# zju3dv/EnvGS

Hardware: AMD Instinct MI355X
Metric: train iters/s (fwd+bwd of the render hot path + Adam step, one 800x800 view per GPU per iter) + render Mpix/s (higher is better)
Workload: dtype f32

## Files before the change

### envgs_amd/_lib.py

```python
import ctypes
import os

import torch

HERE = os.path.dirname(os.path.abspath(__file__))
LIB_PATH = os.path.join(HERE, "libenvgs_hip.so")
_lib = None

c_void_p, c_int, c_uint32, c_size_t = ctypes.c_void_p, ctypes.c_int, ctypes.c_uint32, ctypes.c_size_t


class RasterCfg(ctypes.Structure):
    _fields_ = [("P", ctypes.c_int32), ("sh_degree", ctypes.c_int32), ("sh_coeffs", ctypes.c_int32),
                ("channels", ctypes.c_int32), ("width", ctypes.c_int32), ("height", ctypes.c_int32),
                ("bg_len", ctypes.c_int32), ("debug", ctypes.c_int32), ("scale_modifier", ctypes.c_float),
                ("tanfovx", ctypes.c_float), ("tanfovy", ctypes.c_float), ("feature_f16", ctypes.c_int32)]


class AdamTensor(ctypes.Structure):
    _fields_ = [("param", ctypes.c_void_p), ("grad", ctypes.c_void_p), ("exp_avg", ctypes.c_void_p), ("exp_avg_sq", ctypes.c_void_p),
                ("numel", ctypes.c_int64), ("lr", ctypes.c_float), ("step", ctypes.c_float)]


class RowsTensor(ctypes.Structure):
    _fields_ = [("src", ctypes.c_void_p), ("dst", ctypes.c_void_p), ("row_bytes", ctypes.c_int64)]


class GrowTensor(ctypes.Structure):
    _fields_ = [("src", ctypes.c_void_p), ("dst", ctypes.c_void_p), ("row_bytes", ctypes.c_int64), ("kind", ctypes.c_int32), ("reserved0", ctypes.c_int32)]


class DensifyPlanArgs(ctypes.Structure):
    _fields_ = ([("P", ctypes.c_int64), ("N", ctypes.c_int32), ("flags", ctypes.c_uint32)]
                + [(n, ctypes.c_float) for n in ("grad_threshold", "size_limit", "split_screen_threshold", "min_opacity", "min_gradient", "r")]
                + [(n, ctypes.c_void_p) for n in ("ga", "dn", "mr", "wa", "scal", "opac", "cls", "scan", "counters", "temp")]
                + [("temp_bytes", ctypes.c_size_t)])


class DensifyRewriteArgs(ctypes.Structure):
    _fields_ = ([("P", ctypes.c_int64), ("out_rows", ctypes.c_int64), ("n_samples", ctypes.c_int64), ("N", ctypes.c_int32), ("count", ctypes.c_int32),
                 ("ratio_n", ctypes.c_double), ("r", ctypes.c_float), ("reserved0", ctypes.c_uint32)]
                + [(n, ctypes.c_void_p) for n in ("cls", "scan", "counters", "scal", "rotation", "samples")]
                + [("tensors", ctypes.POINTER(GrowTensor))])


class TraceLists(ctypes.Structure):
    _fields_ = [("hit_lists", ctypes.c_void_p), ("hit_cnt", ctypes.c_void_p), ("n_used", ctypes.c_void_p), ("cap", ctypes.c_int32),
                ("surf_acc", ctypes.c_void_p), ("surf_cnt", ctypes.c_void_p), ("surf_off", ctypes.c_void_p),
                ("scan_temp", ctypes.c_void_p), ("scan_temp_bytes", ctypes.c_size_t), ("ray_keys", ctypes.c_void_p),
                ("ray_order", ctypes.c_void_p), ("ray_sort_temp", ctypes.c_void_p), ("ray_sort_temp_bytes", ctypes.c_size_t),
                ("records", ctypes.c_void_p),
                ("num_records", ctypes.c_uint64), ("hit_state", ctypes.c_void_p), ("entries", ctypes.c_void_p), ("pairs", ctypes.c_void_p),
                ("n_entries", ctypes.c_void_p), ("compact_rows", ctypes.c_uint64), ("row_off", ctypes.c_void_p), ("batch_rows", ctypes.c_void_p),
                ("row_blk", ctypes.c_void_p), ("sh_perm", ctypes.c_void_p), ("state_planes", ctypes.c_int32),
                ("sparse_hits", ctypes.c_void_p), ("sparse_cap", ctypes.c_uint64),
                ("defer_reduce", ctypes.c_uint32), ("reserved0", ctypes.c_uint32), ("bwd_order", ctypes.c_void_p)]


class TraceCfg(ctypes.Structure):
    _fields_ = [("P", ctypes.c_int32), ("num_rays", ctypes.c_int32), ("sh_degree", ctypes.c_int32),
                ("sh_coeffs", ctypes.c_int32), ("max_trace_depth", ctypes.c_int32), ("start_from_first", ctypes.c_int32),
                ("has_others", ctypes.c_int32), ("bg_len", ctypes.c_int32), ("debug", ctypes.c_int32),
                ("ray_h", ctypes.c_int32), ("ray_w", ctypes.c_int32),
                ("scale_modifier", ctypes.c_float), ("specular_threshold", ctypes.c_float), ("feature_f16", ctypes.c_int32)]


TRACE_COUNTER_WORDS, TRACE_COUNTER_MIRROR, TRACE_MAX_SEG = 96, 72, 4
CTR_RAY_FETCH, CTR_MAX_LIST, CTR_TOTALS = 0, 1, 2
(TOT_HITS, TOT_NODE_VISITS, TOT_ROUNDS, TOT_FOUND, TOT_PACKET_NODES, TOT_PACKET_LEAVES, TOT_COOP_EXPAND, TOT_COOP_WALK, TOT_COOP_WAIT,
 TOT_COUNT) = range(10)
CTR_STACK_OVERFLOWS, CTR_RAYS_WITHOUT_ROWS, CTR_ROW_CLAIM, CTR_LONG_QUEUE, CTR_SEG_FIRST_ROW = 20, 21, 22, 24, 28
CTR_BATCH_FETCH, CTR_BATCH_FETCH_STRIDE = 32, 8
CTR_SPARSE_FILED, CTR_BATCH_ENTRIES, CTR_SPARSE_SKIPPED = 64, 65, 66
DBG_TRACE, DBG_TRACE_NO_SORT, DBG_TRACE_SMALL_STACK, DBG_TRACE_PREPARE_INLINE = 0, 64, 1024, 16384
DBG_TRACE_RETIRED = 8 | 16 | 512 | 2048 | 4096 | 8192


class SupervisorArgs(ctypes.Structure):
    _fields_ = ([("N", ctypes.c_int64), ("P", ctypes.c_int64), ("flags", ctypes.c_uint32), ("reserved0", ctypes.c_uint32),
                 ("weight", ctypes.c_float * 5), ("reserved1", ctypes.c_float)]
                + [(n, ctypes.c_void_p) for n in ("norm_map", "surf_norm_map", "acc_map", "dpt_map", "dist_map", "env_opacity", "prior", "msk", "R", "near_far")]
                + [(n, ctypes.c_int64) for n in ("norm_map_row", "norm_map_ch", "surf_norm_map_row", "surf_norm_map_ch", "acc_map_row", "dpt_map_row",
                                                 "dist_map_row", "env_opacity_row", "prior_row", "prior_ch", "msk_row")]
                + [(n, ctypes.c_void_p) for n in ("g_norm_map", "g_surf_norm_map", "g_acc_map", "g_dist_map", "g_env_opacity", "partial")])


class SurfelInputsArgs(ctypes.Structure):
    _fields_ = ([(n, ctypes.c_int32) for n in ("P", "sh_degree", "sh_coeffs", "spec_channels")]
                + [(n, ctypes.c_void_p) for n in ("xyz", "features_dc", "features_rest", "scaling", "rotation", "opacity", "specular", "roughness", "campos",
                                                  "scales", "rotations", "opacities", "specular_act", "roughness_act", "shs", "colors", "others", "vertices",
                                                  "clamped",
                                                  "g_scales", "g_rotations", "g_opacities", "g_specular_act", "g_roughness_act", "g_shs", "g_colors", "g_others",
                                                  "d_xyz", "d_features_dc", "d_features_rest", "d_scaling", "d_rotation", "d_opacity", "d_specular", "d_roughness")])


class TsdfVolume(ctypes.Structure):
    _fields_ = ([(n, ctypes.c_int32) for n in ("nx", "ny", "nz")] + [(n, ctypes.c_float) for n in ("ox", "oy", "oz", "voxel")]
                + [(n, ctypes.c_void_p) for n in ("tsdf", "weight", "rgb")])


class TsdfView(ctypes.Structure):
    _fields_ = [("depth", ctypes.c_void_p), ("rgb", ctypes.c_void_p), ("H", ctypes.c_int32), ("W", ctypes.c_int32),
                ("fx", ctypes.c_float), ("fy", ctypes.c_float), ("cx", ctypes.c_float), ("cy", ctypes.c_float),
                ("R", ctypes.c_float * 9), ("T", ctypes.c_float * 3), ("depth_max", ctypes.c_float), ("trunc", ctypes.c_float)]


class TsdfViews(ctypes.Structure):
    _fields_ = [("count", ctypes.c_int32), ("reserved0", ctypes.c_int32), ("v", TsdfView * 8)]


_P = c_void_p
SYMBOLS = {
    "envgs_raster_scan_temp_bytes": (c_size_t, [ctypes.c_int32]),
    "envgs_raster_sort_temp_bytes": (c_size_t, [c_uint32, ctypes.c_int32, ctypes.c_int32]),
    "envgs_raster_project": (c_int, [ctypes.POINTER(RasterCfg)] + [_P] * 15 + [_P, c_size_t, ctypes.POINTER(c_uint32), _P]),
    "envgs_raster_bin_and_render": (c_int, [ctypes.POINTER(RasterCfg), c_uint32] + [_P] * 7 + [_P, c_size_t] + [_P] * 7 + [_P]),
    "envgs_raster_render_audit": (c_int, [ctypes.POINTER(RasterCfg)] + [_P] * 11 + [ctypes.c_int32, _P, _P]),
    "envgs_raster_backward": (c_int, [ctypes.POINTER(RasterCfg), c_uint32] + [_P] * 29 + [_P]),
    "envgs_bvh_temp_bytes": (c_size_t, [ctypes.c_int32]),
    "envgs_bvh_node_floats": (c_size_t, [ctypes.c_int32]),
    "envgs_bvh_build": (c_int, [ctypes.c_int32, _P, _P, _P, _P, c_size_t, ctypes.c_int32, _P]),
    "envgs_bvh_refit": (c_int, [ctypes.c_int32, _P, _P, _P, _P, _P, c_size_t, ctypes.c_int32, _P]),
    "envgs_bvh_quality": (c_int, [ctypes.c_int32, _P, _P, _P]),
    "envgs_trace_ray_sort_temp_bytes": (c_size_t, [ctypes.c_int32]),
    "envgs_trace_ray_order": (c_int, [ctypes.c_int32, _P, _P, _P, ctypes.c_int32, _P, _P, _P, c_size_t, _P]),
    "envgs_trace_forward": (c_int, [ctypes.POINTER(TraceCfg)] + [_P] * 22 + [ctypes.POINTER(TraceLists), _P]),
    "envgs_trace_backward": (c_int, [ctypes.POINTER(TraceCfg)] + [_P] * 35 + [ctypes.POINTER(TraceLists), _P]),
    "envgs_trace_backward_join": (c_int, [_P]),
    "envgs_sh_colors_forward": (c_int, [ctypes.c_int32] * 4 + [_P] * 7 + [_P]),
    "envgs_sh_colors_backward": (c_int, [ctypes.c_int32] * 4 + [_P] * 9 + [_P]),
    "envgs_surfel_quads": (c_int, [ctypes.c_int32] + [_P] * 5 + [_P]),
    "envgs_blend_forward": (c_int, [ctypes.c_int32] * 3 + [_P] * 3 + [_P]),
    "envgs_blend_backward": (c_int, [ctypes.c_int32] * 3 + [_P] * 5 + [_P]),
    "envgs_bounce_rays_forward": (c_int, [ctypes.c_int32] + [_P] * 8 + [_P]),
    "envgs_bounce_rays_backward": (c_int, [ctypes.c_int32] + [_P] * 13 + [_P]),
    "envgs_bounce_blend_forward": (c_int, [ctypes.c_int32] + [_P] * 5 + [_P]),
    "envgs_bounce_blend_backward": (c_int, [ctypes.c_int32] + [_P] * 8 + [_P]),
    "envgs_bounce_pack_mid": (c_int, [ctypes.c_int32, _P, ctypes.c_int32, ctypes.c_int32] + [_P] * 8 + [_P]),
    "envgs_reflect_forward": (c_int, [ctypes.c_int32, ctypes.c_int32, ctypes.c_float] + [_P] * 8 + [_P]),
    "envgs_reflect_backward": (c_int, [ctypes.c_int32, ctypes.c_int32, ctypes.c_float] + [_P] * 11 + [_P]),
    "envgs_select_acc": (c_int, [ctypes.c_int32, ctypes.c_int32, ctypes.c_float, _P, _P, _P]),
    "envgs_reflect_filtered_forward": (c_int, [ctypes.c_int32, ctypes.c_int32, ctypes.c_float, ctypes.c_int32] + [_P] * 10 + [_P]),
    "envgs_reflect_filtered_backward": (c_int, [ctypes.c_int32, ctypes.c_int32, ctypes.c_float, ctypes.c_int32] + [_P] * 13 + [_P]),
    "envgs_blend_filtered_forward": (c_int, [ctypes.c_int32] * 4 + [_P] * 6 + [_P]),
    "envgs_blend_filtered_backward": (c_int, [ctypes.c_int32] * 4 + [_P] * 7 + [_P]),
    "envgs_surface_normal_forward": (c_int, [ctypes.c_int32, ctypes.c_int32, ctypes.c_float, ctypes.c_float, ctypes.c_float] + [_P] * 4 + [_P]),
    "envgs_surface_normal_backward": (c_int, [ctypes.c_int32, ctypes.c_int32, ctypes.c_float, ctypes.c_float, ctypes.c_float] + [_P] * 5 + [_P]),
    "envgs_surfel_inputs_forward": (c_int, [ctypes.POINTER(SurfelInputsArgs), _P]),
    "envgs_surfel_inputs_backward": (c_int, [ctypes.POINTER(SurfelInputsArgs), _P]),
    "envgs_fused_adam": (c_int, [ctypes.c_int32, ctypes.POINTER(AdamTensor), ctypes.c_float, ctypes.c_float, ctypes.c_float, _P]),
    "envgs_compact_temp_bytes": (ctypes.c_size_t, [ctypes.c_int64]),
    "envgs_compact_scan": (c_int, [ctypes.c_int64, _P, _P, _P, _P, ctypes.c_size_t, _P]),
    "envgs_compact_gather": (c_int, [ctypes.c_int32, ctypes.POINTER(RowsTensor), ctypes.c_int64, _P, _P, _P]),
    "envgs_compact_gather_rows": (c_int, [ctypes.c_int32, ctypes.POINTER(RowsTensor), ctypes.c_int64, ctypes.c_int64, _P, _P, _P]),
    "envgs_knn3_mean_dist2": (c_int, [ctypes.c_int32, _P, _P, _P]),
    "envgs_densify_stats": (c_int, [ctypes.c_int64, ctypes.c_int32] + [_P] * 8 + [_P]),
    "envgs_densify_plan_temp_bytes": (ctypes.c_size_t, [ctypes.c_int64]),
    "envgs_densify_plan": (c_int, [ctypes.POINTER(DensifyPlanArgs), _P]),
    "envgs_densify_split_stds": (c_int, [ctypes.c_int64, ctypes.c_int32] + [_P] * 5 + [ctypes.c_int64, _P]),
    "envgs_densify_rewrite": (c_int, [ctypes.POINTER(DensifyRewriteArgs), _P]),
    "envgs_weight_select_temp_bytes": (ctypes.c_size_t, []),
    "envgs_weight_select": (c_int, [ctypes.c_int64, _P, _P, ctypes.c_int32, ctypes.c_int64, ctypes.c_int64, _P, _P, _P, ctypes.c_size_t, _P]),
    "envgs_visibility_mask_temp_bytes": (ctypes.c_size_t, [ctypes.c_int64]),
    "envgs_visibility_mask": (c_int, [ctypes.c_int64, _P, _P, ctypes.c_int64, _P, _P, _P, _P, ctypes.c_size_t, _P]),
    "envgs_oversize_plan": (c_int, [ctypes.c_int64, c_uint32, ctypes.c_float, ctypes.c_float] + [_P] * 8 + [_P]),
    "envgs_tsdf_integrate": (c_int, [ctypes.POINTER(TsdfVolume), ctypes.POINTER(TsdfViews), ctypes.c_float, _P]),
    "envgs_mesh_temp_bytes": (c_size_t, [ctypes.c_int32] * 3),
    "envgs_mesh_count": (c_int, [ctypes.POINTER(TsdfVolume), ctypes.c_float, ctypes.c_float, _P, c_size_t, _P, _P]),
    "envgs_mesh_extract": (c_int, [ctypes.POINTER(TsdfVolume), ctypes.c_float, _P, c_size_t, c_uint32, c_uint32, _P, _P, _P, _P]),
    "envgs_mesh_components_temp_bytes": (c_size_t, [c_uint32, c_uint32]),
    "envgs_mesh_components": (c_int, [c_uint32, c_uint32, _P, _P, c_size_t] + [_P] * 5 + [_P]),
    "envgs_mesh_select_temp_bytes": (c_size_t, [c_uint32, c_uint32]),
    "envgs_mesh_select_count": (c_int, [c_uint32, c_uint32, _P, _P, _P, c_size_t, _P, _P]),
    "envgs_mesh_select_emit": (c_int, [c_uint32, c_uint32] + [_P] * 4 + [_P, c_size_t, c_uint32, c_uint32] + [_P] * 4 + [_P]),
    "envgs_mesh_simplify_temp_bytes": (c_size_t, [c_uint32, c_uint32] + [ctypes.c_int32] * 3),
    "envgs_mesh_simplify_cluster": (c_int, [c_uint32, c_uint32, _P, _P, _P] + [ctypes.c_float] * 4 + [ctypes.c_int32] * 3 + [_P, c_size_t] + [_P] * 6 + [_P]),
    "envgs_mesh_sample_temp_bytes": (c_size_t, [c_uint32, c_uint32]),
    "envgs_mesh_sample_count": (c_int, [c_uint32, c_uint32, _P, _P, ctypes.c_float, c_uint32, _P, c_size_t, _P, _P]),
    "envgs_mesh_sample_emit": (c_int, [c_uint32, c_uint32, _P, _P, _P, c_uint32, _P, c_size_t, c_uint32, _P, _P, _P, _P]),
    "envgs_points_grid_temp_bytes": (c_size_t, [c_uint32] + [ctypes.c_int32] * 3),
    "envgs_points_grid_build": (c_int, [c_uint32, _P] + [ctypes.c_float] * 4 + [ctypes.c_int32] * 3 + [_P, c_size_t, _P, _P, _P]),
    "envgs_points_nearest": (c_int, [c_uint32, _P] + [ctypes.c_float] * 5 + [ctypes.c_int32] * 3 + [_P] * 4 + [_P]),
    "envgs_l1_ssim_partial_count": (ctypes.c_int64, [ctypes.c_int32, ctypes.c_int32, ctypes.c_int32]),
    "envgs_l1_ssim_forward": (c_int, [ctypes.c_int32, ctypes.c_int32, ctypes.c_int32, _P, _P, _P, _P, _P]),
    "envgs_l1_ssim_backward": (c_int, [ctypes.c_int32, ctypes.c_int32, ctypes.c_int32, _P, _P, _P, _P, ctypes.c_float, ctypes.c_float, _P, _P]),
    "envgs_depth_percentiles_temp_bytes": (c_size_t, []),
    "envgs_depth_percentiles": (c_int, [ctypes.c_int64, _P, ctypes.c_int64, _P, _P, c_size_t, _P]),
    "envgs_supervisor_partial_count": (ctypes.c_int64, [ctypes.c_int64, ctypes.c_int64]),
    "envgs_supervisor_forward": (c_int, [ctypes.POINTER(SupervisorArgs), _P]),
    "envgs_supervisor_finish": (c_int, [ctypes.POINTER(SupervisorArgs), _P, _P]),
    "envgs_supervisor_backward": (c_int, [ctypes.c_int64, _P, _P, _P, _P]),
    "envgs_debug_set": (None, [ctypes.c_int32, ctypes.c_int32]),
    "envgs_debug_get": (ctypes.c_int32, [ctypes.c_int32]),
    "envgs_prof_enable": (None, [c_int]),
    "envgs_prof_select": (None, [ctypes.c_uint64]),
    "envgs_prof_read": (c_int, [c_int, ctypes.POINTER(ctypes.c_double), ctypes.POINTER(c_int)]),
    "envgs_prof_kernel_name": (ctypes.c_char_p, [c_int]),
}


LIB_DIAG_PATH = os.path.join(HERE, "libenvgs_hip_diag.so")
_libs = {}
_selected = {"kind": "product"}


def _open(path):
    if not os.path.exists(path):
        raise RuntimeError(
            "envgs_amd: %s is missing. Build it with `python -m envgs_amd.build` (hipcc, gfx950). "
            "There is no CPU fallback for the render-and-trace path." % path)
    lib = ctypes.CDLL(path)
    for name, (res, args) in SYMBOLS.items():
        fn = getattr(lib, name)
        fn.restype = res
        fn.argtypes = args
    return lib


def load():
    global _lib
    kind = _selected["kind"]
    lib = _libs.get(kind)
    if lib is None:
        lib = _libs[kind] = _open(LIB_PATH if kind == "product" else LIB_DIAG_PATH)
    _lib = lib
    return lib


def select(kind):
    if kind not in ("product", "diag"):
        raise ValueError(kind)
    old = _selected["kind"]
    _selected["kind"] = kind
    load()
    return old


def ptr(t):
    return None if t is None else ctypes.c_void_p(t.data_ptr())


def check(rc, what):
    if rc != 0:
        raise RuntimeError("envgs_amd: %s failed with code %d (%s)" % (
            what, rc, {-1: "bad argument", -2: "temp buffer too small"}.get(rc, "hipError_t")))
```

### envgs_amd/csrc/common.h

```cpp
#pragma once
#include <hip/hip_runtime.h>
#include <hip/hip_fp16.h>
#include <stdint.h>

#include "../../include/envgs_raster.h"
#include "prof.h"

namespace envgs {

constexpr int TILE = ENVGS_TILE;
constexpr int GEOM = ENVGS_GEOM_STRIDE;
constexpr int GREC = ENVGS_GRAD_STRIDE;
constexpr float NEAR_N = 0.2f;
constexpr float FAR_N = 100.0f;
constexpr float FILTER_SIZE = 0.707106f;
constexpr float FILTER_INV_SQ = 2.0f;
constexpr float ALPHA_CAP = 0.99f;
constexpr float ALPHA_MIN = 1.0f / 255.0f;
constexpr float T_EPS = 0.0001f;

struct Feat {
    const void *p;
    bool h;
    __device__ __forceinline__ float operator[](size_t i) const {
        return h ? __half2float(reinterpret_cast<const __half *>(p)[i]) : reinterpret_cast<const float *>(p)[i];
    }
    __device__ __forceinline__ Feat at(size_t i) const { return Feat{reinterpret_cast<const char *>(p) + i * (h ? 2 : 4), h}; }
};

#define ENVGS_CHECK_LAUNCH(cfg, stream)                                             \
    do {                                                                            \
        hipError_t e__ = hipGetLastError();                                         \
        if (e__ != hipSuccess) return (int)e__;                                     \
        if ((cfg)->debug) {                                                         \
            e__ = hipStreamSynchronize((hipStream_t)(stream));                      \
            if (e__ != hipSuccess) return (int)e__;                                 \
        }                                                                           \
    } while (0)

template <int CTRL, int ROW_MASK = 0xf, int BANK_MASK = 0xf, bool BOUND = true>
__device__ __forceinline__ float dpp_mov(float v) {
    return __builtin_bit_cast(float, __builtin_amdgcn_update_dpp(0, __builtin_bit_cast(int, v), CTRL, ROW_MASK, BANK_MASK, BOUND));
}
template <int CTRL> __device__ __forceinline__ int dpp_mov_i32(int v) { return __builtin_amdgcn_update_dpp(0, v, CTRL, 0xf, 0xf, true); }
__device__ __forceinline__ float quad_sum(float v) { v += dpp_mov<0xB1>(v); v += dpp_mov<0x4E>(v); return v; }

__device__ __forceinline__ float wave_sum(float v) {
    v += dpp_mov<0xB1>(v);
    v += dpp_mov<0x4E>(v);
    v += dpp_mov<0x141>(v);
    v += dpp_mov<0x140>(v);
    v += dpp_mov<0x142, 0xa, 0xf, false>(v);
    v += dpp_mov<0x143, 0xc, 0xf, false>(v);
    return __builtin_bit_cast(float, __builtin_amdgcn_readlane(__builtin_bit_cast(int, v), 63));
}


typedef unsigned envgs_u2 __attribute__((ext_vector_type(2)));

__device__ __forceinline__ float wave_reduce64(const float (&g)[64], const int lane)
{
    float z[32];
#pragma unroll
    for (int i = 0; i < 32; i++) {
        const envgs_u2 r = __builtin_amdgcn_permlane32_swap(__float_as_uint(g[i]), __float_as_uint(g[i + 32]), false, false);
        z[i] = __uint_as_float(r.x) + __uint_as_float(r.y);
    }
    float w[16];
#pragma unroll
    for (int k = 0; k < 16; k++) {
        const envgs_u2 q = __builtin_amdgcn_permlane16_swap(__float_as_uint(z[k]), __float_as_uint(z[k + 16]), false, false);
        w[k] = __uint_as_float(q.x) + __uint_as_float(q.y);
    }
    const bool b3 = lane & 8, b2 = lane & 4, b1 = lane & 2, b0 = lane & 1;
    float a[8];
#pragma unroll
    for (int k = 0; k < 8; k++) a[k] = (b3 ? w[k + 8] : w[k]) + dpp_mov<0x140>(b3 ? w[k] : w[k + 8]);
    float b[4];
#pragma unroll
    for (int k = 0; k < 4; k++) b[k] = (b2 ? a[k + 4] : a[k]) + dpp_mov<0x141>(b2 ? a[k] : a[k + 4]);
    float c[2];
#pragma unroll
    for (int k = 0; k < 2; k++) c[k] = (b1 ? b[k + 2] : b[k]) + dpp_mov<0x1B>(b1 ? b[k] : b[k + 2]);
    return (b0 ? c[1] : c[0]) + dpp_mov<0xB1>(b0 ? c[0] : c[1]);
}

template <int CTRL, int ROW_MASK = 0xf>
__device__ __forceinline__ float dpp_fill(float v, float ident) {
    return __builtin_bit_cast(float, __builtin_amdgcn_update_dpp(__builtin_bit_cast(int, ident), __builtin_bit_cast(int, v), CTRL, ROW_MASK, 0xf, false));
}
__device__ __forceinline__ float wave_scan_add(float v) {
    v += dpp_fill<0x111>(v, 0.f); v += dpp_fill<0x112>(v, 0.f); v += dpp_fill<0x114>(v, 0.f); v += dpp_fill<0x118>(v, 0.f);
    v += dpp_fill<0x142, 0xa>(v, 0.f);
    v += dpp_fill<0x143, 0xc>(v, 0.f);
    return v;
}
__device__ __forceinline__ float wave_scan_mul(float v) {
    v *= dpp_fill<0x111>(v, 1.f); v *= dpp_fill<0x112>(v, 1.f); v *= dpp_fill<0x114>(v, 1.f); v *= dpp_fill<0x118>(v, 1.f);
    v *= dpp_fill<0x142, 0xa>(v, 1.f);
    v *= dpp_fill<0x143, 0xc>(v, 1.f);
    return v;
}
__device__ __forceinline__ float wave_bcast(float v, int l) { return __builtin_bit_cast(float, __builtin_amdgcn_readlane(__builtin_bit_cast(int, v), l)); }

template <int CTRL, int ROW_MASK = 0xf>
__device__ __forceinline__ uint32_t dpp_fill_u32(uint32_t v) {
    return (uint32_t)__builtin_amdgcn_update_dpp(0, (int)v, CTRL, ROW_MASK, 0xf, false);
}
__device__ __forceinline__ uint32_t wave_scan_add_u32(uint32_t v) {
    v += dpp_fill_u32<0x111>(v); v += dpp_fill_u32<0x112>(v); v += dpp_fill_u32<0x114>(v); v += dpp_fill_u32<0x118>(v);
    v += dpp_fill_u32<0x142, 0xa>(v);
    v += dpp_fill_u32<0x143, 0xc>(v);
    return v;
}

template <int N4>
__device__ __forceinline__ float wave_transpose_reduce(const float (&g)[4 * N4], const int lane)
{
    float z[2 * N4];
#pragma unroll
    for (int i = 0; i < 2 * N4; i++) {
        const envgs_u2 r = __builtin_amdgcn_permlane32_swap(__float_as_uint(g[i]), __float_as_uint(g[i + 2 * N4]), false, false);
        z[i] = __uint_as_float(r.x) + __uint_as_float(r.y);
    }
    float w[N4];
#pragma unroll
    for (int k = 0; k < N4; k++) {
        const envgs_u2 q = __builtin_amdgcn_permlane16_swap(__float_as_uint(z[k]), __float_as_uint(z[k + N4]), false, false);
        float v = __uint_as_float(q.x) + __uint_as_float(q.y);
        v += dpp_mov<0x128>(v);
        v += dpp_mov<0x124>(v);
        v += dpp_mov<0x122>(v);
        v += dpp_mov<0x121>(v);
        w[k] = v;
    }
    float out = w[0];
#pragma unroll
    for (int k = 1; k < N4; k++) out = ((lane & 15) == k) ? w[k] : out;
    return out;
}

__device__ __forceinline__ int lane_id() { return __builtin_amdgcn_mbcnt_hi(~0u, __builtin_amdgcn_mbcnt_lo(~0u, 0u)); }

template <int NW>
__device__ __forceinline__ uint32_t block_exclusive_u32(uint32_t v, uint32_t *s_w, uint32_t &total)
{
    const int lane = lane_id(), wave = threadIdx.x >> 6;
    const uint32_t inc = wave_scan_add_u32(v);
    if (lane == 63) s_w[wave] = inc;
    __syncthreads();
    uint32_t before = 0, all = 0;
#pragma unroll
    for (int k = 0; k < NW; k++) { const uint32_t t = s_w[k]; all += t; before += (k < wave) ? t : 0u; }
    total = all;
    __syncthreads();
    return before + inc - v;
}

__device__ __forceinline__ void atomic_add_f32(float *p, float v) { unsafeAtomicAdd(p, v); }

int launch_project(const envgs_raster_cfg *cfg, const float *means3D, const float *scales, const float *rotations,
                   const float *opacities, const float *shs, const float *transmat_precomp, const float *viewmatrix,
                   const float *projmatrix, const float *campos, float *geom, float *rgb, uint8_t *clamped,
                   int32_t *radii, uint32_t *tiles_touched, hipStream_t stream);
int launch_scan(const uint32_t *in, uint32_t *out, int n, void *temp, size_t temp_bytes, hipStream_t stream);
size_t scan_temp_bytes(int n);
size_t sort_temp_bytes(uint32_t n, int width, int height);
int launch_bin(const envgs_raster_cfg *cfg, uint32_t N, const float *geom, const int32_t *radii, uint64_t *tile_pairs,
               uint64_t *keys_sorted, uint32_t *point_list, void *bin_temp, size_t bin_temp_bytes, uint32_t *ranges, hipStream_t stream);
size_t key_sort_temp_bytes(int n);
int launch_key_sort(int n, const uint64_t *keys_in, uint64_t *keys_out, int top_bit, void *temp, size_t temp_bytes, hipStream_t stream);
size_t ray_sort_temp_bytes(int R);
int launch_ray_sort(int R, const float *ray_o, const float *ray_d, const float4 *nodes, int P, uint64_t *pairs, uint32_t *order, void *temp,
                    size_t temp_bytes, hipStream_t stream);
int launch_render_fwd(const envgs_raster_cfg *cfg, const uint32_t *ranges, const uint32_t *point_list, const float *geom,
                      const float *colors, const float *bg, float *out_color, float *allmap, float *final_T,
                      int32_t *n_contrib, float *weight, hipStream_t stream, uint8_t *audit_contrib = nullptr, int audit_lmax = 0, int colors_f16 = 0,
                      uint8_t *contrib_mask = nullptr, const uint8_t *audit_skip = nullptr);
int launch_render_bwd(const envgs_raster_cfg *cfg, const uint32_t *ranges, const uint32_t *point_list, const float *geom,
                      const float *colors, const float *bg, const float *final_T, const int32_t *n_contrib,
                      const float *dL_dcolor, const float *dL_dallmap, float *grad_rec, hipStream_t stream, int colors_f16 = 0,
                      const uint8_t *contrib_mask = nullptr);
int launch_project_bwd(const envgs_raster_cfg *cfg, const float *geom, const float *means3D, const float *scales,
                       const float *rotations, const float *shs, const uint8_t *clamped, const float *transmat_precomp,
                       const int32_t *radii, const float *viewmatrix, const float *projmatrix, const float *campos,
                       const float *grad_rec, float *dmeans3D, float *dmeans2D, float *dscales, float *drots, float *dshs,
                       float *dcolors, float *dopacities, float *dtransmat_precomp, hipStream_t stream);

int launch_sh_record_bwd(int P, int D, const float *means3D, const float *shs, const float *campos, const uint8_t *clamped, const int32_t *radii,
                         const float *grad_rec, float *dmeans3D, float *dshs, hipStream_t stream);

__host__ __device__ inline int tile_bits(int width, int height) {
    int tiles = ((width + TILE - 1) / TILE) * ((height + TILE - 1) / TILE);
    int b = 0;
    while ((1 << b) < tiles) b++;
    return b < 1 ? 1 : b;
}

}
```

### envgs_amd/csrc/raster_api.hip

```cpp
#include "common.h"

using namespace envgs;

extern "C" {

size_t envgs_raster_scan_temp_bytes(int32_t P) { return scan_temp_bytes(P); }

size_t envgs_raster_sort_temp_bytes(uint32_t N, int32_t width, int32_t height)
{
    return sort_temp_bytes(N, width, height);
}

static int check_cfg(const envgs_raster_cfg *cfg)
{
    if (!cfg) return ENVGS_ERR_BAD_ARG;
    if (cfg->channels != 3 && cfg->channels != 5 && cfg->channels != 7) return ENVGS_ERR_BAD_ARG;
    if (cfg->sh_degree < 0 || cfg->sh_degree > 3) return ENVGS_ERR_BAD_ARG;
    if (cfg->width <= 0 || cfg->height <= 0 || cfg->P < 0) return ENVGS_ERR_BAD_ARG;
    return 0;
}

int envgs_raster_project(const envgs_raster_cfg *cfg, const float *means3D, const float *scales, const float *rotations,
                         const float *opacities, const float *shs, const float *transmat_precomp,
                         const float *viewmatrix, const float *projmatrix, const float *campos, float *geom, float *rgb,
                         uint8_t *clamped, int32_t *radii, uint32_t *tiles_touched, uint32_t *offsets, void *scan_temp,
                         size_t scan_temp_bytes_, uint32_t *num_rendered_host, void *stream_)
{
    int rc = check_cfg(cfg);
    if (rc) return rc;
    if (num_rendered_host) *num_rendered_host = 0;
    if (cfg->P == 0) return 0;
    if (!means3D || !opacities || !viewmatrix || !projmatrix || !geom || !radii || !tiles_touched || !offsets) return ENVGS_ERR_BAD_ARG;
    if (!transmat_precomp && (!scales || !rotations)) return ENVGS_ERR_BAD_ARG;
    if (shs && (cfg->channels != 3 || !rgb || !clamped || !campos || cfg->sh_coeffs < (cfg->sh_degree + 1) * (cfg->sh_degree + 1))) return ENVGS_ERR_BAD_ARG;
    hipStream_t stream = (hipStream_t)stream_;
    rc = launch_project(cfg, means3D, scales, rotations, opacities, shs, transmat_precomp, viewmatrix, projmatrix, campos,
                        geom, rgb, clamped, radii, tiles_touched, stream);
    if (rc) return rc;
    if (scan_temp_bytes_ < scan_temp_bytes(cfg->P)) return ENVGS_ERR_TEMP_TOO_SMALL;
    rc = launch_scan(tiles_touched, offsets, cfg->P, scan_temp, scan_temp_bytes_, stream);
    if (rc) return rc;
    if (!num_rendered_host) return 0;
    hipError_t e = hipMemcpyAsync(num_rendered_host, offsets + (cfg->P - 1), sizeof(uint32_t), hipMemcpyDeviceToHost, stream);
    if (e != hipSuccess) return (int)e;
    e = hipStreamSynchronize(stream);
    return (int)e;
}

int envgs_raster_bin_and_render(const envgs_raster_cfg *cfg, uint32_t N, const float *geom, const int32_t *radii,
                                const float *colors, const float *bg, uint64_t *tile_pairs, uint64_t *keys_sorted, uint32_t *point_list,
                                void *bin_temp, size_t bin_temp_bytes_, uint32_t *ranges, float *out_color, float *allmap,
                                float *final_T, int32_t *n_contrib, float *weight, uint8_t *contrib_mask, void *stream_)
{
    int rc = check_cfg(cfg);
    if (rc) return rc;
    if (!ranges || !out_color || !allmap || !final_T || !n_contrib || !bg) return ENVGS_ERR_BAD_ARG;
    if (cfg->P > 0 && (!geom || !radii || !colors || !weight)) return ENVGS_ERR_BAD_ARG;
    if (N > 0 && (!tile_pairs || !point_list || !bin_temp)) return ENVGS_ERR_BAD_ARG;
    hipStream_t stream = (hipStream_t)stream_;
    rc = launch_bin(cfg, N, geom, radii, tile_pairs, keys_sorted, point_list, bin_temp, bin_temp_bytes_, ranges, stream);
    if (rc) return rc;
    return launch_render_fwd(cfg, ranges, point_list, geom, colors, bg, out_color, allmap, final_T, n_contrib, weight, stream, nullptr, 0,
                             (cfg->feature_f16 && cfg->sh_coeffs == 0) ? 1 : 0, contrib_mask);
}

int envgs_raster_render_audit(const envgs_raster_cfg *cfg, const float *geom, const float *colors, const float *bg,
                              const uint32_t *point_list, const uint32_t *ranges, float *out_color, float *allmap, float *final_T,
                              int32_t *n_contrib, float *weight, uint8_t *contrib, int32_t lmax, const uint8_t *skip_px, void *stream_)
{
    int rc = check_cfg(cfg);
    if (rc) return rc;
    if (!ranges || !out_color || !allmap || !final_T || !n_contrib || !bg || !contrib || lmax <= 0) return ENVGS_ERR_BAD_ARG;
    if (cfg->P > 0 && (!geom || !colors || !weight || !point_list)) return ENVGS_ERR_BAD_ARG;
    hipStream_t stream = (hipStream_t)stream_;
    hipError_t e = hipMemsetAsync(contrib, 0, (size_t)cfg->width * cfg->height * (size_t)lmax, stream);
    if (e != hipSuccess) return (int)e;
    return launch_render_fwd(cfg, ranges, point_list, geom, colors, bg, out_color, allmap, final_T, n_contrib, weight, stream, contrib, lmax,
                             (cfg->feature_f16 && cfg->sh_coeffs == 0) ? 1 : 0, nullptr, skip_px);
}

int envgs_raster_backward(const envgs_raster_cfg *cfg, uint32_t N, const float *geom, const float *colors, const float *bg,
                          const uint32_t *point_list, const uint32_t *ranges, const float *final_T,
                          const int32_t *n_contrib, const uint8_t *contrib_mask, const float *dL_dcolor, const float *dL_dallmap, const float *means3D,
                          const float *scales, const float *rotations, const float *shs, const uint8_t *clamped,
                          const float *transmat_precomp, const int32_t *radii, const float *viewmatrix,
                          const float *projmatrix, const float *campos, float *grad_rec, float *dmeans3D, float *dmeans2D,
                          float *dscales, float *drots, float *dshs, float *dcolors, float *dopacities,
                          float *dtransmat_precomp, void *stream_)
{
    int rc = check_cfg(cfg);
    if (rc) return rc;
    if (cfg->P == 0) return 0;
    if (!geom || !colors || !bg || !ranges || !final_T || !n_contrib || !grad_rec || !radii ||
        !dmeans2D || !dopacities || !viewmatrix || !projmatrix)
        return ENVGS_ERR_BAD_ARG;
    if (N > 0 && !point_list) return ENVGS_ERR_BAD_ARG;
    if (shs ? (!dshs || !clamped || !campos || !means3D) : !dcolors) return ENVGS_ERR_BAD_ARG;
    if (transmat_precomp ? !dtransmat_precomp : (!scales || !rotations || !means3D || !dmeans3D || !dscales || !drots)) return ENVGS_ERR_BAD_ARG;
    hipStream_t stream = (hipStream_t)stream_;
    rc = launch_render_bwd(cfg, ranges, point_list, geom, colors, bg, final_T, n_contrib, dL_dcolor, dL_dallmap, grad_rec, stream,
                           (cfg->feature_f16 && !shs) ? 1 : 0, contrib_mask);
    if (rc) return rc;
    return launch_project_bwd(cfg, geom, means3D, scales, rotations, shs, clamped, transmat_precomp, radii, viewmatrix,
                              projmatrix, campos, grad_rec, dmeans3D, dmeans2D, dscales, drots, dshs, dcolors, dopacities,
                              dtransmat_precomp, stream);
}

}
```

### envgs_amd/csrc/raster_bin.hip

```cpp
#include "common.h"
#include "ray_key.h"
#include "tile_sort.h"

namespace envgs {

constexpr int SCAN_ITEMS = 1024;

size_t scan_temp_bytes(int n) { return sizeof(uint32_t) * (size_t)(((n > 0 ? n : 1) + SCAN_ITEMS - 1) / SCAN_ITEMS) + 64; }

__global__ void __launch_bounds__(256)
scan_block_sums(const uint32_t *__restrict__ in, uint32_t *__restrict__ sums, int n)
{
    __shared__ uint32_t s_w[5];
    const int base = blockIdx.x * SCAN_ITEMS + threadIdx.x * 4;
    uint32_t s = 0;
#pragma unroll
    for (int k = 0; k < 4; k++) s += (base + k < n) ? in[base + k] : 0u;
    uint32_t total;
    (void)block_exclusive_u32<4>(s, s_w, total);
    if (threadIdx.x == 0) sums[blockIdx.x] = total;
}

__global__ void __launch_bounds__(256)
scan_apply(const uint32_t *in, uint32_t *out, const uint32_t *__restrict__ sums, int n)
{
    __shared__ uint32_t s_w[5];
    uint32_t pre = 0;
    for (int k = threadIdx.x; k < (int)blockIdx.x; k += 256) pre += sums[k];
    uint32_t before;
    (void)block_exclusive_u32<4>(pre, s_w, before);
    const int base = blockIdx.x * SCAN_ITEMS + threadIdx.x * 4;
    uint32_t a[4];
#pragma unroll
    for (int k = 0; k < 4; k++) a[k] = (base + k < n) ? in[base + k] : 0u;
    a[1] += a[0]; a[2] += a[1]; a[3] += a[2];
    uint32_t total;
    const uint32_t ex = block_exclusive_u32<4>(a[3], s_w, total) + before;
#pragma unroll
    for (int k = 0; k < 4; k++) if (base + k < n) out[base + k] = ex + a[k];
}

int launch_scan(const uint32_t *in, uint32_t *out, int n, void *temp, size_t temp_bytes, hipStream_t stream)
{
    if (n <= 0) return 0;
    if (temp_bytes < scan_temp_bytes(n)) return ENVGS_ERR_TEMP_TOO_SMALL;
    ProfScope prof_(K_SCAN, stream);
    const int nb = (n + SCAN_ITEMS - 1) / SCAN_ITEMS;
    hipLaunchKernelGGL(scan_block_sums, dim3(nb), dim3(256), 0, stream, in, (uint32_t *)temp, n);
    hipLaunchKernelGGL(scan_apply, dim3(nb), dim3(256), 0, stream, in, out, (const uint32_t *)temp, n);
    return (int)hipGetLastError();
}

constexpr int BIN_ROWS_MAX = 512;
constexpr int BIN_SLICE_MIN = 1024;
constexpr int BIN_BAND = 16384;
constexpr int BIG_RECT = 32;
constexpr int SORT_LONG_N = 16384;
constexpr int SORT_LONG_WGS = 256;

struct BinPlan { int rows, slice, ntiles; };
static BinPlan bin_plan(int P, int W, int H)
{
    BinPlan p;
    p.ntiles = ((W + TILE - 1) / TILE) * ((H + TILE - 1) / TILE);
    int rows = (P + BIN_SLICE_MIN - 1) / BIN_SLICE_MIN;
    rows = rows < 1 ? 1 : (rows > BIN_ROWS_MAX ? BIN_ROWS_MAX : rows);
    p.slice = (((P + rows - 1) / rows + 255) / 256) * 256;
    p.rows = p.slice > 0 ? (P + p.slice - 1) / p.slice : 1;
    if (p.rows < 1) p.rows = 1;
    return p;
}

size_t sort_temp_bytes(uint32_t, int width, int height)
{
    const size_t ntiles = (size_t)((width + TILE - 1) / TILE) * ((height + TILE - 1) / TILE);
    return sizeof(uint32_t) * ((size_t)BIN_ROWS_MAX * ntiles + 3 * ntiles + 1 + 4) + 256;
}

__device__ __forceinline__ bool tile_rect(int i, int W, int H, const float *__restrict__ geom, const int32_t *__restrict__ radii,
                                          int &x0, int &y0, int &x1, int &y1, uint32_t &dbits)
{
    const int rad = radii[i];
    if (rad <= 0) return false;
    const float cx = geom[(size_t)i * GEOM + 9], cy = geom[(size_t)i * GEOM + 10];
    dbits = __float_as_uint(geom[(size_t)i * GEOM + 15]);
    const float radius = (float)rad;
    const int gx = (W + TILE - 1) / TILE, gy = (H + TILE - 1) / TILE;
    x0 = (int)((cx - radius) / (float)TILE); x0 = x0 < 0 ? 0 : (x0 > gx ? gx : x0);
    y0 = (int)((cy - radius) / (float)TILE); y0 = y0 < 0 ? 0 : (y0 > gy ? gy : y0);
    x1 = (int)((cx + radius + (float)(TILE - 1)) / (float)TILE); x1 = x1 < 0 ? 0 : (x1 > gx ? gx : x1);
    y1 = (int)((cy + radius + (float)(TILE - 1)) / (float)TILE); y1 = y1 < 0 ? 0 : (y1 > gy ? gy : y1);
    return x1 > x0 && y1 > y0;
}

struct SurfelRect { int x0, y0, x1, y1; uint32_t dbits; bool vis; };
__device__ __forceinline__ SurfelRect load_rect(int i, int g1, int W, int H, const float *__restrict__ geom, const int32_t *__restrict__ radii)
{
    SurfelRect r;
    r.x0 = r.y0 = r.x1 = r.y1 = 0; r.dbits = 0;
    r.vis = i < g1 && tile_rect(i, W, H, geom, radii, r.x0, r.y0, r.x1, r.y1, r.dbits);
    return r;
}

template <bool SCATTER>
__global__ void __launch_bounds__(256)
bin_pass(int P, int W, int H, int slice, int ntiles, const float *__restrict__ geom, const int32_t *__restrict__ radii,
         uint32_t *hist, const uint32_t *__restrict__ tile_start, uint64_t *__restrict__ pairs, uint32_t cap)
{
    extern __shared__ uint32_t s_bin[];
    const int gx = (W + TILE - 1) / TILE;
    const int g0 = blockIdx.x * slice, g1 = min(P, g0 + slice);
    uint32_t *row = hist + (size_t)blockIdx.x * ntiles;
    const int lane = lane_id();
    for (int band0 = 0; band0 < ntiles; band0 += BIN_BAND) {
        const int bn = min(BIN_BAND, ntiles - band0);
        SurfelRect cur = load_rect(g0 + (int)threadIdx.x, g1, W, H, geom, radii);
        for (int t = threadIdx.x; t < bn; t += 256) s_bin[t] = SCATTER ? tile_start[band0 + t] + row[band0 + t] : 0u;
        __syncthreads();
        auto visit = [&](int t, uint64_t pair) {
            t -= band0;
            if ((unsigned)t >= (unsigned)bn) return;
            const uint32_t slot = atomicAdd(&s_bin[t], 1u);
            if (SCATTER && slot < cap) pairs[slot] = pair;
        };
        for (int ib = g0; ib < g1; ib += 256) {
            const int i = ib + (int)threadIdx.x;
            const SurfelRect c = cur;
            cur = load_rect(i + 256, g1, W, H, geom, radii);
            const int x0 = c.x0, y0 = c.y0, x1 = c.x1, y1 = c.y1;
            const uint32_t dbits = c.dbits;
            const bool vis = c.vis;
            const uint64_t pair = ((uint64_t)dbits << 32) | (uint32_t)i;
            const bool big = vis && (x1 - x0) * (y1 - y0) > BIG_RECT;
            if (vis && !big)
                for (int y = y0; y < y1; y++)
                    for (int x = x0; x < x1; x++) visit(y * gx + x, pair);
            uint64_t m = __builtin_amdgcn_ballot_w64(big);
            while (m) {
                const int l = __builtin_ctzll(m);
                m &= m - 1;
                const int bx0 = __builtin_amdgcn_readlane(x0, l), by0 = __builtin_amdgcn_readlane(y0, l);
                const int bw = __builtin_amdgcn_readlane(x1, l) - bx0, bh = __builtin_amdgcn_readlane(y1, l) - by0;
                const uint64_t bp = ((uint64_t)(uint32_t)__builtin_amdgcn_readlane((int)dbits, l) << 32) | (uint32_t)__builtin_amdgcn_readlane(i, l);
                for (int k = lane; k < bw * bh; k += 64) visit((by0 + k / bw) * gx + bx0 + k % bw, bp);
            }
        }
        __syncthreads();
        if (!SCATTER)
            for (int t = threadIdx.x; t < bn; t += 256) row[band0 + t] = s_bin[t];
        __syncthreads();
    }
}

constexpr int CS_SEG = 16, CS_ROWS = BIN_ROWS_MAX / CS_SEG;
__global__ void __launch_bounds__(256)
bin_column_scan(int rows, int ntiles, uint32_t *hist, uint32_t *__restrict__ tile_count)
{
    __shared__ uint32_t s_seg[CS_SEG][16];
    const int tl = threadIdx.x & 15, seg = threadIdx.x >> 4;
    const int t = blockIdx.x * 16 + tl;
    const int per = (rows + CS_SEG - 1) / CS_SEG, r0 = seg * per;
    uint32_t v[CS_ROWS];
    uint32_t s = 0;
#pragma unroll
    for (int k = 0; k < CS_ROWS; k++) {
        const int r = r0 + k;
        v[k] = (t < ntiles && k < per && r < rows) ? hist[(size_t)r * ntiles + t] : 0u;
        s += v[k];
    }
    s_seg[seg][tl] = s;
    __syncthreads();
    uint32_t acc = 0;
#pragma unroll
    for (int k = 0; k < CS_SEG; k++) acc += (k < seg) ? s_seg[k][tl] : 0u;
    if (t >= ntiles) return;
#pragma unroll
    for (int k = 0; k < CS_ROWS; k++) {
        const int r = r0 + k;
        if (k < per && r < rows) hist[(size_t)r * ntiles + t] = acc;
        acc += v[k];
    }
    if (seg == CS_SEG - 1) tile_count[t] = acc;
}

__global__ void __launch_bounds__(1024)
bin_tile_scan(int ntiles, const uint32_t *__restrict__ tile_count, uint32_t *__restrict__ tile_start, uint32_t *__restrict__ ranges,
              uint32_t cap, uint32_t *__restrict__ hdr)
{
    __shared__ uint32_t s_w[17];
    const int per = (ntiles + 1023) / 1024, b = min(ntiles, (int)threadIdx.x * per), e = min(ntiles, b + per);
    uint32_t s = 0;
    for (int k = b; k < e; k++) s += tile_count[k];
    uint32_t total;
    uint32_t run = block_exclusive_u32<16>(s, s_w, total);
    const bool ok = total <= cap;
    for (int k = b; k < e; k++) {
        const uint32_t c = tile_count[k];
        tile_start[k] = run;
        ranges[2 * k] = (c && ok) ? run : 0u;
        ranges[2 * k + 1] = (c && ok) ? run + c : 0u;
        run += c;
    }
    if (threadIdx.x == 0) { tile_start[ntiles] = total; hdr[0] = total; hdr[1] = 0u; hdr[2] = 0u; hdr[3] = 0u; }
}

template <int NT>
__device__ __forceinline__ void sort_padded_lds(uint64_t *s, int lp, int tid)
{
    const int npad = 1 << lp;
    for (int g = tid; g < (npad >> TS_S); g += NT) bitonic_first(s, g, lp);
    __syncthreads();
    for (int lk = TS_S + 1; lk <= lp; lk++)
        for (int a = lk - 1; a >= 0;) {
            const int S = ts_chunk(a);
            if (S == 4) { for (int g = tid; g < (npad >> 4); g += NT) bitonic_group<4>(s, g, lk, a, lp); }
            else if (S == 3) { for (int g = tid; g < (npad >> 3); g += NT) bitonic_group<3>(s, g, lk, a, lp); }
            else if (S == 2) { for (int g = tid; g < (npad >> 2); g += NT) bitonic_group<2>(s, g, lk, a, lp); }
            else { for (int g = tid; g < (npad >> 1); g += NT) bitonic_group<1>(s, g, lk, a, lp); }
            __syncthreads();
            a -= S;
        }
}

template <int NT>
__device__ __forceinline__ void merge_padded_lds(uint64_t *s, int lc, int tid)
{
    const int npad = 1 << lc;
    for (int a = lc - 1; a >= 0;) {
        const int S = ts_chunk(a);
        if (S == 4) { for (int g = tid; g < (npad >> 4); g += NT) bitonic_group<4>(s, g, lc, a, lc); }
        else if (S == 3) { for (int g = tid; g < (npad >> 3); g += NT) bitonic_group<3>(s, g, lc, a, lc); }
        else if (S == 2) { for (int g = tid; g < (npad >> 2); g += NT) bitonic_group<2>(s, g, lc, a, lc); }
        else { for (int g = tid; g < (npad >> 1); g += NT) bitonic_group<1>(s, g, lc, a, lc); }
        __syncthreads();
        a -= S;
    }
}

constexpr int lds_slots(int lp_cap) { return (1 << lp_cap) + (1 << (lp_cap - 5)); }

__device__ __forceinline__ void store_sorted(uint64_t v, uint32_t tile, size_t at, uint64_t *keys_sorted, uint32_t *point_list, int full64)
{
    if (full64) { keys_sorted[at] = v; return; }
    point_list[at] = (uint32_t)v;
    if (keys_sorted) keys_sorted[at] = ((uint64_t)tile << 32) | (v >> 32);
}

template <int NT>
__device__ __forceinline__ void load_sort_write(uint64_t *s, const uint64_t *pairs, int n, uint32_t tile, uint32_t b,
                                                uint64_t *keys_sorted, uint32_t *point_list, int tid, int full64)
{
    const int lp = ts_log2_padded(n);
    for (int i = tid; i < (1 << lp); i += NT) s[ts_slot(i)] = i < n ? pairs[b + i] : ~0ull;
    __syncthreads();
    sort_padded_lds<NT>(s, lp, tid);
    for (int i = tid; i < n; i += NT) store_sorted(s[ts_slot(i)], tile, (size_t)b + i, keys_sorted, point_list, full64);
}

template <int LP_CAP, int NT>
__global__ void __launch_bounds__(NT)
sort_tile_lists(const uint32_t *__restrict__ ranges, const uint64_t *pairs, uint64_t *keys_sorted, uint32_t *__restrict__ point_list,
                uint32_t *__restrict__ hdr, uint32_t *__restrict__ long_list, int full64)
{
    __shared__ uint64_t s_k[lds_slots(LP_CAP)];
    const uint32_t t = blockIdx.x, b = ranges[2 * t];
    const int n = (int)(ranges[2 * t + 1] - b);
    if (n == 0) return;
    if (n > (1 << LP_CAP)) {
        if (threadIdx.x == 0) long_list[atomicAdd(&hdr[1], 1u)] = t;
        return;
    }
    load_sort_write<NT>(s_k, pairs, n, t, b, keys_sorted, point_list, (int)threadIdx.x, full64);
}

constexpr int LONG_ITEM = 4096;
constexpr int LONG_BATCH = 256;

__device__ __forceinline__ uint32_t long_claim(uint32_t *hdr, uint32_t *s_item)
{
    __syncthreads();
    if (threadIdx.x == 0) *s_item = atomicAdd(&hdr[2], 1u);
    __syncthreads();
    return *s_item;
}
__device__ __forceinline__ void long_wait(uint32_t *hdr, const uint32_t base)
{
    if (threadIdx.x == 0)
        while (__hip_atomic_load(&hdr[3], __ATOMIC_ACQUIRE, __HIP_MEMORY_SCOPE_AGENT) < base) __builtin_amdgcn_s_sleep(4);
    __syncthreads();
    __threadfence();
}
__device__ __forceinline__ void long_done(uint32_t *hdr)
{
    __threadfence();
    __syncthreads();
    if (threadIdx.x == 0) __hip_atomic_fetch_add(&hdr[3], 1u, __ATOMIC_RELEASE, __HIP_MEMORY_SCOPE_AGENT);
}

__global__ void __launch_bounds__(1024)
sort_long_lists(const uint32_t *__restrict__ ranges, uint64_t *pairs, uint64_t *keys_sorted, uint32_t *__restrict__ point_list,
                uint32_t *hdr, const uint32_t *__restrict__ long_list, int full64)
{
    __shared__ uint64_t s_long[lds_slots(14)];
    __shared__ uint32_t s_item;
    __shared__ uint32_t s_bt[LONG_BATCH], s_bb[LONG_BATCH], s_bn[LONG_BATCH], s_pref[LONG_BATCH + 1];
    const uint32_t count = hdr[1];
    const int tid = (int)threadIdx.x, G = (int)gridDim.x;
    constexpr int LC = 14, C = 1 << LC;
    const bool copy_out = !(full64 && keys_sorted == pairs);
    uint32_t small_seen = 0u, big = 0u;
    for (uint32_t w = 0; w < count; w++) {
        const uint32_t t = long_list[w], b = ranges[2 * t];
        const int n = (int)(ranges[2 * t + 1] - b);
        if (n > SORT_LONG_N) { big++; continue; }
        if ((small_seen++ % (uint32_t)G) != blockIdx.x) continue;
        load_sort_write<1024>(s_long, pairs, n, t, b, keys_sorted, point_list, tid, full64);
        __syncthreads();
    }
    if (big == 0u) return;
    auto lp_of = [&](const int n) { int lp = LC; while ((1 << lp) < n) lp++; return lp; };
    auto items_of = [&](const int kind, const int lk, const int n) -> uint32_t {
        const int lp = lp_of(n);
        if (kind == 1) return lk <= lp ? (uint32_t)(((1ll << (lp - 1)) + LONG_ITEM - 1) / LONG_ITEM) : 0u;
        return (kind == 2 || lk <= lp) ? (uint32_t)((n + C - 1) / C) : 0u;
    };
    auto do_item = [&](const int kind, const int lk, const int q, const int l, const uint32_t it) {
        const uint32_t t = s_bt[l], b = s_bb[l];
        const int n = (int)s_bn[l];
        uint64_t *seg = pairs + b;
        if (kind == 0) {
            const int c = (int)it;
            for (int i = tid; i < C; i += 1024) s_long[ts_slot(i)] = ((long long)c * C + i) < n ? seg[(size_t)c * C + i] : ~0ull;
            __syncthreads();
            if (lk == LC) sort_padded_lds<1024>(s_long, LC, tid);
            else merge_padded_lds<1024>(s_long, LC, tid);
            for (int i = tid; i < C; i += 1024)
                if ((long long)c * C + i < n) seg[(size_t)c * C + i] = s_long[ts_slot(i)];
        } else if (kind == 1) {
            const int lp = lp_of(n);
            const long long i0 = (long long)it * LONG_ITEM, i1 = min(i0 + LONG_ITEM, 1ll << (lp - 1));
            for (long long idx = i0 + tid; idx < i1; idx += 1024) ascending_step(seg, n, lk, q, (int)idx);
        } else {
            const long long i0 = (long long)it * C, i1 = min(i0 + C, (long long)n);
            for (long long i = i0 + tid; i < i1; i += 1024) store_sorted(seg[i], t, (size_t)b + (size_t)i, keys_sorted, point_list, full64);
        }
    };
    uint32_t base = 0u, my = long_claim(hdr, &s_item);
    uint32_t w = 0;
    while (w < count) {
        __syncthreads();
        int nl = 0, lp_max = LC;
        for (; w < count && nl < LONG_BATCH; w++) {
            const uint32_t t = long_list[w], b = ranges[2 * t];
            const int n = (int)(ranges[2 * t + 1] - b);
            if (n <= SORT_LONG_N) continue;
            if (tid == 0) { s_bt[nl] = t; s_bb[nl] = b; s_bn[nl] = (uint32_t)n; }
            lp_max = max(lp_max, lp_of(n));
            nl++;
        }
        if (nl == 0) break;
        auto run_phase = [&](const int kind, const int lk, const int q) {
            __syncthreads();
            if (tid < nl) {
                uint32_t acc = 0u;
                for (int l = 0; l < tid; l++) acc += items_of(kind, lk, (int)s_bn[l]);
                s_pref[tid] = acc;
                if (tid == nl - 1) s_pref[nl] = acc + items_of(kind, lk, (int)s_bn[tid]);
            }
            __syncthreads();
            const uint32_t items = s_pref[nl];
            while (my - base < items) {
                const uint32_t j = my - base;
                int lo = 0, hi = nl - 1;
                while (lo < hi) { const int mid = (lo + hi + 1) >> 1; if (s_pref[mid] <= j) lo = mid; else hi = mid - 1; }
                long_wait(hdr, base);
                do_item(kind, lk, q, lo, j - s_pref[lo]);
                long_done(hdr);
                my = long_claim(hdr, &s_item);
            }
            base += items;
        };
        run_phase(0, LC, 0);
        for (int lk = LC + 1; lk <= lp_max; lk++) {
            for (int q = 0; q <= lk - LC - 1; q++) run_phase(1, lk, q);
            run_phase(0, lk, 0);
        }
        if (copy_out) run_phase(2, 0, 0);
    }
}

static int long_sort_grid()
{
    static int cached[16] = {};
    int dev = 0;
    if (hipGetDevice(&dev) != hipSuccess || dev < 0 || dev >= 16) return 64;
    if (cached[dev] == 0) {
        int cus = 0;
        if (hipDeviceGetAttribute(&cus, hipDeviceAttributeMultiprocessorCount, dev) != hipSuccess || cus <= 0) cus = 64;
        cached[dev] = cus < SORT_LONG_WGS ? cus : SORT_LONG_WGS;
    }
    return cached[dev];
}

int launch_bin(const envgs_raster_cfg *cfg, uint32_t N, const float *geom, const int32_t *radii, uint64_t *tile_pairs,
               uint64_t *keys_sorted, uint32_t *point_list, void *bin_temp, size_t bin_temp_bytes, uint32_t *ranges, hipStream_t stream)
{
    const BinPlan pl = bin_plan(cfg->P, cfg->width, cfg->height);
    if (N == 0 || cfg->P <= 0) return (int)hipMemsetAsync(ranges, 0, sizeof(uint32_t) * 2 * (size_t)pl.ntiles, stream);
    if (bin_temp_bytes < sort_temp_bytes(N, cfg->width, cfg->height)) return ENVGS_ERR_TEMP_TOO_SMALL;
    uint32_t *hist = (uint32_t *)bin_temp;
    uint32_t *tile_count = hist + (size_t)BIN_ROWS_MAX * pl.ntiles;
    uint32_t *tile_start = tile_count + pl.ntiles;
    uint32_t *long_list = tile_start + pl.ntiles + 1;
    uint32_t *hdr = long_list + pl.ntiles;
    const size_t lds = sizeof(uint32_t) * (size_t)(pl.ntiles < BIN_BAND ? pl.ntiles : BIN_BAND);
    prof_begin(K_EMIT_KEYS, stream);
    hipLaunchKernelGGL(bin_pass<false>, dim3(pl.rows), dim3(256), lds, stream, cfg->P, cfg->width, cfg->height, pl.slice, pl.ntiles,
                       geom, radii, hist, (const uint32_t *)nullptr, (uint64_t *)nullptr, 0u);
    ENVGS_CHECK_LAUNCH(cfg, stream);
    hipLaunchKernelGGL(bin_column_scan, dim3((pl.ntiles + 15) / 16), dim3(256), 0, stream, pl.rows, pl.ntiles, hist, tile_count);
    ENVGS_CHECK_LAUNCH(cfg, stream);
    hipLaunchKernelGGL(bin_tile_scan, dim3(1), dim3(1024), 0, stream, pl.ntiles, tile_count, tile_start, ranges, N, hdr);
    ENVGS_CHECK_LAUNCH(cfg, stream);
    hipLaunchKernelGGL(bin_pass<true>, dim3(pl.rows), dim3(256), lds, stream, cfg->P, cfg->width, cfg->height, pl.slice, pl.ntiles,
                       geom, radii, hist, tile_start, tile_pairs, N);
    ENVGS_CHECK_LAUNCH(cfg, stream);
    prof_end(K_EMIT_KEYS, stream);
    ProfScope prof_(K_SORT, stream);
    const uint64_t want = (uint64_t)N * 8 / ((uint64_t)pl.ntiles * 5);
    if (want <= 2048)
        hipLaunchKernelGGL((sort_tile_lists<11, 128>), dim3(pl.ntiles), dim3(128), 0, stream, ranges, tile_pairs, keys_sorted, point_list, hdr, long_list, 0);
    else if (want <= 4096)
        hipLaunchKernelGGL((sort_tile_lists<12, 256>), dim3(pl.ntiles), dim3(256), 0, stream, ranges, tile_pairs, keys_sorted, point_list, hdr, long_list, 0);
    else
        hipLaunchKernelGGL((sort_tile_lists<13, 512>), dim3(pl.ntiles), dim3(512), 0, stream, ranges, tile_pairs, keys_sorted, point_list, hdr, long_list, 0);
    ENVGS_CHECK_LAUNCH(cfg, stream);
    hipLaunchKernelGGL(sort_long_lists, dim3(long_sort_grid()), dim3(1024), 0, stream, ranges, tile_pairs,
                       keys_sorted, point_list, hdr, long_list, 0);
    ENVGS_CHECK_LAUNCH(cfg, stream);
    return 0;
}

static void launch_bucket_sorts(uint64_t n, int nb, const uint32_t *ranges, uint64_t *pairs, uint64_t *keys_sorted, uint32_t *point_list,
                                uint32_t *hdr, uint32_t *long_list, int full64, hipStream_t stream)
{
    const uint64_t want = n * 8 / ((uint64_t)nb * 5);
    if (want <= 2048)
        hipLaunchKernelGGL((sort_tile_lists<11, 128>), dim3(nb), dim3(128), 0, stream, ranges, pairs, keys_sorted, point_list, hdr, long_list, full64);
    else if (want <= 4096)
        hipLaunchKernelGGL((sort_tile_lists<12, 256>), dim3(nb), dim3(256), 0, stream, ranges, pairs, keys_sorted, point_list, hdr, long_list, full64);
    else
        hipLaunchKernelGGL((sort_tile_lists<13, 512>), dim3(nb), dim3(512), 0, stream, ranges, pairs, keys_sorted, point_list, hdr, long_list, full64);
    hipLaunchKernelGGL(sort_long_lists, dim3(long_sort_grid()), dim3(1024), 0, stream, ranges, pairs, keys_sorted, point_list, hdr, long_list, full64);
}

static int ray_bucket_bits(int R)
{
    int b = 4;
    while (b < 13 && ((long long)160 << b) < R) b++;
    return b;
}

size_t ray_sort_temp_bytes(int R)
{
    const size_t nb = (size_t)1 << ray_bucket_bits(R);
    return sizeof(uint32_t) * ((size_t)BIN_ROWS_MAX * nb + 5 * nb + 1 + 4 + (size_t)(R > 0 ? R : 1) + 6 * (size_t)BIN_ROWS_MAX) + 256;
}

__global__ void __launch_bounds__(256)
ray_origin_bounds(int R, int slice, const float *__restrict__ ray_o, float *__restrict__ partial)
{
    __shared__ float s_red[4][6];
    const int g0 = blockIdx.x * slice, g1 = min(R, g0 + slice);
    float lo[3] = {3.0e38f, 3.0e38f, 3.0e38f}, hi[3] = {-3.0e38f, -3.0e38f, -3.0e38f};
    for (int i = g0 + (int)threadIdx.x; i < g1; i += 256) {
#pragma unroll
        for (int c = 0; c < 3; c++) { const float x = ray_o[3 * i + c]; if (x == x && fabsf(x) < 1.0e30f) { lo[c] = fminf(lo[c], x); hi[c] = fmaxf(hi[c], x); } }
    }
#pragma unroll
    for (int c = 0; c < 3; c++)
        for (int o = 32; o > 0; o >>= 1) { lo[c] = fminf(lo[c], __shfl_xor(lo[c], o)); hi[c] = fmaxf(hi[c], __shfl_xor(hi[c], o)); }
    const int wave = threadIdx.x >> 6, lane = threadIdx.x & 63;
    if (lane == 0) { for (int c = 0; c < 3; c++) { s_red[wave][c] = lo[c]; s_red[wave][3 + c] = hi[c]; } }
    __syncthreads();
    if (threadIdx.x < 6) {
        const int c = threadIdx.x;
        float v = s_red[0][c];
        for (int w = 1; w < 4; w++) v = c < 3 ? fminf(v, s_red[w][c]) : fmaxf(v, s_red[w][c]);
        partial[blockIdx.x * 6 + c] = v;
    }
}

template <bool SCATTER>
__global__ void __launch_bounds__(256)
ray_bucket_pass(int R, int slice, int nb, int shift, const float *__restrict__ ray_o, const float *__restrict__ ray_d,
                const float *__restrict__ bounds_partial, int nrows, int lead, uint32_t *__restrict__ keys, uint32_t *hist, const uint32_t *__restrict__ bucket_start,
                uint64_t *__restrict__ pairs)
{
    extern __shared__ uint32_t s_bin[];
    __shared__ float s_box[6];
    const int g0 = blockIdx.x * slice, g1 = min(R, g0 + slice);
    uint32_t *row = hist + (size_t)blockIdx.x * nb;
    for (int t = threadIdx.x; t < nb; t += 256) s_bin[t] = SCATTER ? bucket_start[t] + row[t] : 0u;
    if (!SCATTER && threadIdx.x < 64) {
        const int c = threadIdx.x % 6, j0 = threadIdx.x / 6;
        float v = c < 3 ? 3.0e38f : -3.0e38f;
        if (j0 < 10)
            for (int j = j0; j < nrows; j += 10) { const float x = bounds_partial[j * 6 + c]; v = c < 3 ? fminf(v, x) : fmaxf(v, x); }
        float acc = v;
        for (int k = 1; k < 10; k++) { const float x = __shfl(v, (int)(threadIdx.x % 6) + 6 * k); if (threadIdx.x < 6) acc = c < 3 ? fminf(acc, x) : fmaxf(acc, x); }
        if (threadIdx.x < 6) s_box[c] = acc;
    }
    __syncthreads();
    float lo0 = 0.f, lo1 = 0.f, lo2 = 0.f, s0 = 0.f, s1 = 0.f, s2 = 0.f;
    if (!SCATTER) {
        lo0 = s_box[0]; lo1 = s_box[1]; lo2 = s_box[2];
        const float e0 = s_box[3] - lo0, e1 = s_box[4] - lo1, e2 = s_box[5] - lo2;
        s0 = e0 > 0.f ? 32.0f / e0 : 0.f; s1 = e1 > 0.f ? 32.0f / e1 : 0.f; s2 = e2 > 0.f ? 32.0f / e2 : 0.f;
    }
    for (int i = g0 + (int)threadIdx.x; i < g1; i += 256) {
        uint32_t key;
        if (SCATTER) key = keys[i];
        else keys[i] = key = ray_coherence_key(i, ray_o, ray_d, lo0, lo1, lo2, s0, s1, s2, lead);
        const uint32_t slot = atomicAdd(&s_bin[key >> shift], 1u);
        if (SCATTER) pairs[slot] = ((uint64_t)key << 32) | (uint32_t)i;
    }
    __syncthreads();
    if (!SCATTER)
        for (int t = threadIdx.x; t < nb; t += 256) row[t] = s_bin[t];
}

int launch_ray_sort(int R, const float *ray_o, const float *ray_d, const float4 *nodes, int P, uint64_t *pairs, uint32_t *order,
                    void *temp, size_t temp_bytes, hipStream_t stream)
{
    (void)nodes; (void)P;
    if (R <= 0) return 0;
    if (temp_bytes < ray_sort_temp_bytes(R)) return ENVGS_ERR_TEMP_TOO_SMALL;
    const int bits = ray_bucket_bits(R), nb = 1 << bits, shift = 31 - bits;
    int rows = (R + BIN_SLICE_MIN - 1) / BIN_SLICE_MIN;
    rows = rows < 1 ? 1 : (rows > BIN_ROWS_MAX ? BIN_ROWS_MAX : rows);
    const int slice = (((R + rows - 1) / rows + 255) / 256) * 256;
    rows = (R + slice - 1) / slice;
    uint32_t *hist = (uint32_t *)temp;
    uint32_t *count = hist + (size_t)BIN_ROWS_MAX * nb;
    uint32_t *start = count + nb;
    uint32_t *long_list = start + nb + 1;
    uint32_t *hdr = long_list + nb;
    uint32_t *ranges = hdr + 4;
    uint32_t *keys = ranges + 2 * (size_t)nb;
    float *partial = (float *)(keys + (size_t)R);
    const size_t lds = sizeof(uint32_t) * (size_t)nb;
    int lead = debug_switch(ENVGS_DBG_RAYKEY) > 0 ? debug_switch(ENVGS_DBG_RAYKEY) - 1 : RAY_KEY_LEAD;
    lead = lead > 8 ? 8 : lead;
    hipLaunchKernelGGL(ray_origin_bounds, dim3(rows), dim3(256), 0, stream, R, slice, ray_o, partial);
    hipLaunchKernelGGL(ray_bucket_pass<false>, dim3(rows), dim3(256), lds, stream, R, slice, nb, shift, ray_o, ray_d, (const float *)partial, rows, lead, keys, hist,
                       (const uint32_t *)nullptr, (uint64_t *)nullptr);
    hipLaunchKernelGGL(bin_column_scan, dim3((nb + 15) / 16), dim3(256), 0, stream, rows, nb, hist, count);
    hipLaunchKernelGGL(bin_tile_scan, dim3(1), dim3(1024), 0, stream, nb, count, start, ranges, (uint32_t)R, hdr);
    hipLaunchKernelGGL(ray_bucket_pass<true>, dim3(rows), dim3(256), lds, stream, R, slice, nb, shift, ray_o, ray_d, (const float *)partial, rows, lead, keys, hist, start, pairs);
    launch_bucket_sorts(R, nb, ranges, pairs, (uint64_t *)nullptr, order, hdr, long_list, 0, stream);
    return (int)hipGetLastError();
}

size_t key_sort_temp_bytes(int n)
{
    const size_t nb = (size_t)1 << ray_bucket_bits(n);
    return sizeof(uint32_t) * ((size_t)BIN_ROWS_MAX * nb + 5 * nb + 1 + 4) + 256;
}

template <bool SCATTER>
__global__ void __launch_bounds__(256)
key_bucket_pass(int n, int slice, int nb, int shift, const uint64_t *__restrict__ keys, uint32_t *hist, const uint32_t *__restrict__ bucket_start,
                uint64_t *__restrict__ out)
{
    extern __shared__ uint32_t s_bin[];
    const int g0 = blockIdx.x * slice, g1 = min(n, g0 + slice);
    uint32_t *row = hist + (size_t)blockIdx.x * nb;
    for (int t = threadIdx.x; t < nb; t += 256) s_bin[t] = SCATTER ? bucket_start[t] + row[t] : 0u;
    __syncthreads();
    for (int i = g0 + (int)threadIdx.x; i < g1; i += 256) {
        const uint64_t k = keys[i];
        const uint32_t slot = atomicAdd(&s_bin[(uint32_t)(k >> shift) & (uint32_t)(nb - 1)], 1u);
        if (SCATTER) out[slot] = k;
    }
    __syncthreads();
    if (!SCATTER)
        for (int t = threadIdx.x; t < nb; t += 256) row[t] = s_bin[t];
}

int launch_key_sort(int n, const uint64_t *keys_in, uint64_t *keys_out, int top_bit, void *temp, size_t temp_bytes, hipStream_t stream)
{
    if (n <= 0) return 0;
    if (temp_bytes < key_sort_temp_bytes(n)) return ENVGS_ERR_TEMP_TOO_SMALL;
    const int bits = ray_bucket_bits(n), nb = 1 << bits, shift = top_bit - bits;
    int rows = (n + BIN_SLICE_MIN - 1) / BIN_SLICE_MIN;
    rows = rows < 1 ? 1 : (rows > BIN_ROWS_MAX ? BIN_ROWS_MAX : rows);
    const int slice = (((n + rows - 1) / rows + 255) / 256) * 256;
    rows = (n + slice - 1) / slice;
    uint32_t *hist = (uint32_t *)temp;
    uint32_t *count = hist + (size_t)BIN_ROWS_MAX * nb;
    uint32_t *start = count + nb;
    uint32_t *long_list = start + nb + 1;
    uint32_t *hdr = long_list + nb;
    uint32_t *ranges = hdr + 4;
    const size_t lds = sizeof(uint32_t) * (size_t)nb;
    hipLaunchKernelGGL(key_bucket_pass<false>, dim3(rows), dim3(256), lds, stream, n, slice, nb, shift, keys_in, hist, (const uint32_t *)nullptr, (uint64_t *)nullptr);
    hipLaunchKernelGGL(bin_column_scan, dim3((nb + 15) / 16), dim3(256), 0, stream, rows, nb, hist, count);
    hipLaunchKernelGGL(bin_tile_scan, dim3(1), dim3(1024), 0, stream, nb, count, start, ranges, (uint32_t)n, hdr);
    hipLaunchKernelGGL(key_bucket_pass<true>, dim3(rows), dim3(256), lds, stream, n, slice, nb, shift, keys_in, hist, start, keys_out);
    launch_bucket_sorts((uint64_t)n, nb, ranges, keys_out, keys_out, (uint32_t *)nullptr, hdr, long_list, 1, stream);
    return (int)hipGetLastError();
}

}
```

### envgs_amd/csrc/raster_render.hip

```cpp
#include "common.h"

namespace envgs {

struct Hit {
    float sx, sy, inv, kx, ky, kz, lx, ly, lz, rho3d, rho2d, dx, dy, depth, G, alpha;
    bool ok;
};

template <bool EXACT>
__device__ __forceinline__ float recip(float x)
{
    if (EXACT) return 1.0f / x;
    const float r = __builtin_amdgcn_rcpf(x);
    return __builtin_fmaf(__builtin_fmaf(-x, r, 1.0f), r, r);
}
template <bool EXACT>
__device__ __forceinline__ float recip1(float x) { return EXACT ? 1.0f / x : __builtin_amdgcn_rcpf(x); }
template <bool EXACT>
__device__ __forceinline__ float expneg(float x) { return EXACT ? expf(x) : __expf(x); }

template <bool EXACT = false>
__device__ __forceinline__ Hit eval_splat(const float4 r0, const float4 r1, const float4 r2, const float4 r3, float px, float py)
{
    Hit h;
    const float Tux = r0.x, Tuy = r0.y, Tuz = r0.z, Tvx = r0.w, Tvy = r1.x, Tvz = r1.y, Twx = r1.z, Twy = r1.w, Twz = r2.x;
    const float cx = r2.y, cy = r2.z, opa = r3.z;
    h.kx = __builtin_fmaf(px, Twx, -Tux); h.ky = __builtin_fmaf(px, Twy, -Tuy); h.kz = __builtin_fmaf(px, Twz, -Tuz);
    h.lx = __builtin_fmaf(py, Twx, -Tvx); h.ly = __builtin_fmaf(py, Twy, -Tvy); h.lz = __builtin_fmaf(py, Twz, -Tvz);
    const float ppx = __builtin_fmaf(h.ky, h.lz, -(h.kz * h.ly));
    const float ppy = __builtin_fmaf(h.kz, h.lx, -(h.kx * h.lz));
    const float ppz = __builtin_fmaf(h.kx, h.ly, -(h.ky * h.lx));
    h.inv = recip<EXACT>(ppz);
    h.sx = ppx * h.inv; h.sy = ppy * h.inv;
    h.rho3d = __builtin_fmaf(h.sx, h.sx, h.sy * h.sy);
    h.dx = cx - px; h.dy = cy - py;
    h.rho2d = FILTER_INV_SQ * __builtin_fmaf(h.dx, h.dx, h.dy * h.dy);
    const bool use3d = h.rho3d <= h.rho2d;
    const float rho = use3d ? h.rho3d : h.rho2d;
    h.depth = use3d ? __builtin_fmaf(h.sx, Twx, __builtin_fmaf(h.sy, Twy, Twz)) : Twz;
    const float power = -0.5f * rho;
    h.G = expneg<EXACT>(power);
    const float a = opa * h.G;
    h.alpha = a < ALPHA_CAP ? a : ALPHA_CAP;
    h.ok = (ppz != 0.0f) && (h.depth >= NEAR_N) && (power <= 0.0f) && (h.alpha >= ALPHA_MIN);
    return h;
}

template <int C, int B = 256>
struct TileLds {
    float4 rec[4][B];
    float col[C][B];
    uint32_t id[B];
    unsigned long long qbits[4][(B + 63) / 64];
};

constexpr int BWD_BATCH = 192;

__device__ __forceinline__ int xcd_tile(int b, int ntiles)
{
    const int per = (ntiles + 7) >> 3;
    return (b & 7) * per + (b >> 3);
}

__device__ __forceinline__ uint32_t quadrant_mask(const float4 r0, const float4 r1, const float4 r2, const float4 r3, int tile_px, int tile_py)
{
    const float Tux = r0.x, Tuy = r0.y, Tuz = r0.z, Tvx = r0.w, Tvy = r1.x, Tvz = r1.y, Twx = r1.z, Twy = r1.w, Twz = r2.x;
    const float cx = r2.y, cy = r2.z, opa = r3.z;
    const float tau = 2.0f * __logf(255.0f * opa);
    if (!(tau >= 0.0f)) return 0u;
    const float r2d = sqrtf(0.5f * tau);
    float bx0 = cx - r2d, bx1 = cx + r2d, by0 = cy - r2d, by1 = cy + r2d;
    const float d = tau * (Twx * Twx + Twy * Twy) - Twz * Twz;
    if (!(d < 0.0f)) return 0xFu;
    const float id = 1.0f / d;
    const float f0 = tau * id, f2 = -id;
    const float pxc = f0 * (Tux * Twx + Tuy * Twy) + f2 * (Tuz * Twz);
    const float pyc = f0 * (Tvx * Twx + Tvy * Twy) + f2 * (Tvz * Twz);
    const float hx = pxc * pxc - (f0 * (Tux * Tux + Tuy * Tuy) + f2 * (Tuz * Tuz));
    const float hy = pyc * pyc - (f0 * (Tvx * Tvx + Tvy * Tvy) + f2 * (Tvz * Tvz));
    const float ex = sqrtf(fmaxf(hx, 0.0f)), ey = sqrtf(fmaxf(hy, 0.0f));
    bx0 = fminf(bx0, pxc - ex); bx1 = fmaxf(bx1, pxc + ex); by0 = fminf(by0, pyc - ey); by1 = fmaxf(by1, pyc + ey);
    const float mx = 0.05f + 1e-3f * (bx1 - bx0), my = 0.05f + 1e-3f * (by1 - by0);
    bx0 -= mx; bx1 += mx; by0 -= my; by1 += my;
    if (!(bx0 <= bx1 && by0 <= by1)) return 0xFu;
    const float ax = Tvy * Twz - Tvz * Twy, ay = Tvz * Twx - Tvx * Twz, az = Tvx * Twy - Tvy * Twx;
    const float bxx = Twy * Tuz - Twz * Tuy, bxy = Twz * Tux - Twx * Tuz, bxz = Twx * Tuy - Twy * Tux;
    const float A00 = ax * ax + ay * ay - tau * az * az, A11 = bxx * bxx + bxy * bxy - tau * bxz * bxz, A01 = ax * bxx + ay * bxy - tau * az * bxz;
    const float det = A00 * A11 - A01 * A01;
    const bool conic = A00 > 0.0f && A11 > 0.0f && det > 1e-6f * A00 * A11 && hx > 0.0f && hy > 0.0f &&
                       fabsf(hx * A00 - hy * A11) <= 0.02f * (hx * A00 + hy * A11);
    const float bound = conic ? 1.05f * hx * det / A11 : 0.0f;
    const float iA00 = conic ? 1.0f / A00 : 0.0f, iA11 = conic ? 1.0f / A11 : 0.0f;
    uint32_t m = 0;
#pragma unroll
    for (int q = 0; q < 4; q++) {
        const float qx = (float)(tile_px + (q & 1) * 8), qy = (float)(tile_py + (q >> 1) * 8);
        if (!(bx0 <= qx + 7.0f && bx1 >= qx && by0 <= qy + 7.0f && by1 >= qy)) continue;
        bool hit = true;
        if (conic) {
            const float ddx = fmaxf(fmaxf(qx - cx, cx - (qx + 7.0f)), 0.0f), ddy = fmaxf(fmaxf(qy - cy, cy - (qy + 7.0f)), 0.0f);
            const bool disc = ddx * ddx + ddy * ddy <= (r2d + 0.05f) * (r2d + 0.05f);
            const float x0 = qx - 0.05f - pxc, x1 = qx + 7.05f - pxc, y0 = qy - 0.05f - pyc, y1 = qy + 7.05f - pyc;
            bool ell = x0 <= 0.0f && x1 >= 0.0f && y0 <= 0.0f && y1 >= 0.0f;
            if (!ell) {
                float fmin = 3.0e38f;
#pragma unroll
                for (int e = 0; e < 2; e++) {
                    const float yy = e ? y1 : y0;
                    const float xs = fminf(fmaxf(-A01 * yy * iA00, x0), x1);
                    fmin = fminf(fmin, (A00 * xs + 2.0f * A01 * yy) * xs + A11 * yy * yy);
                    const float xx = e ? x1 : x0;
                    const float ys = fminf(fmaxf(-A01 * xx * iA11, y0), y1);
                    fmin = fminf(fmin, (A11 * ys + 2.0f * A01 * xx) * ys + A00 * xx * xx);
                }
                ell = fmin <= bound;
            }
            hit = disc || ell || !(bound == bound);
        }
        if (hit) m |= 1u << q;
    }
    return m;
}

template <int C, bool AUDIT, bool EXACT = false>
__global__ void __launch_bounds__(256, 5)
composite_fwd(int W, int H, int bg_len, const uint32_t *__restrict__ ranges, const uint32_t *__restrict__ point_list,
              const float *__restrict__ geom, const Feat colors, const float *__restrict__ bg,
              float *__restrict__ out_color, float *__restrict__ allmap, float *__restrict__ final_T,
              int32_t *__restrict__ n_contrib, float *__restrict__ weight, uint8_t *__restrict__ audit_contrib, int audit_lmax,
              uint8_t *__restrict__ contrib_mask, const uint8_t *__restrict__ audit_skip)
{
    __shared__ TileLds<C> lds;
    __shared__ float wacc[256];
    __shared__ unsigned char cmk[256][4];
    const int gx = (W + TILE - 1) / TILE, gy = (H + TILE - 1) / TILE;
    const int tile = xcd_tile(blockIdx.x, gx * gy);
    if (tile >= gx * gy) return;
    const int tx = tile % gx, ty = tile / gx;
    const int tid = threadIdx.x, wave = tid >> 6, lane = tid & 63;
    const int pxi = tx * TILE + (wave & 1) * 8 + (lane & 7);
    const int pyi = ty * TILE + (wave >> 1) * 8 + (lane >> 3);
    const bool inside = pxi < W && pyi < H;
    const float px = (float)pxi, py = (float)pyi;
    const uint32_t r0 = ranges[2 * tile], r1 = ranges[2 * tile + 1];

    const bool wskip = AUDIT && audit_skip && inside && audit_skip[(size_t)pyi * W + pxi] != 0;
    bool done = !inside;
    float T = 1.0f, Cacc[C], N0 = 0.f, N1 = 0.f, N2 = 0.f, D = 0.f, M1 = 0.f, M2 = 0.f, dist = 0.f, med = 0.f;
    int32_t last = 0, medc = -1;
#pragma unroll
    for (int c = 0; c < C; c++) Cacc[c] = 0.f;
    wacc[tid] = 0.f; reinterpret_cast<unsigned *>(&cmk[0][0])[tid] = 0u;

    for (uint32_t base = r0; base < r1; base += 256) {
        if (__syncthreads_and(done)) break;
        uint32_t qm = 0u;
        if (base + tid < r1) {
            const uint32_t g = point_list[base + tid];
            const float4 *gp = reinterpret_cast<const float4 *>(geom + (size_t)g * GEOM);
            const float4 a0 = gp[0], a1 = gp[1], a2 = gp[2], a3 = gp[3];
            lds.id[tid] = g;
            lds.rec[0][tid] = a0; lds.rec[1][tid] = a1; lds.rec[2][tid] = a2; lds.rec[3][tid] = a3;
            qm = quadrant_mask(a0, a1, a2, a3, tx * TILE, ty * TILE);
#pragma unroll
            for (int c = 0; c < C; c++) lds.col[c][tid] = colors[(size_t)g * C + c];
        }
#pragma unroll
        for (int q = 0; q < 4; q++) {
            const unsigned long long m = __builtin_amdgcn_ballot_w64((qm >> q) & 1u);
            if (lane == 0) lds.qbits[q][wave] = m;
        }
        __syncthreads();
        const int count = (int)min(256u, r1 - base);
        for (int ck = 0; ck * 64 < count && __builtin_amdgcn_ballot_w64(!done) != 0; ck++) {
          unsigned long long todo = lds.qbits[wave][ck];
          todo = ((unsigned long long)(unsigned)__builtin_amdgcn_readfirstlane((int)(todo >> 32)) << 32) | (unsigned)__builtin_amdgcn_readfirstlane((int)todo);
          while (todo != 0ull) {
            const int j = ck * 64 + (int)__builtin_ctzll(todo);
            todo &= todo - 1ull;
            if (__builtin_amdgcn_ballot_w64(!done) == 0) break;
            const Hit h = eval_splat<EXACT>(lds.rec[0][j], lds.rec[1][j], lds.rec[2][j], lds.rec[3][j], px, py);
            bool contrib = !done && h.ok;
            const float test_T = T * (1.0f - h.alpha);
            const bool stop = contrib && test_T < T_EPS;
            done = done || stop;
            contrib = contrib && !stop;
            float w = 0.f;
            if (contrib) {
                const float4 r2 = lds.rec[2][j], r3 = lds.rec[3][j];
                w = h.alpha * T;
                const float A = 1.0f - T;
                const float m = FAR_N / (FAR_N - NEAR_N) * (1.0f - NEAR_N / h.depth);
                dist += (m * m * A + M2 - 2.0f * m * M1) * w;
                D += h.depth * w;
                M1 += m * w;
                M2 += m * m * w;
                const int32_t contributor = (int32_t)(base - r0) + j + 1;
                if (AUDIT) { if (contributor <= audit_lmax) audit_contrib[((size_t)pyi * W + pxi) * (size_t)audit_lmax + (contributor - 1)] = 1; }
                if (T > 0.5f) { med = h.depth; medc = contributor; }
                N0 += r2.w * w; N1 += r3.x * w; N2 += r3.y * w;
#pragma unroll
                for (int c = 0; c < C; c++) Cacc[c] += lds.col[c][j] * w;
                T = test_T;
                last = contributor;
            }
            if (__builtin_amdgcn_ballot_w64(contrib) != 0) {
                const float ws = wave_sum((AUDIT && wskip) ? 0.f : w);
                if (lane == 0) { atomic_add_f32(&wacc[j], ws); cmk[j][wave] = 1; }
            }
          }
        }
        __syncthreads();
        if (tid < count) {
            const float ws = wacc[tid];
            if (ws != 0.0f) { atomic_add_f32(weight + lds.id[tid], ws); wacc[tid] = 0.f; }
            if (contrib_mask) {
                unsigned *cw = reinterpret_cast<unsigned *>(&cmk[0][0]) + tid;
                const unsigned v = *cw;
                contrib_mask[base + tid] = (uint8_t)((v & 1u) | ((v >> 7) & 2u) | ((v >> 14) & 4u) | ((v >> 21) & 8u));
                if (v) *cw = 0u;
            }
        }
    }

    if (inside) {
        const size_t HW = (size_t)H * W, pid = (size_t)pyi * W + pxi;
        final_T[pid] = T; final_T[HW + pid] = M1; final_T[2 * HW + pid] = M2;
        n_contrib[pid] = last; n_contrib[HW + pid] = medc;
#pragma unroll
        for (int c = 0; c < C; c++) out_color[c * HW + pid] = Cacc[c] + T * (c < bg_len ? bg[c] : 0.0f);
        allmap[0 * HW + pid] = D;
        allmap[1 * HW + pid] = 1.0f - T;
        allmap[2 * HW + pid] = N0; allmap[3 * HW + pid] = N1; allmap[4 * HW + pid] = N2;
        allmap[5 * HW + pid] = med;
        allmap[6 * HW + pid] = dist;
    }
}

template <int C, bool DIST, bool EXACT>
__device__ __forceinline__ void composite_bwd_tile(TileLds<C, BWD_BATCH> &lds, float (*gacc)[15 + C], const int W, const int H, const int bg_len,
                                                   const uint32_t *__restrict__ point_list, const float *__restrict__ geom,
                                                   const Feat colors, const float *__restrict__ bg,
                                                   const float *__restrict__ final_T, const int32_t *__restrict__ n_contrib,
                                                   const float *__restrict__ dL_dcolor, const float *__restrict__ dL_dallmap,
                                                   float *__restrict__ grad_rec, const uint32_t r0, const int tx, const int ty, const int max_last,
                                                   const uint8_t *__restrict__ contrib_mask)
{
    constexpr int V = 15 + C;
    constexpr int N4 = (V + 3) / 4;
    const int tid = threadIdx.x, wave = tid >> 6, lane = tid & 63;
    const int pxi = tx * TILE + (wave & 1) * 8 + (lane & 7);
    const int pyi = ty * TILE + (wave >> 1) * 8 + (lane >> 3);
    const bool inside = pxi < W && pyi < H;
    const float px = (float)pxi, py = (float)pyi;
    const size_t HW = (size_t)H * W, pid = (size_t)(inside ? pyi : 0) * W + (inside ? pxi : 0);

    const float T_final = inside ? final_T[pid] : 0.f;
    float T = T_final;
    const int32_t last = inside ? n_contrib[pid] : 0;
    const int32_t medc = inside ? n_contrib[HW + pid] : 0;
    float dpix[C];
    float bg_dot = 0.f;
#pragma unroll
    for (int c = 0; c < C; c++) {
        dpix[c] = (inside && dL_dcolor) ? dL_dcolor[c * HW + pid] : 0.f;
        bg_dot += (c < bg_len ? bg[c] : 0.0f) * dpix[c];
    }
    const float dL_ddepth = (inside && dL_dallmap) ? dL_dallmap[0 * HW + pid] : 0.f;
    const float dL_daccum = (inside && dL_dallmap) ? dL_dallmap[1 * HW + pid] : 0.f;
    const float dL_dn0 = (inside && dL_dallmap) ? dL_dallmap[2 * HW + pid] : 0.f;
    const float dL_dn1 = (inside && dL_dallmap) ? dL_dallmap[3 * HW + pid] : 0.f;
    const float dL_dn2 = (inside && dL_dallmap) ? dL_dallmap[4 * HW + pid] : 0.f;
    const float dL_dmed = (inside && dL_dallmap) ? dL_dallmap[5 * HW + pid] : 0.f;
    const float dL_dreg = (DIST && inside && dL_dallmap) ? dL_dallmap[6 * HW + pid] : 0.f;
    const float final_D = (DIST && inside) ? final_T[HW + pid] : 0.f;
    const float final_D2 = (DIST && inside) ? final_T[2 * HW + pid] : 0.f;
    const float final_A = 1.0f - T_final;
    const float bgT = -T_final * bg_dot;
    float last_alpha = 0.f, lastX = 0.f, accX = 0.f;
    int wmax_last = last;
    wmax_last = max(wmax_last, __shfl_xor(wmax_last, 1)); wmax_last = max(wmax_last, __shfl_xor(wmax_last, 2)); wmax_last = max(wmax_last, __shfl_xor(wmax_last, 4));
    wmax_last = max(wmax_last, __shfl_xor(wmax_last, 8)); wmax_last = max(wmax_last, __shfl_xor(wmax_last, 16)); wmax_last = max(wmax_last, __shfl_xor(wmax_last, 32));
    wmax_last = __builtin_amdgcn_readfirstlane(wmax_last);
    constexpr float MD_A = FAR_N / (FAR_N - NEAR_N), MD_B = (FAR_N * NEAR_N) / (FAR_N - NEAR_N);

    for (int top = max_last; top > 0; top -= BWD_BATCH) {
        __syncthreads();
        uint32_t qm = 0u;
        if (tid < BWD_BATCH && top - 1 - tid >= 0) {
            const uint32_t g = point_list[r0 + (uint32_t)(top - 1 - tid)];
            const float4 *gp = reinterpret_cast<const float4 *>(geom + (size_t)g * GEOM);
            const float4 a0 = gp[0], a1 = gp[1], a2 = gp[2], a3 = gp[3];
            lds.id[tid] = g;
            lds.rec[0][tid] = a0; lds.rec[1][tid] = a1; lds.rec[2][tid] = a2; lds.rec[3][tid] = a3;
            qm = contrib_mask ? (uint32_t)contrib_mask[r0 + (uint32_t)(top - 1 - tid)] : quadrant_mask(a0, a1, a2, a3, tx * TILE, ty * TILE);
#pragma unroll
            for (int c = 0; c < C; c++) lds.col[c][tid] = colors[(size_t)g * C + c];
        }
        if (wave * 64 < BWD_BATCH) {
#pragma unroll
            for (int q = 0; q < 4; q++) {
                const unsigned long long m = __builtin_amdgcn_ballot_w64((qm >> q) & 1u);
                if (lane == 0) lds.qbits[q][wave] = m;
            }
        }
        __syncthreads();
        const int count = min(BWD_BATCH, top);
        const int jmin = max(0, top - wmax_last);
        for (int ck = jmin >> 6; ck * 64 < count; ck++) {
          unsigned long long todo = lds.qbits[wave][ck];
          todo = ((unsigned long long)(unsigned)__builtin_amdgcn_readfirstlane((int)(todo >> 32)) << 32) | (unsigned)__builtin_amdgcn_readfirstlane((int)todo);
          if (ck == (jmin >> 6)) todo &= ~0ull << (jmin & 63);
          while (todo != 0ull) {
            const int j = ck * 64 + (int)__builtin_ctzll(todo);
            todo &= todo - 1ull;
            const int ci = top - 1 - j;
            const bool cand = ci < last;
            if (__builtin_amdgcn_ballot_w64(cand) == 0) continue;
            const float4 q0 = lds.rec[0][j], q1 = lds.rec[1][j], q2 = lds.rec[2][j], q3 = lds.rec[3][j];
            const Hit h = eval_splat<EXACT>(q0, q1, q2, q3, px, py);
            const bool act = cand && h.ok;
            if (__builtin_amdgcn_ballot_w64(act) == 0) continue;

            float gv[4 * N4];
#pragma unroll
            for (int v = 0; v < 4 * N4; v++) gv[v] = 0.f;
            if (act) {
                const float Twx = q1.z, Twy = q1.w, opa = q3.z;
                const float nrm0 = q2.w, nrm1 = q3.x, nrm2 = q3.y;
                const float alpha = h.alpha, G = h.G;
                const float r1 = recip1<EXACT>(1.0f - alpha);
                T = T * r1;
                const float w = alpha * T;
                float X = h.depth * dL_ddepth + dL_daccum;
                X += nrm0 * dL_dn0; X += nrm1 * dL_dn1; X += nrm2 * dL_dn2;
#pragma unroll
                for (int c = 0; c < C; c++) {
                    X += lds.col[c][j] * dpix[c];
                    gv[15 + c] = w * dpix[c];
                }
                float dL_dz = w * dL_ddepth;
                if (ci == medc - 1) dL_dz += dL_dmed;
                if (DIST) {
                    const float idep = recip1<EXACT>(h.depth);
                    const float m_d = MD_A * (1.0f - NEAR_N * idep);
                    X += (final_D2 + m_d * m_d * final_A - 2.0f * m_d * final_D) * dL_dreg;
                    dL_dz += 2.0f * w * (m_d * final_A - final_D) * dL_dreg * (MD_B * idep * idep);
                }
                accX = last_alpha * lastX + (1.f - last_alpha) * accX;
                lastX = X;
                last_alpha = alpha;
                const float dL_dalpha = (X - accX) * T + bgT * r1;
                gv[9] = w * dL_dn0; gv[10] = w * dL_dn1; gv[11] = w * dL_dn2;
                gv[12] = G * dL_dalpha;
                const float nGd = -(opa * dL_dalpha) * G;
                if (h.rho3d <= h.rho2d) {
                    const float dsx = __builtin_fmaf(nGd, h.sx, dL_dz * Twx);
                    const float dsy = __builtin_fmaf(nGd, h.sy, dL_dz * Twy);
                    const float dpx = dsx * h.inv, dpy = dsy * h.inv;
                    const float dpz = -__builtin_fmaf(dpx, h.sx, dpy * h.sy);
                    const float dkx = __builtin_fmaf(h.ly, dpz, -(h.lz * dpy)), dky = __builtin_fmaf(h.lz, dpx, -(h.lx * dpz)), dkz = __builtin_fmaf(h.lx, dpy, -(h.ly * dpx));
                    const float dlx = __builtin_fmaf(dpy, h.kz, -(dpz * h.ky)), dly = __builtin_fmaf(dpz, h.kx, -(dpx * h.kz)), dlz = __builtin_fmaf(dpx, h.ky, -(dpy * h.kx));
                    gv[0] = -dkx; gv[1] = -dky; gv[2] = -dkz;
                    gv[3] = -dlx; gv[4] = -dly; gv[5] = -dlz;
                    gv[6] = __builtin_fmaf(px, dkx, __builtin_fmaf(py, dlx, dL_dz * h.sx));
                    gv[7] = __builtin_fmaf(px, dky, __builtin_fmaf(py, dly, dL_dz * h.sy));
                    gv[8] = __builtin_fmaf(px, dkz, __builtin_fmaf(py, dlz, dL_dz));
                } else {
                    gv[13] = nGd * (FILTER_INV_SQ * h.dx);
                    gv[14] = nGd * (FILTER_INV_SQ * h.dy);
                    gv[8] = dL_dz;
                }
            }
            const float mine = wave_transpose_reduce<N4>(gv, lane);
            const int vi = (lane & 15) + (lane >> 4) * N4;
            if ((lane & 15) < N4 && vi < V) atomic_add_f32(&gacc[j][vi], mine);
          }
        }
        __syncthreads();
        for (int i = tid; i < count * V; i += 256) {
            const int j = i / V, v = i - j * V;
            const float val = gacc[j][v];
            if (val != 0.0f) { atomic_add_f32(grad_rec + (size_t)lds.id[j] * GREC + v, val); gacc[j][v] = 0.f; }
        }
    }
}

template <int C, bool EXACT = false>
__global__ void __launch_bounds__(256, 4)
composite_bwd(int W, int H, int bg_len, const uint32_t *__restrict__ ranges, const uint32_t *__restrict__ point_list,
              const float *__restrict__ geom, const Feat colors, const float *__restrict__ bg,
              const float *__restrict__ final_T, const int32_t *__restrict__ n_contrib,
              const float *__restrict__ dL_dcolor, const float *__restrict__ dL_dallmap, float *__restrict__ grad_rec,
              const uint8_t *__restrict__ contrib_mask)
{
    constexpr int V = 15 + C;
    __shared__ TileLds<C, BWD_BATCH> lds;
    __shared__ float gacc[BWD_BATCH][V];
    __shared__ int s_max_last, s_dist;
    const int gx = (W + TILE - 1) / TILE, gy = (H + TILE - 1) / TILE;
    const int tile = xcd_tile(blockIdx.x, gx * gy);
    if (tile >= gx * gy) return;
    const int tx = tile % gx, ty = tile / gx;
    const int tid = threadIdx.x, wave = tid >> 6, lane = tid & 63;
    const int pxi = tx * TILE + (wave & 1) * 8 + (lane & 7);
    const int pyi = ty * TILE + (wave >> 1) * 8 + (lane >> 3);
    const bool inside = pxi < W && pyi < H;
    const size_t HW = (size_t)H * W, pid = (size_t)(inside ? pyi : 0) * W + (inside ? pxi : 0);
    const int32_t last = inside ? n_contrib[pid] : 0;
    const bool reg = inside && dL_dallmap && dL_dallmap[6 * HW + pid] != 0.0f;

    if (tid == 0) { s_max_last = 0; s_dist = 0; }
    for (int i = tid; i < BWD_BATCH * V; i += 256) (&gacc[0][0])[i] = 0.f;
    __syncthreads();
    {
        int m = last;
        m = max(m, __shfl_xor(m, 1)); m = max(m, __shfl_xor(m, 2)); m = max(m, __shfl_xor(m, 4));
        m = max(m, __shfl_xor(m, 8)); m = max(m, __shfl_xor(m, 16)); m = max(m, __shfl_xor(m, 32));
        if (lane == 0) atomicMax(&s_max_last, m);
        const bool any_reg = __builtin_amdgcn_ballot_w64(reg) != 0;
        if (lane == 0 && any_reg) s_dist = 1;
    }
    __syncthreads();
    const int max_last = s_max_last;
    const uint32_t r0 = ranges[2 * tile];
    if (s_dist)
        composite_bwd_tile<C, true, EXACT>(lds, gacc, W, H, bg_len, point_list, geom, colors, bg, final_T, n_contrib, dL_dcolor, dL_dallmap, grad_rec, r0, tx, ty, max_last, contrib_mask);
    else
        composite_bwd_tile<C, false, EXACT>(lds, gacc, W, H, bg_len, point_list, geom, colors, bg, final_T, n_contrib, dL_dcolor, dL_dallmap, grad_rec, r0, tx, ty, max_last, contrib_mask);
}

template <int C>
static int run_fwd(const envgs_raster_cfg *cfg, const uint32_t *ranges, const uint32_t *point_list, const float *geom,
                   const float *colors, const float *bg, float *out_color, float *allmap, float *final_T,
                   int32_t *n_contrib, float *weight, uint8_t *audit_contrib, int audit_lmax, hipStream_t stream, int colors_f16, uint8_t *contrib_mask,
                   const uint8_t *audit_skip)
{
    const int gx = (cfg->width + TILE - 1) / TILE, gy = (cfg->height + TILE - 1) / TILE;
    ProfScope prof_(K_COMPOSITE_FWD, stream);
    const dim3 grid(8 * ((gx * gy + 7) / 8)), block(256);
    const Feat colors_{colors, colors_f16 != 0};
#ifdef ENVGS_DIAG
    if (debug_switch(ENVGS_DBG_RASTER_EXACT)) {
        if (audit_contrib)
            hipLaunchKernelGGL((composite_fwd<C, true, true>), grid, block, 0, stream, cfg->width, cfg->height, cfg->bg_len, ranges,
                               point_list, geom, colors_, bg, out_color, allmap, final_T, n_contrib, weight, audit_contrib, audit_lmax, contrib_mask, audit_skip);
        else
            hipLaunchKernelGGL((composite_fwd<C, false, true>), grid, block, 0, stream, cfg->width, cfg->height, cfg->bg_len, ranges,
                               point_list, geom, colors_, bg, out_color, allmap, final_T, n_contrib, weight, (uint8_t *)nullptr, 0, contrib_mask, (const uint8_t *)nullptr);
        ENVGS_CHECK_LAUNCH(cfg, stream);
        return 0;
    }
#endif
    if (audit_contrib)
        hipLaunchKernelGGL((composite_fwd<C, true>), grid, block, 0, stream, cfg->width, cfg->height, cfg->bg_len, ranges,
                           point_list, geom, colors_, bg, out_color, allmap, final_T, n_contrib, weight, audit_contrib, audit_lmax, contrib_mask, audit_skip);
    else
        hipLaunchKernelGGL((composite_fwd<C, false>), grid, block, 0, stream, cfg->width, cfg->height, cfg->bg_len, ranges,
                           point_list, geom, colors_, bg, out_color, allmap, final_T, n_contrib, weight, (uint8_t *)nullptr, 0, contrib_mask, (const uint8_t *)nullptr);
    ENVGS_CHECK_LAUNCH(cfg, stream);
    return 0;
}

int launch_render_fwd(const envgs_raster_cfg *cfg, const uint32_t *ranges, const uint32_t *point_list, const float *geom,
                      const float *colors, const float *bg, float *out_color, float *allmap, float *final_T,
                      int32_t *n_contrib, float *weight, hipStream_t stream, uint8_t *audit_contrib, int audit_lmax, int colors_f16, uint8_t *contrib_mask,
                      const uint8_t *audit_skip)
{
    if (cfg->P > 0) {
        hipError_t e = hipMemsetAsync(weight, 0, sizeof(float) * (size_t)cfg->P, stream);
        if (e != hipSuccess) return (int)e;
    }
    switch (cfg->channels) {
    case 3: return run_fwd<3>(cfg, ranges, point_list, geom, colors, bg, out_color, allmap, final_T, n_contrib, weight, audit_contrib, audit_lmax, stream, colors_f16, contrib_mask, audit_skip);
    case 5: return run_fwd<5>(cfg, ranges, point_list, geom, colors, bg, out_color, allmap, final_T, n_contrib, weight, audit_contrib, audit_lmax, stream, colors_f16, contrib_mask, audit_skip);
    case 7: return run_fwd<7>(cfg, ranges, point_list, geom, colors, bg, out_color, allmap, final_T, n_contrib, weight, audit_contrib, audit_lmax, stream, colors_f16, contrib_mask, audit_skip);
    default: return ENVGS_ERR_BAD_ARG;
    }
}

template <int C>
static int run_bwd(const envgs_raster_cfg *cfg, const uint32_t *ranges, const uint32_t *point_list, const float *geom,
                   const float *colors, const float *bg, const float *final_T, const int32_t *n_contrib,
                   const float *dL_dcolor, const float *dL_dallmap, float *grad_rec, hipStream_t stream, int colors_f16, const uint8_t *contrib_mask)
{
    const int gx = (cfg->width + TILE - 1) / TILE, gy = (cfg->height + TILE - 1) / TILE;
    ProfScope prof_(K_COMPOSITE_BWD, stream);
#ifdef ENVGS_DIAG
    if (debug_switch(ENVGS_DBG_RASTER_EXACT)) {
        hipLaunchKernelGGL((composite_bwd<C, true>), dim3(8 * ((gx * gy + 7) / 8)), dim3(256), 0, stream, cfg->width, cfg->height, cfg->bg_len, ranges,
                           point_list, geom, Feat{colors, colors_f16 != 0}, bg, final_T, n_contrib, dL_dcolor, dL_dallmap, grad_rec, contrib_mask);
        ENVGS_CHECK_LAUNCH(cfg, stream);
        return 0;
    }
#endif
    hipLaunchKernelGGL((composite_bwd<C, false>), dim3(8 * ((gx * gy + 7) / 8)), dim3(256), 0, stream, cfg->width, cfg->height, cfg->bg_len, ranges,
                       point_list, geom, Feat{colors, colors_f16 != 0}, bg, final_T, n_contrib, dL_dcolor, dL_dallmap, grad_rec, contrib_mask);
    ENVGS_CHECK_LAUNCH(cfg, stream);
    return 0;
}

int launch_render_bwd(const envgs_raster_cfg *cfg, const uint32_t *ranges, const uint32_t *point_list, const float *geom,
                      const float *colors, const float *bg, const float *final_T, const int32_t *n_contrib,
                      const float *dL_dcolor, const float *dL_dallmap, float *grad_rec, hipStream_t stream, int colors_f16, const uint8_t *contrib_mask)
{
    if (cfg->P <= 0) return 0;
    hipError_t e = hipMemsetAsync(grad_rec, 0, sizeof(float) * GREC * (size_t)cfg->P, stream);
    if (e != hipSuccess) return (int)e;
    switch (cfg->channels) {
    case 3: return run_bwd<3>(cfg, ranges, point_list, geom, colors, bg, final_T, n_contrib, dL_dcolor, dL_dallmap, grad_rec, stream, colors_f16, contrib_mask);
    case 5: return run_bwd<5>(cfg, ranges, point_list, geom, colors, bg, final_T, n_contrib, dL_dcolor, dL_dallmap, grad_rec, stream, colors_f16, contrib_mask);
    case 7: return run_bwd<7>(cfg, ranges, point_list, geom, colors, bg, final_T, n_contrib, dL_dcolor, dL_dallmap, grad_rec, stream, colors_f16, contrib_mask);
    default: return ENVGS_ERR_BAD_ARG;
    }
}

}
```

### envgs_amd/csrc/trace_common.h

```cpp
#ifndef ENVGS_TRACE_COMMON_H
#define ENVGS_TRACE_COMMON_H

#include "common.h"
#include "prof.h"
#include "sh_basis.h"

#include <cstdlib>
#include <cstring>

#include "../../include/envgs_trace.h"

namespace envgs {

constexpr int KBUF = 16;
constexpr int STACK = 64;
constexpr int NCOPY = 8;
constexpr int MAX_ROUNDS = 256;
constexpr float UV_MAX = 3.0f;
constexpr int MID = ENVGS_MID_CHANNELS;
constexpr int SREC = ENVGS_SREC_STRIDE;
constexpr int NODE = ENVGS_NODE_STRIDE;

struct SurfHit { float t, u, v, G, alpha, denom; bool ok; };

__device__ __forceinline__ SurfHit hit_surfel(const float4 s0, const float4 s1, const float4 s2, const float4 s3,
                                              const float ox, const float oy, const float oz, const float dx,
                                              const float dy, const float dz)
{
    SurfHit h;
    float qx, qy, qz;
    {
#pragma clang fp contract(off)
        h.denom = s3.x * dx + s3.y * dy + s3.z * dz;
        const float num = s3.x * (s0.x - ox) + s3.y * (s0.y - oy) + s3.z * (s0.z - oz);
        h.t = num / h.denom;
        qx = ox + h.t * dx - s0.x; qy = oy + h.t * dy - s0.y; qz = oz + h.t * dz - s0.z;
    }
    h.u = s1.x * qx + s1.y * qy + s1.z * qz;
    h.v = s2.x * qx + s2.y * qy + s2.z * qz;
    h.G = __expf(-0.5f * (h.u * h.u + h.v * h.v));
    const float a = s0.w * h.G;
    h.alpha = a < ALPHA_CAP ? a : ALPHA_CAP;
    h.ok = (h.denom != 0.0f) && (fabsf(h.u) <= UV_MAX) && (fabsf(h.v) <= UV_MAX) && (h.alpha >= ALPHA_MIN);
    return h;
}

__device__ __forceinline__ SurfHit hit_surfel_at(const float4 s0, const float4 s1, const float4 s2, const float4 s3, const float t,
                                                 const float ox, const float oy, const float oz, const float dx, const float dy, const float dz)
{
    SurfHit h;
    float qx, qy, qz;
    {
#pragma clang fp contract(off)
        h.denom = s3.x * dx + s3.y * dy + s3.z * dz;
        h.t = t;
        qx = ox + h.t * dx - s0.x; qy = oy + h.t * dy - s0.y; qz = oz + h.t * dz - s0.z;
    }
    h.u = s1.x * qx + s1.y * qy + s1.z * qz;
    h.v = s2.x * qx + s2.y * qy + s2.z * qz;
    h.G = __expf(-0.5f * (h.u * h.u + h.v * h.v));
    const float a = s0.w * h.G;
    h.alpha = a < ALPHA_CAP ? a : ALPHA_CAP;
    h.ok = true;
    return h;
}

__device__ __forceinline__ float first_tmin(int start_from_first) { return start_from_first == 1 ? NEAR_N : (start_from_first == 2 ? 1.0e-3f : 0.0f); }

struct TraceArgs {
    int P, R, D, M, ND, start_from_first, has_others, bg_len;
    int f16;
    float spec_thr;
    const float4 *nodes;
    const float4 *srec;
    const float *shs, *colors, *others, *bg;
    const float *ray_o, *ray_d;
    unsigned *counter;
    unsigned long long *stats;
    float *rgb, *dpt, *acc, *norm, *dist, *aux, *mid, *wet, *final_T;
    const float *f_rgb, *f_dpt, *f_acc, *f_norm, *f_aux, *f_T;
    const float *g_rgb, *g_dpt, *g_acc, *g_norm, *g_aux;
    float *geo_rec, *dshs, *dcolors, *dothers, *dray_o, *dray_d;
    float mod;
    uint2 *hits;
    int *hit_cnt;
    int *n_used;
    int cap;
    unsigned long long *surf_acc;
    int wfrac;
    unsigned *surf_cnt;
    const unsigned *surf_off;
    float *records;
    unsigned long long num_records;
    const unsigned *order;
    int exp;
    int only_overflow;
    int batch0, batch1;
    uint4 *sparse;
    unsigned sparse_cap;
    int sparse_max;
    int reduce_adds;
    int seg;
    unsigned long long *entries;
    unsigned *pairs;
    int *n_entries;
    unsigned *long_list;
    float4 *state;
    size_t state_plane;
    int colour_state;
    unsigned *batch_cnt;
    const unsigned *row_off;
    const uint2 *batch_rows;
    const void *shp;
    const unsigned *bwd_order;
};

struct KBuf {
    float t[KBUF];
    int id[KBUF];
    int n;
    __device__ __forceinline__ void reset() {
#pragma unroll
        for (int i = 0; i < KBUF; i++) { t[i] = 3.0e38f; id[i] = 0x7fffffff; }
        n = 0;
    }
    __device__ __forceinline__ void insert(float ct, int cid) {
#pragma unroll
        for (int i = 0; i < KBUF; i++) {
            const bool before = (ct < t[i]) || (ct == t[i] && cid < id[i]);
            const float tt = before ? t[i] : ct; const int ii = before ? id[i] : cid;
            t[i] = before ? ct : t[i]; id[i] = before ? cid : id[i];
            ct = tt; cid = ii;
        }
        n = n < KBUF ? n + 1 : KBUF;
    }
};

__device__ __forceinline__ void traverse(const TraceArgs &A, int (*stk)[64], const int lane, const bool active,
                                         const float ox, const float oy, const float oz, const float dx, const float dy,
                                         const float dz, const float tlo, const int idlo, KBuf &kb, unsigned &visits)
{
    kb.reset();
    const float ix = 1.0f / dx, iy = 1.0f / dy, iz = 1.0f / dz;
    int sp = 0;
    int cur = active ? 0 : -1;
    float tmax = 3.0e38f;
    while (true) {
        if (cur < 0) {
            if (sp == 0) break;
            cur = stk[--sp][lane];
        }
        const float4 *nd = A.nodes + (size_t)cur * 4;
        visits++;
        const float4 n0 = nd[0], n1 = nd[1], n2 = nd[2], n3 = nd[3];
        const int lc = __float_as_int(n3.x), rc = __float_as_int(n3.y);
        float a0 = (n0.x - ox) * ix, a1 = (n0.w - ox) * ix, b0 = (n0.y - oy) * iy, b1 = (n1.x - oy) * iy, c0 = (n0.z - oz) * iz, c1 = (n1.y - oz) * iz;
        float tnL = fmaxf(fmaxf(fminf(a0, a1), fminf(b0, b1)), fminf(c0, c1));
        float tfL = fminf(fminf(fmaxf(a0, a1), fmaxf(b0, b1)), fmaxf(c0, c1));
        a0 = (n1.z - ox) * ix; a1 = (n2.y - ox) * ix; b0 = (n1.w - oy) * iy; b1 = (n2.z - oy) * iy; c0 = (n2.x - oz) * iz; c1 = (n2.w - oz) * iz;
        float tnR = fmaxf(fmaxf(fminf(a0, a1), fminf(b0, b1)), fminf(c0, c1));
        float tfR = fminf(fminf(fmaxf(a0, a1), fmaxf(b0, b1)), fmaxf(c0, c1));
        bool hitL = (tnL <= tfL) && (tfL >= tlo) && (tnL <= tmax);
        bool hitR = (tnR <= tfR) && (tfR >= tlo) && (tnR <= tmax);
#pragma unroll
        for (int side = 0; side < 2; side++) {
            const bool hit = side == 0 ? hitL : hitR;
            const int ch = side == 0 ? lc : rc;
            if (hit && ch < 0) {
                const int sid = ~ch;
                const float4 *sr = A.srec + (size_t)sid * 4;
                const SurfHit h = hit_surfel(sr[0], sr[1], sr[2], sr[3], ox, oy, oz, dx, dy, dz);
                const bool after = (h.t > tlo) || (h.t == tlo && sid > idlo);
                const bool fits = (kb.n < KBUF) || (h.t < kb.t[KBUF - 1]) || (h.t == kb.t[KBUF - 1] && sid < kb.id[KBUF - 1]);
                if (h.ok && after && fits) {
                    kb.insert(h.t, sid);
                    if (kb.n == KBUF) tmax = kb.t[KBUF - 1];
                }
            }
        }
        hitL = hitL && lc >= 0;
        hitR = hitR && rc >= 0;
        if (hitL && hitR) {
            const bool leftFirst = tnL <= tnR;
            stk[sp++][lane] = leftFirst ? rc : lc;
            cur = leftFirst ? lc : rc;
        } else if (hitL) cur = lc;
        else if (hitR) cur = rc;
        else cur = -1;
    }
}

struct StageSums { float rgb[3], dpt, acc, nrm[3], dist, aux[2], T, M1, M2; };

__device__ __forceinline__ void unpack_h8(const uint4 x, float *v)
{
    const unsigned w[4] = {x.x, x.y, x.z, x.w};
#pragma unroll
    for (int q = 0; q < 4; q++) {
        v[2 * q] = __half2float(__ushort_as_half((unsigned short)(w[q] & 0xFFFFu)));
        v[2 * q + 1] = __half2float(__ushort_as_half((unsigned short)(w[q] >> 16)));
    }
}

__device__ __forceinline__ void load_sh(const TraceArgs &A, const int sid, const int nb, float *v)
{
    if (A.M == 16 && A.f16) {
        const uint4 *s8 = reinterpret_cast<const uint4 *>(reinterpret_cast<const __half *>(A.shs) + (size_t)sid * 48);
        const int nq = (nb * 3 + 7) >> 3;
#pragma unroll
        for (int q = 0; q < 6; q++) {
            uint4 x = make_uint4(0u, 0u, 0u, 0u);
            if (q < nq) x = s8[q];
            unpack_h8(x, v + 8 * q);
        }
#pragma unroll
        for (int k = 0; k < 48; k++) if (k >= nb * 3) v[k] = 0.f;
    } else if (A.M == 16) {
        const float4 *s4 = reinterpret_cast<const float4 *>(A.shs + (size_t)sid * 48);
        const int nq = (nb * 3 + 3) >> 2;
#pragma unroll
        for (int q = 0; q < 12; q++) {
            float4 x = make_float4(0.f, 0.f, 0.f, 0.f);
            if (q < nq) x = s4[q];
            v[4 * q] = x.x; v[4 * q + 1] = x.y; v[4 * q + 2] = x.z; v[4 * q + 3] = x.w;
        }
    } else {
        const Feat sh = Feat{A.shs, A.f16 != 0}.at((size_t)sid * A.M * 3);
#pragma unroll
        for (int k = 0; k < 16; k++) {
            const bool in = k < nb;
            v[k * 3] = in ? sh[k * 3] : 0.f; v[k * 3 + 1] = in ? sh[k * 3 + 1] : 0.f; v[k * 3 + 2] = in ? sh[k * 3 + 2] : 0.f;
        }
    }
}

__device__ __forceinline__ void sh_colour_clamped(const float *basis, const float *shv, const int nb, float *col, bool *cl)
{
    float r0 = 0.f, r1 = 0.f, r2 = 0.f;
#pragma unroll
    for (int k = 0; k < 16; k++)
        if (k < nb) { const float b = basis[k]; r0 += b * shv[k * 3]; r1 += b * shv[k * 3 + 1]; r2 += b * shv[k * 3 + 2]; }
    r0 += 0.5f; r1 += 0.5f; r2 += 0.5f;
    cl[0] = r0 < 0.f; cl[1] = r1 < 0.f; cl[2] = r2 < 0.f;
    col[0] = cl[0] ? 0.f : r0; col[1] = cl[1] ? 0.f : r1; col[2] = cl[2] ? 0.f : r2;
}

__device__ __forceinline__ void surfel_color(const TraceArgs &A, int sid, const float *basis, float *col, bool *cl)
{
    if (A.M > 0) {
        const int nb = (A.D + 1) * (A.D + 1);
        float v[48];
        load_sh(A, sid, nb, v);
        sh_colour_clamped(basis, v, nb, col, cl);
    } else {
        const Feat c = Feat{A.colors, A.f16 != 0}.at((size_t)sid * 3);
        col[0] = c[0]; col[1] = c[1]; col[2] = c[2];
        cl[0] = cl[1] = cl[2] = false;
    }
}

__device__ __forceinline__ int ray_index(int slot, int R, int rh, int rw)
{
    if (rh > 0 && (rh & 7) == 0 && (rw & 7) == 0) {
        const int blk = slot >> 6, in = slot & 63;
        const int bw = rw >> 3;
        const int by = blk / bw, bx = blk - by * bw;
        return (by * 8 + (in >> 3)) * rw + bx * 8 + (in & 7);
    }
    return slot;
}

static __device__ __constant__ float kShForm[16][11] = {
    {1, 0, 0, 0, kC0, 0, 0, 0, 0, 0, 0},
    {0, 0, 1, 0, -kC1, 0, 0, 0, 0, 0, 0},
    {0, 0, 0, 1, kC1, 0, 0, 0, 0, 0, 0},
    {0, 1, 0, 0, -kC1, 0, 0, 0, 0, 0, 0},
    {1, 0, 0, 0, 0, 0, 0, 0, kC2xy, 0, 0},
    {1, 0, 0, 0, 0, 0, 0, 0, 0, -kC2xy, 0},
    {1, 0, 0, 0, 0, -kC2zz, -kC2zz, 2.f * kC2zz, 0, 0, 0},
    {1, 0, 0, 0, 0, 0, 0, 0, 0, 0, -kC2xy},
    {1, 0, 0, 0, 0, kC2xx, -kC2xx, 0, 0, 0, 0},
    {0, 0, 1, 0, 0, 3.f * -kC3a, kC3a, 0, 0, 0, 0},
    {0, 0, 0, 1, 0, 0, 0, 0, kC3b, 0, 0},
    {0, 0, 1, 0, 0, kC3c, kC3c, 4.f * -kC3c, 0, 0, 0},
    {0, 0, 0, 1, 0, -3.f * kC3d, -3.f * kC3d, 2.f * kC3d, 0, 0, 0},
    {0, 1, 0, 0, 0, kC3c, kC3c, 4.f * -kC3c, 0, 0, 0},
    {0, 0, 0, 1, 0, kC3e, -kC3e, 0, 0, 0, 0},
    {0, 1, 0, 0, 0, -kC3a, 3.f * kC3a, 0, 0, 0, 0},
};

constexpr int NFLD = 22;
constexpr int GEO = ENVGS_GEOREC_STRIDE;

struct BwdRay {
    float ox, oy, oz, dx, dy, dz;
    float gR0, gR1, gR2, gD, gA, gN0, gN1, gN2, gX0, gX1;
    float fT, bgdot, fr0, fr1, fr2, fD, fA, fN0, fN1, fN2, fX0, fX1;
    float dl2, il, ux, uy, uz;
};
struct BwdAcc {
    float T, c0, c1, c2, cD, cA, cN0, cN1, cN2, cX0, cX1;
    float dO0, dO1, dO2, dD0, dD1, dD2;
    float Sk[16];
};

__device__ __forceinline__ void bwd_load_ray(const TraceArgs &A, int r, BwdRay &B)
{
    B.ox = A.ray_o[3 * r]; B.oy = A.ray_o[3 * r + 1]; B.oz = A.ray_o[3 * r + 2];
    B.dx = A.ray_d[3 * r]; B.dy = A.ray_d[3 * r + 1]; B.dz = A.ray_d[3 * r + 2];
    B.gR0 = B.gR1 = B.gR2 = B.gD = B.gA = B.gN0 = B.gN1 = B.gN2 = B.gX0 = B.gX1 = 0.f;
    if (A.g_rgb) { B.gR0 = A.g_rgb[3 * r]; B.gR1 = A.g_rgb[3 * r + 1]; B.gR2 = A.g_rgb[3 * r + 2]; }
    if (A.g_dpt) B.gD = A.g_dpt[r];
    if (A.g_acc) B.gA = A.g_acc[r];
    if (A.g_norm) { B.gN0 = A.g_norm[3 * r]; B.gN1 = A.g_norm[3 * r + 1]; B.gN2 = A.g_norm[3 * r + 2]; }
    if (A.g_aux) { B.gX0 = A.g_aux[2 * r]; B.gX1 = A.g_aux[2 * r + 1]; }
    B.fT = A.f_T[r];
    const float bg0 = 0 < A.bg_len ? A.bg[0] : 0.f, bg1 = 1 < A.bg_len ? A.bg[1] : 0.f, bg2 = 2 < A.bg_len ? A.bg[2] : 0.f;
    B.bgdot = bg0 * B.gR0 + bg1 * B.gR1 + bg2 * B.gR2;
    B.fr0 = A.f_rgb[3 * r] - B.fT * bg0; B.fr1 = A.f_rgb[3 * r + 1] - B.fT * bg1; B.fr2 = A.f_rgb[3 * r + 2] - B.fT * bg2;
    B.fD = A.f_dpt[r]; B.fA = A.f_acc[r];
    B.fN0 = A.f_norm[3 * r]; B.fN1 = A.f_norm[3 * r + 1]; B.fN2 = A.f_norm[3 * r + 2];
    B.fX0 = A.f_aux[2 * r]; B.fX1 = A.f_aux[2 * r + 1];
    B.dl2 = B.dx * B.dx + B.dy * B.dy + B.dz * B.dz; B.il = 1.0f / sqrtf(B.dl2);
    B.ux = B.dx * B.il; B.uy = B.dy * B.il; B.uz = B.dz * B.il;
}

__device__ __forceinline__ void bwd_init_acc(BwdAcc &a)
{
    a.T = 1.0f; a.c0 = a.c1 = a.c2 = a.cD = a.cA = a.cN0 = a.cN1 = a.cN2 = a.cX0 = a.cX1 = 0.f;
    a.dO0 = a.dO1 = a.dO2 = a.dD0 = a.dD1 = a.dD2 = 0.f;
#pragma unroll
    for (int k = 0; k < 16; k++) a.Sk[k] = 0.f;
}

__device__ __forceinline__ float bwd_final_dot(const BwdRay &B)
{
    return B.gR0 * B.fr0 + B.gR1 * B.fr1 + B.gR2 * B.fr2 + B.gD * B.fD + B.gA * B.fA + B.gN0 * B.fN0 + B.gN1 * B.fN1 + B.gN2 * B.fN2 +
           B.gX0 * B.fX0 + B.gX1 * B.fX1 + B.fT * B.bgdot;
}

__device__ __forceinline__ float alpha_grad_from_state(const bool colour_only, const float gR0, const float gR1, const float gR2, const float gD, const float gA,
                                                       const float gN0, const float gN1, const float gN2, const float gX0, const float gX1, const float Fsum,
                                                       const float *col, const float t, const float nf0, const float nf1, const float nf2, const float x0, const float x1,
                                                       const float alpha, const float inv1m, const float4 st0, const float4 st1, const float sx0, const float sx1)
{
    const float Tb = st0.x;
    float gv_ = gR0 * col[0] + gR1 * col[1] + gR2 * col[2], gS = gR0 * st0.y + gR1 * st0.z + gR2 * st0.w;
    if (!colour_only) {
        gv_ += gD * t + gA + gN0 * nf0 + gN1 * nf1 + gN2 * nf2 + gX0 * x0 + gX1 * x1;
        gS += gD * st1.x + gA * (1.0f - Tb * (1.0f - alpha)) + gN0 * st1.y + gN1 * st1.z + gN2 * st1.w + gX0 * sx0 + gX1 * sx1;
    }
    return Tb * gv_ - (Fsum - gS) * inv1m;
}

__device__ __forceinline__ void hit_geometry_grad(const float4 s0, const float4 s1, const float4 s2, const float4 s3, const SurfHit &h, const float ox, const float oy,
                                                  const float oz, const float dx, const float dy, const float dz, const float w, const float sgn, const float dLa,
                                                  const float gD, const float gN0, const float gN1, const float gN2, const float mod, const float isu, const float isv,
                                                  const float iden, float *gw, float &e0, float &e1, float &e2)
{
    const float dLG = s0.w * dLa;
    const float dLu = dLG * (-h.G * h.u), dLv = dLG * (-h.G * h.v);
    const float qx = ox + h.t * dx - s0.x, qy = oy + h.t * dy - s0.y, qz = oz + h.t * dz - s0.z;
    const float dq0 = dLu * s1.x + dLv * s2.x, dq1 = dLu * s1.y + dLv * s2.y, dq2 = dLu * s1.z + dLv * s2.z;
    const float cu = dLu * isu, cv = dLv * isv;
    const float dLt_tot = w * gD + dq0 * dx + dq1 * dy + dq2 * dz;
    const float kt = dLt_tot * iden;
    e0 = dq0 - kt * s3.x; e1 = dq1 - kt * s3.y; e2 = dq2 - kt * s3.z;
    gw[0] = -e0; gw[1] = -e1; gw[2] = -e2;
    gw[3] = cu * qx; gw[4] = cu * qy; gw[5] = cu * qz;
    gw[6] = cv * qx; gw[7] = cv * qy; gw[8] = cv * qz;
    const float ws = w * sgn;
    gw[9] = ws * gN0 - kt * qx; gw[10] = ws * gN1 - kt * qy; gw[11] = ws * gN2 - kt * qz;
    gw[12] = -cu * h.u * mod;
    gw[13] = -cv * h.v * mod;
    gw[14] = h.G * dLa;
}

__device__ __forceinline__ void ray_dir_grad(const BwdRay &B, const float dd0, const float dd1, const float dd2, float *out)
{
    const float inv3 = B.il * B.il * B.il;
    out[0] = ((B.dl2 - B.dx * B.dx) * dd0 - B.dy * B.dx * dd1 - B.dz * B.dx * dd2) * inv3;
    out[1] = (-B.dx * B.dy * dd0 + (B.dl2 - B.dy * B.dy) * dd1 - B.dz * B.dy * dd2) * inv3;
    out[2] = (-B.dx * B.dz * dd0 - B.dy * B.dz * dd1 + (B.dl2 - B.dz * B.dz) * dd2) * inv3;
}

__device__ __forceinline__ bool bwd_hit(const TraceArgs &A, const BwdRay &B, BwdAcc &a, const float *basis, const int nb,
                                        const int sid, float &dc0, float &dc1, float &dc2, float *gv)
{
    const float4 *sr = A.srec + (size_t)sid * 4;
    const float4 s0 = sr[0], s1 = sr[1], s2 = sr[2], s3 = sr[3];
    const SurfHit h = hit_surfel(s0, s1, s2, s3, B.ox, B.oy, B.oz, B.dx, B.dy, B.dz);
    const float alpha = h.alpha;
    const float test_T = a.T * (1.0f - alpha);
    if (test_T < T_EPS) return false;
    const float T = a.T;
    const float w = alpha * T;
    float col[3]; bool cl[3];
    float shv[48];
    if (A.M > 0) {
        load_sh(A, sid, nb, shv);
        sh_colour_clamped(basis, shv, nb, col, cl);
    } else surfel_color(A, sid, basis, col, cl);
    const float sgn = h.denom < 0.0f ? 1.0f : -1.0f;
    const float nf0 = sgn * s3.x, nf1 = sgn * s3.y, nf2 = sgn * s3.z;
    const float x0 = A.has_others ? A.others[2 * sid] : 0.f, x1 = A.has_others ? A.others[2 * sid + 1] : 0.f;
    a.c0 += w * col[0]; a.c1 += w * col[1]; a.c2 += w * col[2];
    a.cD += w * h.t; a.cA += w;
    a.cN0 += w * nf0; a.cN1 += w * nf1; a.cN2 += w * nf2;
    a.cX0 += w * x0; a.cX1 += w * x1;
    const float inv1m = 1.0f / (1.0f - alpha);
    float dLa = B.gR0 * (T * col[0] - (B.fr0 - a.c0) * inv1m) + B.gR1 * (T * col[1] - (B.fr1 - a.c1) * inv1m) + B.gR2 * (T * col[2] - (B.fr2 - a.c2) * inv1m);
    dLa += B.gD * (T * h.t - (B.fD - a.cD) * inv1m);
    dLa += B.gA * (T - (B.fA - a.cA) * inv1m);
    dLa += B.gN0 * (T * nf0 - (B.fN0 - a.cN0) * inv1m) + B.gN1 * (T * nf1 - (B.fN1 - a.cN1) * inv1m) + B.gN2 * (T * nf2 - (B.fN2 - a.cN2) * inv1m);
    dLa += B.gX0 * (T * x0 - (B.fX0 - a.cX0) * inv1m) + B.gX1 * (T * x1 - (B.fX1 - a.cX1) * inv1m);
    dLa += -(B.fT * inv1m) * B.bgdot;
    dc0 = cl[0] ? 0.f : w * B.gR0; dc1 = cl[1] ? 0.f : w * B.gR1; dc2 = cl[2] ? 0.f : w * B.gR2;
    if (A.M > 0) {
#pragma unroll
        for (int k = 0; k < 16; k++)
            if (k < nb) a.Sk[k] += shv[k * 3] * dc0 + shv[k * 3 + 1] * dc1 + shv[k * 3 + 2] * dc2;
    }
    if (A.has_others && A.dothers) { atomic_add_f32(A.dothers + 2 * sid, w * B.gX0); atomic_add_f32(A.dothers + 2 * sid + 1, w * B.gX1); }
    float e0, e1, e2;
    hit_geometry_grad(s0, s1, s2, s3, h, B.ox, B.oy, B.oz, B.dx, B.dy, B.dz, w, sgn, dLa, B.gD, B.gN0, B.gN1, B.gN2, A.mod,
                      1.0f / s1.w, 1.0f / s2.w, 1.0f / h.denom, gv, e0, e1, e2);
    a.dO0 += e0; a.dO1 += e1; a.dO2 += e2;
    a.dD0 += h.t * e0; a.dD1 += h.t * e1; a.dD2 += h.t * e2;
    a.T = test_T;
    return true;
}

struct FlushRole { float form[11]; int fc; bool sh_lane, geo_lane; };

__device__ __forceinline__ FlushRole flush_role(const TraceArgs &A, int lane)
{
    FlushRole R;
    const int fk = lane / 3;
    R.fc = lane - 3 * fk;
#pragma unroll
    for (int i = 0; i < 11; i++) R.form[i] = kShForm[fk < 16 ? fk : 0][i];
    const int nb = (A.D + 1) * (A.D + 1);
    R.sh_lane = A.M > 0 ? (lane < 48 && fk < nb) : (lane < 3);
    R.geo_lane = lane >= 48 && lane < 48 + 15;
    return R;
}

__device__ __forceinline__ void flush_hits(const TraceArgs &A, float (*fld)[65], const int lane, const FlushRole &R,
                                           const bool has, const int sid, const float dc0, const float dc1, const float dc2, const float *gv)
{
    const unsigned long long hm = __builtin_amdgcn_ballot_w64(has);
    if (hm == 0) return;
    fld[0][lane] = __int_as_float(sid); fld[1][lane] = dc0; fld[2][lane] = dc1; fld[3][lane] = dc2;
#pragma unroll
    for (int k = 0; k < 15; k++) fld[4 + k][lane] = gv[k];
    __syncthreads();
    unsigned long long m = hm;
    while (m) {
        const int l = __builtin_ctzll(m);
        m &= m - 1;
        const int hs = __float_as_int(fld[0][l]);
        float val = 0.f; float *dst = nullptr;
        if (A.M > 0) {
            const float x = fld[19][l], y = fld[20][l], z = fld[21][l];
            const float lin = R.form[0] + R.form[1] * x + R.form[2] * y + R.form[3] * z;
            const float quad = R.form[4] + R.form[5] * (x * x) + R.form[6] * (y * y) + R.form[7] * (z * z) + R.form[8] * (x * y) + R.form[9] * (y * z) + R.form[10] * (x * z);
            const float dcc = R.fc == 0 ? fld[1][l] : (R.fc == 1 ? fld[2][l] : fld[3][l]);
            val = lin * quad * dcc;
            dst = A.dshs + (size_t)hs * A.M * 3 + lane;
        } else {
            val = fld[1 + (lane < 3 ? lane : 0)][l];
            dst = A.dcolors + (size_t)hs * 3 + lane;
        }
        if (R.geo_lane) { val = fld[4 + (lane - 48)][l]; dst = A.geo_rec + (size_t)hs * GEO + (lane - 48); }
        if (R.sh_lane || R.geo_lane) atomic_add_f32(dst, val);
    }
    __syncthreads();
}

__device__ __forceinline__ void bwd_store_ray(const TraceArgs &A, int r, const BwdRay &B, const BwdAcc &a)
{
    float dd0 = 0.f, dd1 = 0.f, dd2 = 0.f;
    if (A.M > 0) {
        float bgx[16], bgy[16], bgz[16];
        basis16_grad_contracted(A.D, B.ux, B.uy, B.uz, bgx, bgy, bgz);
#pragma unroll
        for (int k = 0; k < 16; k++) { dd0 += bgx[k] * a.Sk[k]; dd1 += bgy[k] * a.Sk[k]; dd2 += bgz[k] * a.Sk[k]; }
    }
    float e[3];
    ray_dir_grad(B, dd0, dd1, dd2, e);
    A.dray_o[3 * r] = a.dO0; A.dray_o[3 * r + 1] = a.dO1; A.dray_o[3 * r + 2] = a.dO2;
    A.dray_d[3 * r] = a.dD0 + e[0]; A.dray_d[3 * r + 1] = a.dD1 + e[1]; A.dray_d[3 * r + 2] = a.dD2 + e[2];
}

__device__ __forceinline__ int ray_of(const TraceArgs &A, int slot) { return slot < A.R ? (A.order ? (int)A.order[slot] : slot) : A.R; }


__device__ __forceinline__ int xcd_block(int b, int nblocks) { return (b & 7) * (nblocks >> 3) + (b >> 3); }

__device__ __forceinline__ int xcc_id()
{
    unsigned v;
    asm volatile("s_getreg_b32 %0, hwreg(HW_REG_XCC_ID)" : "=s"(v));
    return (int)(v & 7u);
}

__device__ __forceinline__ int fetch_batch(unsigned *ctr , int nbatch, int home, int lane)
{
    const int per = (nbatch + 7) >> 3;
    int b = -1;
    if (lane == 0) {
        for (int k = 0; k < 8 && b < 0; k++) {
            const int x = (home + k) & 7;
            const int lo = x * per, hi = min(lo + per, nbatch);
            if (lo >= hi) continue;
            const int i = (int)atomicAdd(ctr + x, 1u);
            if (lo + i < hi) b = lo + i;
        }
    }
    return __builtin_amdgcn_readfirstlane(b);
}

__device__ __forceinline__ size_t state_row0(const TraceArgs &A, const int slot, const int r)
{
    return A.row_off ? (size_t)A.row_off[slot] : (size_t)r * A.cap;
}
__device__ __forceinline__ char *state_row1(const TraceArgs &A, const size_t i)
{
    return reinterpret_cast<char *>(A.state + A.state_plane) + i * (A.has_others ? (size_t)24 : (size_t)16);
}
__device__ __forceinline__ void batch_region(const TraceArgs &A, const int batch, size_t &start, size_t &size)
{
    if (A.batch_rows) { const uint2 br = A.batch_rows[batch]; start = br.x; size = br.y; }
    else { size = (size_t)64 * A.cap; start = (size_t)batch * size; }
}

constexpr float KILL_OD = 9.2104f * 1.03f + 0.05f;

constexpr int WIDE_EMPTY = ENVGS_WIDE_EMPTY;
constexpr int SORT_MAX = 1024;
constexpr int RH_W = 8;

#ifndef ENVGS_BSB_WAVES
#define ENVGS_BSB_WAVES 2
#endif
struct ForwardPrepare {
    ZeroBatch zero; int zero_blocks;
    int P, rec_blocks; float mod; const float *means, *scales, *rots, *opac; float *srec;
    int perm_blocks, nb, f16; const void *shs; void *shp;
};
__global__ void __launch_bounds__(256) forward_prepare(const ForwardPrepare F);
__global__ void __launch_bounds__(64) trace_fwd(const TraceArgs A, const int ray_h, const int ray_w);
__global__ void __launch_bounds__(64) trace_bwd(const TraceArgs A, const int ray_h, const int ray_w);
__global__ void __launch_bounds__(256, 8)
collect_hits_coop(const TraceArgs A, const float4 *__restrict__ nodes, const float4 *__restrict__ nodes4, const float4 *__restrict__ srec);

template <int EMAX, bool LONG, bool QSH> __global__ void __launch_bounds__(256) sort_composite_fwd(const TraceArgs A);
extern template __global__ void __launch_bounds__(256) sort_composite_fwd<4, false, false>(const TraceArgs A);
extern template __global__ void __launch_bounds__(256) sort_composite_fwd<8, true, false>(const TraceArgs A);
extern template __global__ void __launch_bounds__(256) sort_composite_fwd<16, true, false>(const TraceArgs A);
extern template __global__ void __launch_bounds__(256) sort_composite_fwd<4, false, true>(const TraceArgs A);
extern template __global__ void __launch_bounds__(256) sort_composite_fwd<8, true, true>(const TraceArgs A);
extern template __global__ void __launch_bounds__(256) sort_composite_fwd<16, true, true>(const TraceArgs A);
template <bool CACHED> __global__ void __launch_bounds__(64 * RH_W) register_hits(const TraceArgs A);
__global__ void __launch_bounds__(256) row_scan_blocks(unsigned *__restrict__ blk, int n, unsigned *rows_used, unsigned *seg_base);
__global__ void __launch_bounds__(256) row_offsets(const TraceArgs A, const unsigned *__restrict__ blk, unsigned *__restrict__ row_off, uint2 *__restrict__ batch_rows,
                                                   const unsigned *__restrict__ seg_base, unsigned long long limit);
__global__ void __launch_bounds__(256) unpack_surfel_acc(int P, int wfrac, const unsigned long long *__restrict__ acc, unsigned *__restrict__ cnt,
                                                         float *__restrict__ wet, unsigned *ray_counter, const int *__restrict__ n_entries, int nbatch,
                                                         unsigned *__restrict__ bwd_order, int order_classes);
__global__ void __launch_bounds__(256) sparse_hits_bwd(const TraceArgs A, const int rgbo);
template <bool RGBO, bool OTH> __global__ void __attribute__((amdgpu_waves_per_eu(ENVGS_BSB_WAVES, ENVGS_BSB_WAVES))) __launch_bounds__(64) batch_surfel_bwd(const TraceArgs A);
extern template __global__ void __attribute__((amdgpu_waves_per_eu(ENVGS_BSB_WAVES, ENVGS_BSB_WAVES))) __launch_bounds__(64) batch_surfel_bwd<false, false>(const TraceArgs A);
extern template __global__ void __attribute__((amdgpu_waves_per_eu(ENVGS_BSB_WAVES, ENVGS_BSB_WAVES))) __launch_bounds__(64) batch_surfel_bwd<false, true>(const TraceArgs A);
extern template __global__ void __attribute__((amdgpu_waves_per_eu(ENVGS_BSB_WAVES, ENVGS_BSB_WAVES))) __launch_bounds__(64) batch_surfel_bwd<true, false>(const TraceArgs A);
__global__ void __launch_bounds__(256) reduce_surfel_records(const TraceArgs A);
__global__ void __launch_bounds__(256) finish_surfel_grads(int P, const float *__restrict__ rots, const float *__restrict__ geo_rec,
                                                           float *__restrict__ dmeans, float *__restrict__ dscales, float *__restrict__ dopac,
                                                           float *__restrict__ drots, float *__restrict__ dgrads3D);

}
#endif
```

### envgs_amd/raster.py

```python
from typing import NamedTuple

import torch
from torch import nn

from . import _lib


LAST_STATS = {}


class GaussianRasterizationSettings(NamedTuple):
    image_height: int
    image_width: int
    tanfovx: float
    tanfovy: float
    bg: torch.Tensor
    scale_modifier: float
    viewmatrix: torch.Tensor
    projmatrix: torch.Tensor
    sh_degree: int
    campos: torch.Tensor
    prefiltered: bool
    debug: bool


def _f32c(t):
    if t is None:
        return None
    if t.dtype != torch.float32:
        t = t.float()
    return t.contiguous()


def _featc(t):
    if t is None:
        return None
    if t.dtype != torch.float16:
        return _f32c(t)
    return t.contiguous()


def _stream(dev):
    return _lib.c_void_p(torch.cuda.current_stream(dev).cuda_stream)


import weakref

_DEG_CACHE = {}


def sh_degree_of(deg):
    if not torch.is_tensor(deg):
        return int(deg)
    key = id(deg)
    hit = _DEG_CACHE.get(key)
    if hit is not None and hit[0]() is deg and hit[1] == deg._version:
        return hit[2]
    v = int(deg.reshape(-1)[0].item())
    if len(_DEG_CACHE) > 64:
        for k in [k for k, h in _DEG_CACHE.items() if h[0]() is None]:
            del _DEG_CACHE[k]
    _DEG_CACHE[key] = (weakref.ref(deg), deg._version, v)
    return v


SPECULATIVE_N = {"on": True}
_N_GUESS = {}
_N_MIRROR = {}


def _n_mirror(dev):
    m = _N_MIRROR.get(dev.index)
    if m is None:
        m = _N_MIRROR[dev.index] = dict(host=torch.empty(1, dtype=torch.int32).pin_memory(), event=torch.cuda.Event())
    return m


FEATURE_STORAGE = {"f16": False}


def _store(t):
    if t is not None and FEATURE_STORAGE["f16"] and t.dtype == torch.float32 and t.numel() > 0:
        return t.detach().half()
    return t


CONTRIB_MASK = {"on": True}


def _cfg(settings, P, C, sh_coeffs, bg_len, f16=False):
    deg = sh_degree_of(settings.sh_degree)
    return _lib.RasterCfg(P, deg, sh_coeffs, C, int(settings.image_width), int(settings.image_height), bg_len,
                          1 if settings.debug else 0, float(settings.scale_modifier), float(settings.tanfovx),
                          float(settings.tanfovy), 1 if f16 else 0)


def rasterize_forward(C, means3D, shs, colors_precomp, opacities, scales, rotations, cov3D_precomp, settings,
                      keep_binning=False):
    lib = _lib.load()
    dev = means3D.device
    if dev.type != "cuda":
        raise RuntimeError("envgs_amd rasterizer needs tensors on the GPU (got %s); there is no CPU path" % dev)
    P = means3D.shape[0]
    H, W = int(settings.image_height), int(settings.image_width)
    means3D = _f32c(means3D); opacities = _f32c(opacities)
    shs = _featc(shs); colors_precomp = _featc(colors_precomp)
    f16 = any(t is not None and t.dtype == torch.float16 for t in (shs, colors_precomp))
    scales = _f32c(scales); rotations = _f32c(rotations); cov3D_precomp = _f32c(cov3D_precomp)
    if shs is not None and C != 3:
        raise RuntimeError("in-kernel SH evaluation produces 3 channels; the %d-channel rasterizer needs colors_precomp" % C)
    if colors_precomp is not None and colors_precomp.shape[-1] != C:
        raise RuntimeError("colors_precomp has %d channels, this rasterizer composites %d" % (colors_precomp.shape[-1], C))
    bg = _f32c(settings.bg).reshape(-1).to(dev)
    view = _f32c(settings.viewmatrix).to(dev); proj = _f32c(settings.projmatrix).to(dev)
    campos = _f32c(settings.campos).reshape(-1).to(dev)
    sh_coeffs = 0 if shs is None else int(shs.shape[1])
    cfg = _cfg(settings, P, C, sh_coeffs, min(int(bg.numel()), C), f16)
    stream = _stream(dev)
    f32 = dict(dtype=torch.float32, device=dev)
    i32 = dict(dtype=torch.int32, device=dev)

    geom = torch.empty(P, 16, **f32)
    radii = torch.empty(P, **i32)
    tiles = torch.empty(P, **i32)
    offsets = torch.empty(P, **i32)
    rgb = torch.empty(P, 3, **f32) if shs is not None else None
    clamped = torch.empty(P, 3, dtype=torch.uint8, device=dev) if shs is not None else None
    scan_bytes = lib.envgs_raster_scan_temp_bytes(P)
    scan_temp = torch.empty(max(scan_bytes, 1), dtype=torch.uint8, device=dev)
    p = _lib.ptr
    tiles_n = ((W + 15) // 16) * ((H + 15) // 16)
    colors = rgb if shs is not None else colors_precomp
    out_color = torch.empty(C, H, W, **f32)
    allmap = torch.empty(7, H, W, **f32)
    final_T = torch.empty(3, H, W, **f32)
    n_contrib = torch.empty(2, H, W, **i32)
    weight = torch.empty(P, 1, **f32)
    ranges = torch.empty(tiles_n, 2, **i32)

    def bin_and_render(cap):
        pairs = torch.empty(max(cap, 1), dtype=torch.int64, device=dev)
        keys_s = torch.empty(max(cap, 1), dtype=torch.int64, device=dev) if keep_binning else None
        point_list = torch.empty(max(cap, 1), **i32)
        bin_bytes = lib.envgs_raster_sort_temp_bytes(max(cap, 1), W, H)
        bin_temp = torch.empty(max(bin_bytes, 1), dtype=torch.uint8, device=dev)
        cmask = torch.empty(max(cap, 1), dtype=torch.uint8, device=dev) if CONTRIB_MASK["on"] else None
        _lib.check(lib.envgs_raster_bin_and_render(cfg, cap, p(geom), p(radii), p(colors), p(bg), p(pairs), p(keys_s), p(point_list),
                                                   p(bin_temp), bin_bytes, p(ranges), p(out_color), p(allmap), p(final_T),
                                                   p(n_contrib), p(weight), p(cmask), stream),
                   "envgs_raster_bin_and_render")
        return pairs, keys_s, point_list, cmask

    key = (dev.index, P, H, W)
    guess = _N_GUESS.get(key) if SPECULATIVE_N["on"] else None
    mirror = _n_mirror(dev)
    if guess is None or P == 0:
        n_host = _lib.c_uint32(0)
        _lib.check(lib.envgs_raster_project(cfg, p(means3D), p(scales), p(rotations), p(opacities), p(shs), p(cov3D_precomp),
                                            p(view), p(proj), p(campos), p(geom), p(rgb), p(clamped), p(radii), p(tiles),
                                            p(offsets), p(scan_temp), scan_bytes, n_host, stream), "envgs_raster_project")
        N = int(n_host.value)
        bufs = bin_and_render(N)
    else:
        _lib.check(lib.envgs_raster_project(cfg, p(means3D), p(scales), p(rotations), p(opacities), p(shs), p(cov3D_precomp),
                                            p(view), p(proj), p(campos), p(geom), p(rgb), p(clamped), p(radii), p(tiles),
                                            p(offsets), p(scan_temp), scan_bytes, None, stream), "envgs_raster_project")
        mirror["host"].copy_(offsets[P - 1:P], non_blocking=True)
        mirror["event"].record(torch.cuda.current_stream(dev))
        cap = guess
        bufs = bin_and_render(cap)
        mirror["event"].synchronize()
        N = int(mirror["host"][0]) & 0xFFFFFFFF
        if N > cap:
            LAST_STATS["n_guess_misses"] = LAST_STATS.get("n_guess_misses", 0) + 1
            bufs = bin_and_render(N)
    pairs, keys_s, point_list, cmask = bufs
    _N_GUESS[key] = max(((max(int(N * 1.15), N + 4096) + 65535) // 65536) * 65536, int(0.97 * (guess or 0)))
    LAST_STATS.update(N=N, P=P, H=H, W=W, C=C)
    saved = dict(cfg=cfg, N=N, geom=geom, colors=colors, bg=bg, point_list=point_list, ranges=ranges, final_T=final_T,
                 n_contrib=n_contrib, contrib_mask=cmask, means3D=means3D, scales=scales, rotations=rotations, shs=shs, clamped=clamped,
                 cov3D_precomp=cov3D_precomp, radii=radii, view=view, proj=proj, campos=campos)
    if keep_binning:
        saved.update(tiles_touched=tiles, offsets=offsets, tile_pairs=pairs, keys_sorted=keys_s)
    return (out_color, radii, allmap, weight), saved


def render_audit(saved, lmax, skip_px=None, want_weight=False):
    lib = _lib.load()
    cfg = saved["cfg"]
    dev = saved["geom"].device
    H, W, C, P = cfg.height, cfg.width, cfg.channels, cfg.P
    f32 = dict(dtype=torch.float32, device=dev)
    out_color = torch.empty(C, H, W, **f32); allmap = torch.empty(7, H, W, **f32); final_T = torch.empty(3, H, W, **f32)
    n_contrib = torch.empty(2, H, W, dtype=torch.int32, device=dev); weight = torch.empty(max(P, 1), **f32)
    contrib = torch.empty(H * W, int(lmax), dtype=torch.uint8, device=dev)
    skip = None if skip_px is None else skip_px.to(device=dev, dtype=torch.uint8).reshape(-1).contiguous()
    if skip is not None and skip.numel() != H * W:
        raise RuntimeError("skip_px must have H*W elements")
    p = _lib.ptr
    _lib.check(lib.envgs_raster_render_audit(cfg, p(saved["geom"]), p(saved["colors"]), p(saved["bg"]), p(saved["point_list"]),
                                             p(saved["ranges"]), p(out_color), p(allmap), p(final_T), p(n_contrib), p(weight),
                                             p(contrib), int(lmax), p(skip), _stream(dev)), "envgs_raster_render_audit")
    if want_weight:
        return contrib, n_contrib, out_color, weight[:P]
    return contrib, n_contrib, out_color


def rasterize_backward(saved, dL_dcolor, dL_dallmap):
    lib = _lib.load()
    cfg = saved["cfg"]
    P, C = cfg.P, cfg.channels
    dev = saved["geom"].device
    f32 = dict(dtype=torch.float32, device=dev)
    dL_dcolor = _f32c(dL_dcolor); dL_dallmap = _f32c(dL_dallmap)
    shs, cov = saved["shs"], saved["cov3D_precomp"]
    grad_rec = torch.empty(P, 32, **f32)
    dmeans3D = torch.empty(P, 3, **f32)
    dmeans2D = torch.empty(P, 3, **f32)
    dopac = torch.empty(P, 1, **f32)
    dscales = torch.empty(P, 2, **f32) if cov is None else None
    drots = torch.empty(P, 4, **f32) if cov is None else None
    dcov = torch.empty(P, 9, **f32) if cov is not None else None
    dshs = torch.empty(shs.shape, **f32) if shs is not None else None
    dcolors = torch.empty(P, C, **f32) if shs is None else None
    p = _lib.ptr
    _lib.check(lib.envgs_raster_backward(cfg, saved["N"], p(saved["geom"]), p(saved["colors"]), p(saved["bg"]),
                                         p(saved["point_list"]), p(saved["ranges"]), p(saved["final_T"]), p(saved["n_contrib"]),
                                         p(saved.get("contrib_mask")), p(dL_dcolor), p(dL_dallmap), p(saved["means3D"]), p(saved["scales"]), p(saved["rotations"]),
                                         p(shs), p(saved["clamped"]), p(cov), p(saved["radii"]), p(saved["view"]), p(saved["proj"]),
                                         p(saved["campos"]), p(grad_rec), p(dmeans3D), p(dmeans2D), p(dscales), p(drots), p(dshs),
                                         p(dcolors), p(dopac), p(dcov), _stream(dev)), "envgs_raster_backward")
    return dict(means3D=dmeans3D, means2D=dmeans2D, shs=dshs, colors_precomp=dcolors, opacities=dopac, scales=dscales,
                rotations=drots, cov3D_precomp=dcov, grad_rec=grad_rec)


def make_package(C):

    class _RasterizeGaussians(torch.autograd.Function):
        @staticmethod
        def forward(ctx, means3D, means2D, sh, colors_precomp, opacities, scales, rotations, cov3Ds_precomp, raster_settings):
            ctx.set_materialize_grads(False)
            none = lambda t: None if (t is None or t.numel() == 0) else t
            outs, saved = rasterize_forward(C, means3D, _store(none(sh)), _store(none(colors_precomp)), opacities, none(scales),
                                            none(rotations), none(cov3Ds_precomp), raster_settings)
            ctx.saved = saved
            ctx.in_dtypes = tuple(None if t is None else t.dtype for t in (means3D, means2D, sh, colors_precomp, opacities, scales, rotations, cov3Ds_precomp))
            color, radii, allmap, weight = outs
            ctx.mark_non_differentiable(radii, weight)
            return color, radii, allmap, weight

        @staticmethod
        def backward(ctx, grad_color, grad_radii, grad_allmap, grad_weight):
            saved = ctx.saved
            cfg = saved["cfg"]
            dev = saved["geom"].device
            g = rasterize_backward(saved, grad_color, grad_allmap)
            outs = (g["means3D"] if saved["cov3D_precomp"] is None or saved["shs"] is not None else None, g["means2D"],
                    g["shs"], g["colors_precomp"], g["opacities"], g["scales"], g["rotations"], g["cov3D_precomp"])
            outs = tuple(None if (o is None or dt is None) else o.to(dt) for o, dt in zip(outs, ctx.in_dtypes))
            return outs + (None,)

    class GaussianRasterizer(nn.Module):
        def __init__(self, raster_settings):
            super().__init__()
            self.raster_settings = raster_settings

        def markVisible(self, positions):
            with torch.no_grad():
                V = self.raster_settings.viewmatrix.to(positions.device).float()
                z = positions.float() @ V[:3, 2] + V[3, 2]
                return z > 0.2

        def forward(self, means3D, means2D, opacities, shs=None, colors_precomp=None, scales=None, rotations=None,
                    cov3D_precomp=None):
            rs = self.raster_settings
            if (shs is None and colors_precomp is None) or (shs is not None and colors_precomp is not None):
                raise Exception('Please provide excatly one of either SHs or precomputed colors!')
            if ((scales is None or rotations is None) and cov3D_precomp is None) or \
               ((scales is not None or rotations is not None) and cov3D_precomp is not None):
                raise Exception('Please provide exactly one of either scale/rotation pair or precomputed 3D covariance!')
            e = torch.Tensor([])
            return _RasterizeGaussians.apply(means3D, means2D, e if shs is None else shs,
                                             e if colors_precomp is None else colors_precomp, opacities,
                                             e if scales is None else scales, e if rotations is None else rotations,
                                             e if cov3D_precomp is None else cov3D_precomp, rs)

    GaussianRasterizer.channels = C
    GaussianRasterizer._function = _RasterizeGaussians
    return GaussianRasterizationSettings, GaussianRasterizer
```

### include/envgs_raster.h

```cpp
#ifndef ENVGS_RASTER_H
#define ENVGS_RASTER_H

#include <stddef.h>
#include <stdint.h>

#ifdef __cplusplus
extern "C" {
#endif

#if defined(__GNUC__)
#define ENVGS_API __attribute__((visibility("default")))
#else
#define ENVGS_API
#endif

#define ENVGS_TILE 16
#define ENVGS_GEOM_STRIDE 16
#define ENVGS_GRAD_STRIDE 32

typedef enum envgs_status {
    ENVGS_OK = 0,
    ENVGS_ERR_BAD_ARG = -1,
    ENVGS_ERR_TEMP_TOO_SMALL = -2
} envgs_status;

typedef struct envgs_raster_cfg {
    int32_t P;
    int32_t sh_degree;
    int32_t sh_coeffs;
    int32_t channels;
    int32_t width, height;
    int32_t bg_len;
    int32_t debug;
    float scale_modifier;
    float tanfovx, tanfovy;
    int32_t feature_f16;
} envgs_raster_cfg;

ENVGS_API size_t envgs_raster_scan_temp_bytes(int32_t P);
ENVGS_API size_t envgs_raster_sort_temp_bytes(uint32_t N, int32_t width, int32_t height);

ENVGS_API int envgs_raster_project(const envgs_raster_cfg *cfg,
                         const float *means3D, const float *scales, const float *rotations,
                         const float *opacities, const float *shs, const float *transmat_precomp,
                         const float *viewmatrix, const float *projmatrix, const float *campos,
                         float *geom, float *rgb, uint8_t *clamped, int32_t *radii,
                         uint32_t *tiles_touched, uint32_t *offsets,
                         void *scan_temp, size_t scan_temp_bytes,
                         uint32_t *num_rendered_host, void *stream);

ENVGS_API int envgs_raster_bin_and_render(const envgs_raster_cfg *cfg, uint32_t N,
                                const float *geom, const int32_t *radii,
                                const float *colors, const float *bg,
                                uint64_t *tile_pairs, uint64_t *keys_sorted , uint32_t *point_list,
                                void *bin_temp, size_t bin_temp_bytes, uint32_t *ranges,
                                float *out_color, float *allmap, float *final_T, int32_t *n_contrib,
                                float *weight, uint8_t *contrib_mask, void *stream);

ENVGS_API int envgs_raster_render_audit(const envgs_raster_cfg *cfg, const float *geom, const float *colors, const float *bg,
                              const uint32_t *point_list, const uint32_t *ranges,
                              float *out_color, float *allmap, float *final_T, int32_t *n_contrib, float *weight,
                              uint8_t *contrib, int32_t lmax, const uint8_t *skip_px, void *stream);

ENVGS_API int envgs_raster_backward(const envgs_raster_cfg *cfg, uint32_t N,
                          const float *geom, const float *colors, const float *bg,
                          const uint32_t *point_list, const uint32_t *ranges,
                          const float *final_T, const int32_t *n_contrib, const uint8_t *contrib_mask ,
                          const float *dL_dcolor, const float *dL_dallmap,
                          const float *means3D, const float *scales, const float *rotations,
                          const float *shs, const uint8_t *clamped, const float *transmat_precomp,
                          const int32_t *radii,
                          const float *viewmatrix, const float *projmatrix, const float *campos,
                          float *grad_rec,
                          float *dmeans3D, float *dmeans2D, float *dscales, float *drots,
                          float *dshs, float *dcolors, float *dopacities, float *dtransmat_precomp,
                          void *stream);

ENVGS_API void envgs_prof_enable(int on);
ENVGS_API void envgs_prof_select(uint64_t kernel_mask);
ENVGS_API int envgs_prof_read(int kernel_id, double *total_ms, int *launches);
ENVGS_API const char *envgs_prof_kernel_name(int kernel_id);

#define ENVGS_DBG_TRACE 0
#define ENVGS_DBG_TRACE_NO_SORT 64
#define ENVGS_DBG_TRACE_SMALL_STACK 1024
#define ENVGS_DBG_TRACE_PREPARE_INLINE 16384
#define ENVGS_DBG_TRACE_RETIRED (8 | 16 | 512 | 2048 | 4096 | 8192)
#define ENVGS_DBG_SEGMENTS 1
#define ENVGS_DBG_COLLECT_WGS 2
#define ENVGS_DBG_RASTER_EXACT 3
#define ENVGS_DBG_RAYKEY 4
#define ENVGS_DBG_SPARSE 5
#define ENVGS_DBG_BALANCE 6
#define ENVGS_DBG_COUNT 7
ENVGS_API void envgs_debug_set(int32_t which, int32_t value);
ENVGS_API int32_t envgs_debug_get(int32_t which);

#ifdef __cplusplus
}
#endif
#endif
```

Measured before the change: 146.7.

## Add cost-sorted persistent tile queues for raster forward and backward

```diff
diff --git a/envgs_amd/_lib.py b/envgs_amd/_lib.py
--- a/envgs_amd/_lib.py
+++ b/envgs_amd/_lib.py
@@ -115,6 +115,9 @@
     "envgs_raster_sort_temp_bytes": (c_size_t, [c_uint32, ctypes.c_int32, ctypes.c_int32]),
     "envgs_raster_project": (c_int, [ctypes.POINTER(RasterCfg)] + [_P] * 15 + [_P, c_size_t, ctypes.POINTER(c_uint32), _P]),
     "envgs_raster_bin_and_render": (c_int, [ctypes.POINTER(RasterCfg), c_uint32] + [_P] * 7 + [_P, c_size_t] + [_P] * 7 + [_P]),
+    "envgs_raster_tile_queue_bytes": (c_size_t, [ctypes.c_int32, ctypes.c_int32]),
+    "envgs_raster_bin_and_render_queued": (c_int, [ctypes.POINTER(RasterCfg), c_uint32] + [_P] * 7 + [_P, c_size_t] + [_P] * 8 + [_P]),
+    "envgs_raster_backward_queued": (c_int, [ctypes.POINTER(RasterCfg), c_uint32] + [_P] * 30 + [_P]),
     "envgs_raster_render_audit": (c_int, [ctypes.POINTER(RasterCfg)] + [_P] * 11 + [ctypes.c_int32, _P, _P]),
     "envgs_raster_backward": (c_int, [ctypes.POINTER(RasterCfg), c_uint32] + [_P] * 29 + [_P]),
     "envgs_bvh_temp_bytes": (c_size_t, [ctypes.c_int32]),
diff --git a/envgs_amd/csrc/common.h b/envgs_amd/csrc/common.h
--- a/envgs_amd/csrc/common.h
+++ b/envgs_amd/csrc/common.h
@@ -159,6 +159,119 @@
 
 __device__ __forceinline__ void atomic_add_f32(float *p, float v) { unsafeAtomicAdd(p, v); }
 
+__device__ __forceinline__ int xcc_id()
+{
+    unsigned v;
+    asm volatile("s_getreg_b32 %0, hwreg(HW_REG_XCC_ID)" : "=s"(v));
+    return (int)(v & 7u);
+}
+
+constexpr int TQ_CLASSES = 32;
+constexpr int TQ_HEAD_STRIDE = 32;
+constexpr int TQ_HEADS = 8 * TQ_HEAD_STRIDE;
+struct TileQueue {
+    uint32_t *heads6, *heads7, *order6, *order7, *tile_cost;
+};
+__host__ __device__ inline size_t tile_queue_words(int ntiles) { return 2 * (size_t)TQ_HEADS + 3 * (size_t)ntiles; }
+inline TileQueue tile_queue_of(uint32_t *block, int ntiles)
+{
+    return TileQueue{block, block + TQ_HEADS, block + 2 * TQ_HEADS, block + 2 * TQ_HEADS + ntiles, block + 2 * TQ_HEADS + 2 * (size_t)ntiles};
+}
+constexpr uint32_t TQ_COST_MAX = (1u << 27) - 1u;
+__host__ __device__ inline int tile_cost_class(uint32_t cost, uint32_t max_cost)
+{
+    return (int)((cost * (uint32_t)TQ_CLASSES) / (max_cost + 1u));
+}
+
+constexpr int TQ_STAGE = 8192;
+struct TileOrderLds {
+    uint32_t hist[8 * TQ_CLASSES];
+    uint32_t base[8 * TQ_CLASSES];
+    uint32_t max_cost;
+    uint32_t cls[TQ_STAGE];
+};
+__device__ __forceinline__ void build_tile_order(const uint32_t *hi, const uint32_t *lo, const int stride, const int ntiles, const bool one_queue,
+                                                 uint32_t *__restrict__ order, uint32_t *__restrict__ heads, TileOrderLds &S)
+{
+    const int tid = threadIdx.x, lane = tid & 63, wave = tid >> 6, nthreads = blockDim.x, nw = nthreads >> 6;
+    if (tid < 8) heads[tid * TQ_HEAD_STRIDE] = 0u;
+    if (ntiles > TQ_STAGE || !hi) {
+        for (int t = tid; t < ntiles; t += nthreads) order[t] = (uint32_t)t;
+        return;
+    }
+    for (int i = tid; i < 8 * TQ_CLASSES; i += nthreads) S.hist[i] = 0u;
+    if (tid == 0) S.max_cost = 0u;
+    __syncthreads();
+    uint32_t m = 0u;
+#pragma nounroll
+    for (int t = tid; t < ntiles; t += nthreads) {
+        uint32_t c = hi[(size_t)t * stride];
+        if (lo) c -= lo[(size_t)t * stride];
+        c = min(c, TQ_COST_MAX);
+        S.cls[t] = c;
+        m = max(m, c);
+    }
+#pragma nounroll
+    for (int d = 1; d < 64; d <<= 1) m = max(m, (uint32_t)__shfl_xor((int)m, d));
+    if (lane == 0) atomicMax(&S.max_cost, m);
+    __syncthreads();
+    const uint32_t max_cost = S.max_cost;
+    const int per = (ntiles + 7) >> 3;
+#pragma nounroll
+    for (int t = tid; t < ntiles; t += nthreads) {
+        const int k = tile_cost_class(S.cls[t], max_cost);
+        S.cls[t] = (uint32_t)k;
+        atomicAdd(&S.hist[(t / per) * TQ_CLASSES + k], 1u);
+    }
+    __syncthreads();
+    static_assert(TQ_CLASSES == 32, "five class bits");
+    const unsigned long long lanes_before = (1ull << lane) - 1ull;
+#pragma nounroll
+    for (int row = wave; row < 8; row += nw) {
+        const int first = row * per, cnt = max(0, min(per, ntiles - first));
+        if (cnt == 0) continue;
+        uint32_t heavier = 0u, base = one_queue ? 0u : (uint32_t)first;
+        if (lane < TQ_CLASSES) {
+            if (one_queue) {
+#pragma nounroll
+                for (int x = 0; x < 8; x++) {
+                    const uint32_t h = S.hist[x * TQ_CLASSES + lane];
+                    heavier += h;
+                    base += x < row ? h : 0u;
+                }
+            } else {
+                heavier = S.hist[row * TQ_CLASSES + lane];
+            }
+        }
+#pragma nounroll
+        for (int k = 1; k < TQ_CLASSES; k++) {
+            const uint32_t h = (uint32_t)__builtin_amdgcn_readlane((int)heavier, k);
+            base += k > lane ? h : 0u;
+        }
+        uint32_t *bases = S.base + row * TQ_CLASSES;
+        if (lane < TQ_CLASSES) __hip_atomic_store(&bases[lane], base, __ATOMIC_RELAXED, __HIP_MEMORY_SCOPE_WORKGROUP);
+#pragma nounroll
+        for (int start = 0; start < cnt; start += 64) {
+            const int i = start + lane;
+            const bool valid = i < cnt;
+            const uint32_t c = valid ? S.cls[first + i] : 0u;
+            unsigned long long same = __builtin_amdgcn_ballot_w64(valid);
+#pragma unroll
+            for (int bit = 0; bit < 5; bit++) {
+                const bool on = (c >> bit) & 1u;
+                const unsigned long long b = __builtin_amdgcn_ballot_w64(on);
+                same &= on ? b : ~b;
+            }
+            if (valid) {
+                const uint32_t rank = (uint32_t)__builtin_popcountll(same & lanes_before);
+                const uint32_t b0 = __hip_atomic_load(&bases[c], __ATOMIC_RELAXED, __HIP_MEMORY_SCOPE_WORKGROUP);
+                order[b0 + rank] = (uint32_t)(first + i);
+                if (rank == 0u) __hip_atomic_store(&bases[c], b0 + (uint32_t)__builtin_popcountll(same), __ATOMIC_RELAXED, __HIP_MEMORY_SCOPE_WORKGROUP);
+            }
+        }
+    }
+}
+
 int launch_project(const envgs_raster_cfg *cfg, const float *means3D, const float *scales, const float *rotations,
                    const float *opacities, const float *shs, const float *transmat_precomp, const float *viewmatrix,
                    const float *projmatrix, const float *campos, float *geom, float *rgb, uint8_t *clamped,
@@ -167,7 +280,10 @@
 size_t scan_temp_bytes(int n);
 size_t sort_temp_bytes(uint32_t n, int width, int height);
 int launch_bin(const envgs_raster_cfg *cfg, uint32_t N, const float *geom, const int32_t *radii, uint64_t *tile_pairs,
-               uint64_t *keys_sorted, uint32_t *point_list, void *bin_temp, size_t bin_temp_bytes, uint32_t *ranges, hipStream_t stream);
+               uint64_t *keys_sorted, uint32_t *point_list, void *bin_temp, size_t bin_temp_bytes, uint32_t *ranges, hipStream_t stream,
+               uint32_t *tile_queue = nullptr);
+void launch_tile_order(int ntiles, const uint32_t *hi, const uint32_t *lo, int stride, uint32_t *order, uint32_t *heads, hipStream_t stream);
+inline bool tile_one_queue() { return (debug_switch(ENVGS_DBG_BALANCE) & 4) == 0; }
 size_t key_sort_temp_bytes(int n);
 int launch_key_sort(int n, const uint64_t *keys_in, uint64_t *keys_out, int top_bit, void *temp, size_t temp_bytes, hipStream_t stream);
 size_t ray_sort_temp_bytes(int R);
@@ -176,11 +292,11 @@
 int launch_render_fwd(const envgs_raster_cfg *cfg, const uint32_t *ranges, const uint32_t *point_list, const float *geom,
                       const float *colors, const float *bg, float *out_color, float *allmap, float *final_T,
                       int32_t *n_contrib, float *weight, hipStream_t stream, uint8_t *audit_contrib = nullptr, int audit_lmax = 0, int colors_f16 = 0,
-                      uint8_t *contrib_mask = nullptr, const uint8_t *audit_skip = nullptr);
+                      uint8_t *contrib_mask = nullptr, const uint8_t *audit_skip = nullptr, uint32_t *tile_queue = nullptr);
 int launch_render_bwd(const envgs_raster_cfg *cfg, const uint32_t *ranges, const uint32_t *point_list, const float *geom,
                       const float *colors, const float *bg, const float *final_T, const int32_t *n_contrib,
                       const float *dL_dcolor, const float *dL_dallmap, float *grad_rec, hipStream_t stream, int colors_f16 = 0,
-                      const uint8_t *contrib_mask = nullptr);
+                      const uint8_t *contrib_mask = nullptr, uint32_t *tile_queue = nullptr);
 int launch_project_bwd(const envgs_raster_cfg *cfg, const float *geom, const float *means3D, const float *scales,
                        const float *rotations, const float *shs, const uint8_t *clamped, const float *transmat_precomp,
                        const int32_t *radii, const float *viewmatrix, const float *projmatrix, const float *campos,
diff --git a/envgs_amd/csrc/raster_api.hip b/envgs_amd/csrc/raster_api.hip
--- a/envgs_amd/csrc/raster_api.hip
+++ b/envgs_amd/csrc/raster_api.hip
@@ -47,10 +47,25 @@
     return (int)e;
 }
 
+size_t envgs_raster_tile_queue_bytes(int32_t width, int32_t height)
+{
+    if (width <= 0 || height <= 0) return 0;
+    return sizeof(uint32_t) * tile_queue_words(((width + TILE - 1) / TILE) * ((height + TILE - 1) / TILE));
+}
+
 int envgs_raster_bin_and_render(const envgs_raster_cfg *cfg, uint32_t N, const float *geom, const int32_t *radii,
                                 const float *colors, const float *bg, uint64_t *tile_pairs, uint64_t *keys_sorted, uint32_t *point_list,
                                 void *bin_temp, size_t bin_temp_bytes_, uint32_t *ranges, float *out_color, float *allmap,
                                 float *final_T, int32_t *n_contrib, float *weight, uint8_t *contrib_mask, void *stream_)
+{
+    return envgs_raster_bin_and_render_queued(cfg, N, geom, radii, colors, bg, tile_pairs, keys_sorted, point_list, bin_temp, bin_temp_bytes_, ranges,
+                                              out_color, allmap, final_T, n_contrib, weight, contrib_mask, nullptr, stream_);
+}
+
+int envgs_raster_bin_and_render_queued(const envgs_raster_cfg *cfg, uint32_t N, const float *geom, const int32_t *radii,
+                                       const float *colors, const float *bg, uint64_t *tile_pairs, uint64_t *keys_sorted, uint32_t *point_list,
+                                       void *bin_temp, size_t bin_temp_bytes_, uint32_t *ranges, float *out_color, float *allmap,
+                                       float *final_T, int32_t *n_contrib, float *weight, uint8_t *contrib_mask, uint32_t *tile_queue, void *stream_)
 {
     int rc = check_cfg(cfg);
     if (rc) return rc;
@@ -58,10 +73,11 @@
     if (cfg->P > 0 && (!geom || !radii || !colors || !weight)) return ENVGS_ERR_BAD_ARG;
     if (N > 0 && (!tile_pairs || !point_list || !bin_temp)) return ENVGS_ERR_BAD_ARG;
     hipStream_t stream = (hipStream_t)stream_;
-    rc = launch_bin(cfg, N, geom, radii, tile_pairs, keys_sorted, point_list, bin_temp, bin_temp_bytes_, ranges, stream);
+    if (tile_queue && (reinterpret_cast<size_t>(tile_queue) & 127)) return ENVGS_ERR_BAD_ARG;
+    rc = launch_bin(cfg, N, geom, radii, tile_pairs, keys_sorted, point_list, bin_temp, bin_temp_bytes_, ranges, stream, tile_queue);
     if (rc) return rc;
     return launch_render_fwd(cfg, ranges, point_list, geom, colors, bg, out_color, allmap, final_T, n_contrib, weight, stream, nullptr, 0,
-                             (cfg->feature_f16 && cfg->sh_coeffs == 0) ? 1 : 0, contrib_mask);
+                             (cfg->feature_f16 && cfg->sh_coeffs == 0) ? 1 : 0, contrib_mask, nullptr, tile_queue);
 }
 
 int envgs_raster_render_audit(const envgs_raster_cfg *cfg, const float *geom, const float *colors, const float *bg,
@@ -88,6 +104,20 @@
                           float *dscales, float *drots, float *dshs, float *dcolors, float *dopacities,
                           float *dtransmat_precomp, void *stream_)
 {
+    return envgs_raster_backward_queued(cfg, N, geom, colors, bg, point_list, ranges, final_T, n_contrib, contrib_mask, dL_dcolor, dL_dallmap, means3D,
+                                        scales, rotations, shs, clamped, transmat_precomp, radii, viewmatrix, projmatrix, campos, grad_rec, dmeans3D,
+                                        dmeans2D, dscales, drots, dshs, dcolors, dopacities, dtransmat_precomp, nullptr, stream_);
+}
+
+int envgs_raster_backward_queued(const envgs_raster_cfg *cfg, uint32_t N, const float *geom, const float *colors, const float *bg,
+                                 const uint32_t *point_list, const uint32_t *ranges, const float *final_T,
+                                 const int32_t *n_contrib, const uint8_t *contrib_mask, const float *dL_dcolor, const float *dL_dallmap, const float *means3D,
+                                 const float *scales, const float *rotations, const float *shs, const uint8_t *clamped,
+                                 const float *transmat_precomp, const int32_t *radii, const float *viewmatrix,
+                                 const float *projmatrix, const float *campos, float *grad_rec, float *dmeans3D, float *dmeans2D,
+                                 float *dscales, float *drots, float *dshs, float *dcolors, float *dopacities,
+                                 float *dtransmat_precomp, uint32_t *tile_queue, void *stream_)
+{
     int rc = check_cfg(cfg);
     if (rc) return rc;
     if (cfg->P == 0) return 0;
@@ -99,7 +129,7 @@
     if (transmat_precomp ? !dtransmat_precomp : (!scales || !rotations || !means3D || !dmeans3D || !dscales || !drots)) return ENVGS_ERR_BAD_ARG;
     hipStream_t stream = (hipStream_t)stream_;
     rc = launch_render_bwd(cfg, ranges, point_list, geom, colors, bg, final_T, n_contrib, dL_dcolor, dL_dallmap, grad_rec, stream,
-                           (cfg->feature_f16 && !shs) ? 1 : 0, contrib_mask);
+                           (cfg->feature_f16 && !shs) ? 1 : 0, contrib_mask, tile_queue);
     if (rc) return rc;
     return launch_project_bwd(cfg, geom, means3D, scales, rotations, shs, clamped, transmat_precomp, radii, viewmatrix,
                               projmatrix, campos, grad_rec, dmeans3D, dmeans2D, dscales, drots, dshs, dcolors, dopacities,
diff --git a/envgs_amd/csrc/raster_bin.hip b/envgs_amd/csrc/raster_bin.hip
--- a/envgs_amd/csrc/raster_bin.hip
+++ b/envgs_amd/csrc/raster_bin.hip
@@ -185,9 +185,10 @@
 
 __global__ void __launch_bounds__(1024)
 bin_tile_scan(int ntiles, const uint32_t *__restrict__ tile_count, uint32_t *__restrict__ tile_start, uint32_t *__restrict__ ranges,
-              uint32_t cap, uint32_t *__restrict__ hdr)
+              uint32_t cap, uint32_t *__restrict__ hdr, uint32_t *__restrict__ order = nullptr, uint32_t *__restrict__ heads = nullptr, int one_queue = 0)
 {
     __shared__ uint32_t s_w[17];
+    __shared__ TileOrderLds s_order;
     const int per = (ntiles + 1023) / 1024, b = min(ntiles, (int)threadIdx.x * per), e = min(ntiles, b + per);
     uint32_t s = 0;
     for (int k = b; k < e; k++) s += tile_count[k];
@@ -202,6 +203,20 @@
         run += c;
     }
     if (threadIdx.x == 0) { tile_start[ntiles] = total; hdr[0] = total; hdr[1] = 0u; hdr[2] = 0u; hdr[3] = 0u; }
+    if (order) build_tile_order(ok ? tile_count : nullptr, nullptr, 1, ntiles, one_queue != 0, order, heads, s_order);
+}
+
+__global__ void __launch_bounds__(512)
+tile_order_kernel(int ntiles, const uint32_t *__restrict__ hi, const uint32_t *__restrict__ lo, int stride, int one_queue,
+                  uint32_t *__restrict__ order, uint32_t *__restrict__ heads)
+{
+    __shared__ TileOrderLds s_order;
+    build_tile_order(hi, lo, stride, ntiles, one_queue != 0, order, heads, s_order);
+}
+
+void launch_tile_order(int ntiles, const uint32_t *hi, const uint32_t *lo, int stride, uint32_t *order, uint32_t *heads, hipStream_t stream)
+{
+    hipLaunchKernelGGL(tile_order_kernel, dim3(1), dim3(512), 0, stream, ntiles, hi, lo, stride, tile_one_queue() ? 1 : 0, order, heads);
 }
 
 template <int NT>
@@ -403,10 +418,15 @@
 }
 
 int launch_bin(const envgs_raster_cfg *cfg, uint32_t N, const float *geom, const int32_t *radii, uint64_t *tile_pairs,
-               uint64_t *keys_sorted, uint32_t *point_list, void *bin_temp, size_t bin_temp_bytes, uint32_t *ranges, hipStream_t stream)
+               uint64_t *keys_sorted, uint32_t *point_list, void *bin_temp, size_t bin_temp_bytes, uint32_t *ranges, hipStream_t stream,
+               uint32_t *tile_queue)
 {
     const BinPlan pl = bin_plan(cfg->P, cfg->width, cfg->height);
-    if (N == 0 || cfg->P <= 0) return (int)hipMemsetAsync(ranges, 0, sizeof(uint32_t) * 2 * (size_t)pl.ntiles, stream);
+    const TileQueue tq = tile_queue_of(tile_queue, pl.ntiles);
+    if (N == 0 || cfg->P <= 0) {
+        if (tile_queue) { launch_tile_order(pl.ntiles, nullptr, nullptr, 1, tq.order6, tq.heads6, stream); ENVGS_CHECK_LAUNCH(cfg, stream); }
+        return (int)hipMemsetAsync(ranges, 0, sizeof(uint32_t) * 2 * (size_t)pl.ntiles, stream);
+    }
     if (bin_temp_bytes < sort_temp_bytes(N, cfg->width, cfg->height)) return ENVGS_ERR_TEMP_TOO_SMALL;
     uint32_t *hist = (uint32_t *)bin_temp;
     uint32_t *tile_count = hist + (size_t)BIN_ROWS_MAX * pl.ntiles;
@@ -420,7 +440,8 @@
     ENVGS_CHECK_LAUNCH(cfg, stream);
     hipLaunchKernelGGL(bin_column_scan, dim3((pl.ntiles + 15) / 16), dim3(256), 0, stream, pl.rows, pl.ntiles, hist, tile_count);
     ENVGS_CHECK_LAUNCH(cfg, stream);
-    hipLaunchKernelGGL(bin_tile_scan, dim3(1), dim3(1024), 0, stream, pl.ntiles, tile_count, tile_start, ranges, N, hdr);
+    hipLaunchKernelGGL(bin_tile_scan, dim3(1), dim3(1024), 0, stream, pl.ntiles, tile_count, tile_start, ranges, N, hdr,
+                       tile_queue ? tq.order6 : nullptr, tile_queue ? tq.heads6 : nullptr, tile_one_queue() ? 1 : 0);
     ENVGS_CHECK_LAUNCH(cfg, stream);
     hipLaunchKernelGGL(bin_pass<true>, dim3(pl.rows), dim3(256), lds, stream, cfg->P, cfg->width, cfg->height, pl.slice, pl.ntiles,
                        geom, radii, hist, tile_start, tile_pairs, N);
@@ -556,7 +577,7 @@
     hipLaunchKernelGGL(ray_bucket_pass<false>, dim3(rows), dim3(256), lds, stream, R, slice, nb, shift, ray_o, ray_d, (const float *)partial, rows, lead, keys, hist,
                        (const uint32_t *)nullptr, (uint64_t *)nullptr);
     hipLaunchKernelGGL(bin_column_scan, dim3((nb + 15) / 16), dim3(256), 0, stream, rows, nb, hist, count);
-    hipLaunchKernelGGL(bin_tile_scan, dim3(1), dim3(1024), 0, stream, nb, count, start, ranges, (uint32_t)R, hdr);
+    hipLaunchKernelGGL(bin_tile_scan, dim3(1), dim3(1024), 0, stream, nb, count, start, ranges, (uint32_t)R, hdr, (uint32_t *)nullptr, (uint32_t *)nullptr, 0);
     hipLaunchKernelGGL(ray_bucket_pass<true>, dim3(rows), dim3(256), lds, stream, R, slice, nb, shift, ray_o, ray_d, (const float *)partial, rows, lead, keys, hist, start, pairs);
     launch_bucket_sorts(R, nb, ranges, pairs, (uint64_t *)nullptr, order, hdr, long_list, 0, stream);
     return (int)hipGetLastError();
@@ -606,7 +627,7 @@
     const size_t lds = sizeof(uint32_t) * (size_t)nb;
     hipLaunchKernelGGL(key_bucket_pass<false>, dim3(rows), dim3(256), lds, stream, n, slice, nb, shift, keys_in, hist, (const uint32_t *)nullptr, (uint64_t *)nullptr);
     hipLaunchKernelGGL(bin_column_scan, dim3((nb + 15) / 16), dim3(256), 0, stream, rows, nb, hist, count);
-    hipLaunchKernelGGL(bin_tile_scan, dim3(1), dim3(1024), 0, stream, nb, count, start, ranges, (uint32_t)n, hdr);
+    hipLaunchKernelGGL(bin_tile_scan, dim3(1), dim3(1024), 0, stream, nb, count, start, ranges, (uint32_t)n, hdr, (uint32_t *)nullptr, (uint32_t *)nullptr, 0);
     hipLaunchKernelGGL(key_bucket_pass<true>, dim3(rows), dim3(256), lds, stream, n, slice, nb, shift, keys_in, hist, start, keys_out);
     launch_bucket_sorts((uint64_t)n, nb, ranges, keys_out, keys_out, (uint32_t *)nullptr, hdr, long_list, 1, stream);
     return (int)hipGetLastError();
diff --git a/envgs_amd/csrc/raster_render.hip b/envgs_amd/csrc/raster_render.hip
--- a/envgs_amd/csrc/raster_render.hip
+++ b/envgs_amd/csrc/raster_render.hip
@@ -60,6 +60,32 @@
 {
     const int per = (ntiles + 7) >> 3;
     return (b & 7) * per + (b >> 3);
+}
+
+__device__ __forceinline__ int take_tile(const uint32_t *__restrict__ order, uint32_t *__restrict__ heads, const int ntiles, const int home,
+                                         const int nqueues, int &dry, int *s_tile)
+{
+    __syncthreads();
+    if (threadIdx.x == 0) {
+        const int per = nqueues ? (ntiles + 7) >> 3 : ntiles;
+        int t = -1;
+        while (dry < (nqueues ? nqueues : 1)) {
+            const int x = nqueues ? (home + dry) & 7 : 0;
+            const int cnt = min(per, ntiles - x * per);
+            if (cnt > 0) {
+                const uint32_t k = atomicAdd(heads + x * TQ_HEAD_STRIDE, 1u);
+                if (k < (uint32_t)cnt) {
+                    const uint32_t e = order[x * per + (int)k];
+                    t = e < (uint32_t)ntiles ? (int)e : -1;
+                    break;
+                }
+            }
+            dry++;
+        }
+        *s_tile = t;
+    }
+    __syncthreads();
+    return *s_tile;
 }
 
 __device__ __forceinline__ uint32_t quadrant_mask(const float4 r0, const float4 r1, const float4 r2, const float4 r3, int tile_px, int tile_py)
@@ -128,16 +154,24 @@
               const float *__restrict__ geom, const Feat colors, const float *__restrict__ bg,
               float *__restrict__ out_color, float *__restrict__ allmap, float *__restrict__ final_T,
               int32_t *__restrict__ n_contrib, float *__restrict__ weight, uint8_t *__restrict__ audit_contrib, int audit_lmax,
-              uint8_t *__restrict__ contrib_mask, const uint8_t *__restrict__ audit_skip)
+              uint8_t *__restrict__ contrib_mask, const uint8_t *__restrict__ audit_skip,
+              const uint32_t *__restrict__ order, uint32_t *__restrict__ heads, uint32_t *__restrict__ tile_cost, const int nqueues)
 {
     __shared__ TileLds<C> lds;
     __shared__ float wacc[256];
     __shared__ unsigned char cmk[256][4];
-    const int gx = (W + TILE - 1) / TILE, gy = (H + TILE - 1) / TILE;
-    const int tile = xcd_tile(blockIdx.x, gx * gy);
-    if (tile >= gx * gy) return;
+    __shared__ int s_tile;
+    __shared__ unsigned s_cost;
+    const int gx = (W + TILE - 1) / TILE, gy = (H + TILE - 1) / TILE, ntiles = gx * gy;
+    const int tid = threadIdx.x, wave = tid >> 6, lane = tid & 63;
+    const int home = order ? xcc_id() : 0;
+    int dry = 0;
+  for (bool first = true;; first = false) {
+    int tile;
+    if (order) tile = take_tile(order, heads, ntiles, home, nqueues, dry, &s_tile);
+    else tile = (first && xcd_tile(blockIdx.x, ntiles) < ntiles) ? xcd_tile(blockIdx.x, ntiles) : -1;
+    if (tile < 0) break;
     const int tx = tile % gx, ty = tile / gx;
-    const int tid = threadIdx.x, wave = tid >> 6, lane = tid & 63;
     const int pxi = tx * TILE + (wave & 1) * 8 + (lane & 7);
     const int pyi = ty * TILE + (wave >> 1) * 8 + (lane >> 3);
     const bool inside = pxi < W && pyi < H;
@@ -151,6 +185,7 @@
 #pragma unroll
     for (int c = 0; c < C; c++) Cacc[c] = 0.f;
     wacc[tid] = 0.f; reinterpret_cast<unsigned *>(&cmk[0][0])[tid] = 0u;
+    if (tid == 0) s_cost = 0u;
 
     for (uint32_t base = r0; base < r1; base += 256) {
         if (__syncthreads_and(done)) break;
@@ -211,16 +246,28 @@
           }
         }
         __syncthreads();
+        unsigned qmask = 0u;
         if (tid < count) {
             const float ws = wacc[tid];
             if (ws != 0.0f) { atomic_add_f32(weight + lds.id[tid], ws); wacc[tid] = 0.f; }
             if (contrib_mask) {
                 unsigned *cw = reinterpret_cast<unsigned *>(&cmk[0][0]) + tid;
                 const unsigned v = *cw;
-                contrib_mask[base + tid] = (uint8_t)((v & 1u) | ((v >> 7) & 2u) | ((v >> 14) & 4u) | ((v >> 21) & 8u));
+                qmask = (v & 1u) | ((v >> 7) & 2u) | ((v >> 14) & 4u) | ((v >> 21) & 8u);
+                contrib_mask[base + tid] = (uint8_t)qmask;
                 if (v) *cw = 0u;
             }
         }
+        if (tile_cost && contrib_mask) {
+            unsigned n = 0u;
+#pragma unroll
+            for (int q = 0; q < 4; q++) n += (unsigned)__builtin_popcountll(__builtin_amdgcn_ballot_w64((qmask >> q) & 1u));
+            if (lane == 0 && n) atomicAdd(&s_cost, n);
+        }
+    }
+    if (tile_cost && contrib_mask) {
+        __syncthreads();
+        if (tid == 0) tile_cost[tile] = s_cost;
     }
 
     if (inside) {
@@ -235,6 +282,7 @@
         allmap[5 * HW + pid] = med;
         allmap[6 * HW + pid] = dist;
     }
+  }
 }
 
 template <int C, bool DIST, bool EXACT>
@@ -392,17 +440,24 @@
               const float *__restrict__ geom, const Feat colors, const float *__restrict__ bg,
               const float *__restrict__ final_T, const int32_t *__restrict__ n_contrib,
               const float *__restrict__ dL_dcolor, const float *__restrict__ dL_dallmap, float *__restrict__ grad_rec,
-              const uint8_t *__restrict__ contrib_mask)
+              const uint8_t *__restrict__ contrib_mask, const uint32_t *__restrict__ order, uint32_t *__restrict__ heads, const int nqueues)
 {
     constexpr int V = 15 + C;
     __shared__ TileLds<C, BWD_BATCH> lds;
     __shared__ float gacc[BWD_BATCH][V];
-    __shared__ int s_max_last, s_dist;
-    const int gx = (W + TILE - 1) / TILE, gy = (H + TILE - 1) / TILE;
-    const int tile = xcd_tile(blockIdx.x, gx * gy);
-    if (tile >= gx * gy) return;
+    __shared__ int s_max_last, s_dist, s_tile;
+    const int gx = (W + TILE - 1) / TILE, gy = (H + TILE - 1) / TILE, ntiles = gx * gy;
+    const int tid = threadIdx.x, wave = tid >> 6, lane = tid & 63;
+    if (!order && xcd_tile(blockIdx.x, ntiles) >= ntiles) return;
+    for (int i = tid; i < BWD_BATCH * V; i += 256) (&gacc[0][0])[i] = 0.f;
+    const int home = order ? xcc_id() : 0;
+    int dry = 0;
+  for (bool first = true;; first = false) {
+    int tile;
+    if (order) tile = take_tile(order, heads, ntiles, home, nqueues, dry, &s_tile);
+    else tile = first ? xcd_tile(blockIdx.x, ntiles) : -1;
+    if (tile < 0) break;
     const int tx = tile % gx, ty = tile / gx;
-    const int tid = threadIdx.x, wave = tid >> 6, lane = tid & 63;
     const int pxi = tx * TILE + (wave & 1) * 8 + (lane & 7);
     const int pyi = ty * TILE + (wave >> 1) * 8 + (lane >> 3);
     const bool inside = pxi < W && pyi < H;
@@ -411,7 +466,6 @@
     const bool reg = inside && dL_dallmap && dL_dallmap[6 * HW + pid] != 0.0f;
 
     if (tid == 0) { s_max_last = 0; s_dist = 0; }
-    for (int i = tid; i < BWD_BATCH * V; i += 256) (&gacc[0][0])[i] = 0.f;
     __syncthreads();
     {
         int m = last;
@@ -428,36 +482,72 @@
         composite_bwd_tile<C, true, EXACT>(lds, gacc, W, H, bg_len, point_list, geom, colors, bg, final_T, n_contrib, dL_dcolor, dL_dallmap, grad_rec, r0, tx, ty, max_last, contrib_mask);
     else
         composite_bwd_tile<C, false, EXACT>(lds, gacc, W, H, bg_len, point_list, geom, colors, bg, final_T, n_contrib, dL_dcolor, dL_dallmap, grad_rec, r0, tx, ty, max_last, contrib_mask);
+  }
+}
+
+struct TileDispatch {
+    const uint32_t *order;
+    uint32_t *heads;
+    int nqueues;
+    unsigned grid;
+};
+
+template <typename Kernel>
+static TileDispatch tile_dispatch(Kernel kernel, int *slots , int ntiles, const uint32_t *order, uint32_t *heads)
+{
+    const int sw = debug_switch(ENVGS_DBG_BALANCE);
+    TileDispatch d{order, heads, (sw & 4) ? 8 : 0, (unsigned)(8 * ((ntiles + 7) / 8))};
+    if (!order || (sw & 2)) { d.order = nullptr; d.heads = nullptr; return d; }
+    int dev = 0;
+    if (hipGetDevice(&dev) != hipSuccess || dev < 0 || dev >= 16) dev = 0;
+    if (slots[dev] == 0) {
+        int cus = 0, per_cu = 0;
+        if (hipDeviceGetAttribute(&cus, hipDeviceAttributeMultiprocessorCount, dev) != hipSuccess || cus <= 0) cus = 64;
+        if (hipOccupancyMaxActiveBlocksPerMultiprocessor(&per_cu, kernel, 256, 0) != hipSuccess || per_cu <= 0) per_cu = 1;
+        slots[dev] = cus * per_cu;
+    }
+    const int cap = debug_switch(ENVGS_DBG_TILE_GRID);
+    d.grid = (unsigned)(cap > 0 ? (cap < slots[dev] ? cap : slots[dev]) : (ntiles < slots[dev] ? ntiles : slots[dev]));
+    return d;
+}
+
+template <int C, bool AUDIT, bool EXACT>
+static void launch_fwd(const envgs_raster_cfg *cfg, const uint32_t *ranges, const uint32_t *point_list, const float *geom,
+                       const Feat colors, const float *bg, float *out_color, float *allmap, float *final_T,
+                       int32_t *n_contrib, float *weight, uint8_t *audit_contrib, int audit_lmax, hipStream_t stream, uint8_t *contrib_mask,
+                       const uint8_t *audit_skip, uint32_t *tile_queue)
+{
+    static int slots[16] = {};
+    const int ntiles = ((cfg->width + TILE - 1) / TILE) * ((cfg->height + TILE - 1) / TILE);
+    const TileQueue tq = tile_queue_of(tile_queue, ntiles);
+    const TileDispatch d = tile_dispatch(composite_fwd<C, AUDIT, EXACT>, slots, ntiles, tile_queue ? tq.order6 : nullptr, tile_queue ? tq.heads6 : nullptr);
+    hipLaunchKernelGGL((composite_fwd<C, AUDIT, EXACT>), dim3(d.grid), dim3(256), 0, stream, cfg->width, cfg->height, cfg->bg_len, ranges,
+                       point_list, geom, colors, bg, out_color, allmap, final_T, n_contrib, weight, audit_contrib, audit_lmax, contrib_mask, audit_skip,
+                       d.order, d.heads, tile_queue ? tq.tile_cost : nullptr, d.nqueues);
 }
 
 template <int C>
 static int run_fwd(const envgs_raster_cfg *cfg, const uint32_t *ranges, const uint32_t *point_list, const float *geom,
                    const float *colors, const float *bg, float *out_color, float *allmap, float *final_T,
                    int32_t *n_contrib, float *weight, uint8_t *audit_contrib, int audit_lmax, hipStream_t stream, int colors_f16, uint8_t *contrib_mask,
-                   const uint8_t *audit_skip)
-{
-    const int gx = (cfg->width + TILE - 1) / TILE, gy = (cfg->height + TILE - 1) / TILE;
+                   const uint8_t *audit_skip, uint32_t *tile_queue)
+{
     ProfScope prof_(K_COMPOSITE_FWD, stream);
-    const dim3 grid(8 * ((gx * gy + 7) / 8)), block(256);
     const Feat colors_{colors, colors_f16 != 0};
 #ifdef ENVGS_DIAG
     if (debug_switch(ENVGS_DBG_RASTER_EXACT)) {
         if (audit_contrib)
-            hipLaunchKernelGGL((composite_fwd<C, true, true>), grid, block, 0, stream, cfg->width, cfg->height, cfg->bg_len, ranges,
-                               point_list, geom, colors_, bg, out_color, allmap, final_T, n_contrib, weight, audit_contrib, audit_lmax, contrib_mask, audit_skip);
+            launch_fwd<C, true, true>(cfg, ranges, point_list, geom, colors_, bg, out_color, allmap, final_T, n_contrib, weight, audit_contrib, audit_lmax, stream, contrib_mask, audit_skip, tile_queue);
         else
-            hipLaunchKernelGGL((composite_fwd<C, false, true>), grid, block, 0, stream, cfg->width, cfg->height, cfg->bg_len, ranges,
-                               point_list, geom, colors_, bg, out_color, allmap, final_T, n_contrib, weight, (uint8_t *)nullptr, 0, contrib_mask, (const uint8_t *)nullptr);
+            launch_fwd<C, false, true>(cfg, ranges, point_list, geom, colors_, bg, out_color, allmap, final_T, n_contrib, weight, nullptr, 0, stream, contrib_mask, nullptr, tile_queue);
         ENVGS_CHECK_LAUNCH(cfg, stream);
         return 0;
     }
 #endif
     if (audit_contrib)
-        hipLaunchKernelGGL((composite_fwd<C, true>), grid, block, 0, stream, cfg->width, cfg->height, cfg->bg_len, ranges,
-                           point_list, geom, colors_, bg, out_color, allmap, final_T, n_contrib, weight, audit_contrib, audit_lmax, contrib_mask, audit_skip);
+        launch_fwd<C, true, false>(cfg, ranges, point_list, geom, colors_, bg, out_color, allmap, final_T, n_contrib, weight, audit_contrib, audit_lmax, stream, contrib_mask, audit_skip, tile_queue);
     else
-        hipLaunchKernelGGL((composite_fwd<C, false>), grid, block, 0, stream, cfg->width, cfg->height, cfg->bg_len, ranges,
-                           point_list, geom, colors_, bg, out_color, allmap, final_T, n_contrib, weight, (uint8_t *)nullptr, 0, contrib_mask, (const uint8_t *)nullptr);
+        launch_fwd<C, false, false>(cfg, ranges, point_list, geom, colors_, bg, out_color, allmap, final_T, n_contrib, weight, nullptr, 0, stream, contrib_mask, nullptr, tile_queue);
     ENVGS_CHECK_LAUNCH(cfg, stream);
     return 0;
 }
@@ -465,52 +555,72 @@
 int launch_render_fwd(const envgs_raster_cfg *cfg, const uint32_t *ranges, const uint32_t *point_list, const float *geom,
                       const float *colors, const float *bg, float *out_color, float *allmap, float *final_T,
                       int32_t *n_contrib, float *weight, hipStream_t stream, uint8_t *audit_contrib, int audit_lmax, int colors_f16, uint8_t *contrib_mask,
-                      const uint8_t *audit_skip)
+                      const uint8_t *audit_skip, uint32_t *tile_queue)
 {
     if (cfg->P > 0) {
         hipError_t e = hipMemsetAsync(weight, 0, sizeof(float) * (size_t)cfg->P, stream);
         if (e != hipSuccess) return (int)e;
     }
     switch (cfg->channels) {
-    case 3: return run_fwd<3>(cfg, ranges, point_list, geom, colors, bg, out_color, allmap, final_T, n_contrib, weight, audit_contrib, audit_lmax, stream, colors_f16, contrib_mask, audit_skip);
-    case 5: return run_fwd<5>(cfg, ranges, point_list, geom, colors, bg, out_color, allmap, final_T, n_contrib, weight, audit_contrib, audit_lmax, stream, colors_f16, contrib_mask, audit_skip);
-    case 7: return run_fwd<7>(cfg, ranges, point_list, geom, colors, bg, out_color, allmap, final_T, n_contrib, weight, audit_contrib, audit_lmax, stream, colors_f16, contrib_mask, audit_skip);
+    case 3: return run_fwd<3>(cfg, ranges, point_list, geom, colors, bg, out_color, allmap, final_T, n_contrib, weight, audit_contrib, audit_lmax, stream, colors_f16, contrib_mask, audit_skip, tile_queue);
+    case 5: return run_fwd<5>(cfg, ranges, point_list, geom, colors, bg, out_color, allmap, final_T, n_contrib, weight, audit_contrib, audit_lmax, stream, colors_f16, contrib_mask, audit_skip, tile_queue);
+    case 7: return run_fwd<7>(cfg, ranges, point_list, geom, colors, bg, out_color, allmap, final_T, n_contrib, weight, audit_contrib, audit_lmax, stream, colors_f16, contrib_mask, audit_skip, tile_queue);
     default: return ENVGS_ERR_BAD_ARG;
     }
+}
+
+template <int C, bool EXACT>
+static void launch_bwd(const envgs_raster_cfg *cfg, const uint32_t *ranges, const uint32_t *point_list, const float *geom,
+                       const Feat colors, const float *bg, const float *final_T, const int32_t *n_contrib,
+                       const float *dL_dcolor, const float *dL_dallmap, float *grad_rec, hipStream_t stream, const uint8_t *contrib_mask, uint32_t *tile_queue)
+{
+    static int slots[16] = {};
+    const int ntiles = ((cfg->width + TILE - 1) / TILE) * ((cfg->height + TILE - 1) / TILE);
+    const TileQueue tq = tile_queue_of(tile_queue, ntiles);
+    const TileDispatch d = tile_dispatch(composite_bwd<C, EXACT>, slots, ntiles, tile_queue ? tq.order7 : nullptr, tile_queue ? tq.heads7 : nullptr);
+    hipLaunchKernelGGL((composite_bwd<C, EXACT>), dim3(d.grid), dim3(256), 0, stream, cfg->width, cfg->height, cfg->bg_len, ranges,
+                       point_list, geom, colors, bg, final_T, n_contrib, dL_dcolor, dL_dallmap, grad_rec, contrib_mask, d.order, d.heads, d.nqueues);
 }
 
 template <int C>
 static int run_bwd(const envgs_raster_cfg *cfg, const uint32_t *ranges, const uint32_t *point_list, const float *geom,
                    const float *colors, const float *bg, const float *final_T, const int32_t *n_contrib,
-                   const float *dL_dcolor, const float *dL_dallmap, float *grad_rec, hipStream_t stream, int colors_f16, const uint8_t *contrib_mask)
-{
-    const int gx = (cfg->width + TILE - 1) / TILE, gy = (cfg->height + TILE - 1) / TILE;
+                   const float *dL_dcolor, const float *dL_dallmap, float *grad_rec, hipStream_t stream, int colors_f16, const uint8_t *contrib_mask,
+                   uint32_t *tile_queue)
+{
     ProfScope prof_(K_COMPOSITE_BWD, stream);
+    const Feat colors_{colors, colors_f16 != 0};
 #ifdef ENVGS_DIAG
     if (debug_switch(ENVGS_DBG_RASTER_EXACT)) {
-        hipLaunchKernelGGL((composite_bwd<C, true>), dim3(8 * ((gx * gy + 7) / 8)), dim3(256), 0, stream, cfg->width, cfg->height, cfg->bg_len, ranges,
-                           point_list, geom, Feat{colors, colors_f16 != 0}, bg, final_T, n_contrib, dL_dcolor, dL_dallmap, grad_rec, contrib_mask);
+        launch_bwd<C, true>(cfg, ranges, point_list, geom, colors_, bg, final_T, n_contrib, dL_dcolor, dL_dallmap, grad_rec, stream, contrib_mask, tile_queue);
         ENVGS_CHECK_LAUNCH(cfg, stream);
         return 0;
     }
 #endif
-    hipLaunchKernelGGL((composite_bwd<C, false>), dim3(8 * ((gx * gy + 7) / 8)), dim3(256), 0, stream, cfg->width, cfg->height, cfg->bg_len, ranges,
-                       point_list, geom, Feat{colors, colors_f16 != 0}, bg, final_T, n_contrib, dL_dcolor, dL_dallmap, grad_rec, contrib_mask);
+    launch_bwd<C, false>(cfg, ranges, point_list, geom, colors_, bg, final_T, n_contrib, dL_dcolor, dL_dallmap, grad_rec, stream, contrib_mask, tile_queue);
     ENVGS_CHECK_LAUNCH(cfg, stream);
     return 0;
 }
 
 int launch_render_bwd(const envgs_raster_cfg *cfg, const uint32_t *ranges, const uint32_t *point_list, const float *geom,
                       const float *colors, const float *bg, const float *final_T, const int32_t *n_contrib,
-                      const float *dL_dcolor, const float *dL_dallmap, float *grad_rec, hipStream_t stream, int colors_f16, const uint8_t *contrib_mask)
+                      const float *dL_dcolor, const float *dL_dallmap, float *grad_rec, hipStream_t stream, int colors_f16, const uint8_t *contrib_mask,
+                      uint32_t *tile_queue)
 {
     if (cfg->P <= 0) return 0;
+    if (tile_queue) {
+        const int ntiles = ((cfg->width + TILE - 1) / TILE) * ((cfg->height + TILE - 1) / TILE);
+        const TileQueue tq = tile_queue_of(tile_queue, ntiles);
+        if (contrib_mask) launch_tile_order(ntiles, tq.tile_cost, nullptr, 1, tq.order7, tq.heads7, stream);
+        else launch_tile_order(ntiles, ranges + 1, ranges, 2, tq.order7, tq.heads7, stream);
+        ENVGS_CHECK_LAUNCH(cfg, stream);
+    }
     hipError_t e = hipMemsetAsync(grad_rec, 0, sizeof(float) * GREC * (size_t)cfg->P, stream);
     if (e != hipSuccess) return (int)e;
     switch (cfg->channels) {
-    case 3: return run_bwd<3>(cfg, ranges, point_list, geom, colors, bg, final_T, n_contrib, dL_dcolor, dL_dallmap, grad_rec, stream, colors_f16, contrib_mask);
-    case 5: return run_bwd<5>(cfg, ranges, point_list, geom, colors, bg, final_T, n_contrib, dL_dcolor, dL_dallmap, grad_rec, stream, colors_f16, contrib_mask);
-    case 7: return run_bwd<7>(cfg, ranges, point_list, geom, colors, bg, final_T, n_contrib, dL_dcolor, dL_dallmap, grad_rec, stream, colors_f16, contrib_mask);
+    case 3: return run_bwd<3>(cfg, ranges, point_list, geom, colors, bg, final_T, n_contrib, dL_dcolor, dL_dallmap, grad_rec, stream, colors_f16, contrib_mask, tile_queue);
+    case 5: return run_bwd<5>(cfg, ranges, point_list, geom, colors, bg, final_T, n_contrib, dL_dcolor, dL_dallmap, grad_rec, stream, colors_f16, contrib_mask, tile_queue);
+    case 7: return run_bwd<7>(cfg, ranges, point_list, geom, colors, bg, final_T, n_contrib, dL_dcolor, dL_dallmap, grad_rec, stream, colors_f16, contrib_mask, tile_queue);
     default: return ENVGS_ERR_BAD_ARG;
     }
 }
diff --git a/envgs_amd/csrc/trace_common.h b/envgs_amd/csrc/trace_common.h
--- a/envgs_amd/csrc/trace_common.h
+++ b/envgs_amd/csrc/trace_common.h
@@ -498,13 +498,6 @@
 
 __device__ __forceinline__ int xcd_block(int b, int nblocks) { return (b & 7) * (nblocks >> 3) + (b >> 3); }
 
-__device__ __forceinline__ int xcc_id()
-{
-    unsigned v;
-    asm volatile("s_getreg_b32 %0, hwreg(HW_REG_XCC_ID)" : "=s"(v));
-    return (int)(v & 7u);
-}
-
 __device__ __forceinline__ int fetch_batch(unsigned *ctr , int nbatch, int home, int lane)
 {
     const int per = (nbatch + 7) >> 3;
diff --git a/envgs_amd/raster.py b/envgs_amd/raster.py
--- a/envgs_amd/raster.py
+++ b/envgs_amd/raster.py
@@ -85,6 +85,7 @@
     return t
 
 
+TILE_QUEUE = {"on": True}
 CONTRIB_MASK = {"on": True}
 
 
@@ -145,11 +146,12 @@
         bin_bytes = lib.envgs_raster_sort_temp_bytes(max(cap, 1), W, H)
         bin_temp = torch.empty(max(bin_bytes, 1), dtype=torch.uint8, device=dev)
         cmask = torch.empty(max(cap, 1), dtype=torch.uint8, device=dev) if CONTRIB_MASK["on"] else None
-        _lib.check(lib.envgs_raster_bin_and_render(cfg, cap, p(geom), p(radii), p(colors), p(bg), p(pairs), p(keys_s), p(point_list),
-                                                   p(bin_temp), bin_bytes, p(ranges), p(out_color), p(allmap), p(final_T),
-                                                   p(n_contrib), p(weight), p(cmask), stream),
-                   "envgs_raster_bin_and_render")
-        return pairs, keys_s, point_list, cmask
+        tq = torch.empty(lib.envgs_raster_tile_queue_bytes(W, H) // 4, **i32) if TILE_QUEUE["on"] else None
+        _lib.check(lib.envgs_raster_bin_and_render_queued(cfg, cap, p(geom), p(radii), p(colors), p(bg), p(pairs), p(keys_s), p(point_list),
+                                                          p(bin_temp), bin_bytes, p(ranges), p(out_color), p(allmap), p(final_T),
+                                                          p(n_contrib), p(weight), p(cmask), p(tq), stream),
+                   "envgs_raster_bin_and_render_queued")
+        return pairs, keys_s, point_list, cmask, tq
 
     key = (dev.index, P, H, W)
     guess = _N_GUESS.get(key) if SPECULATIVE_N["on"] else None
@@ -174,15 +176,21 @@
         if N > cap:
             LAST_STATS["n_guess_misses"] = LAST_STATS.get("n_guess_misses", 0) + 1
             bufs = bin_and_render(N)
-    pairs, keys_s, point_list, cmask = bufs
+    pairs, keys_s, point_list, cmask, tq = bufs
     _N_GUESS[key] = max(((max(int(N * 1.15), N + 4096) + 65535) // 65536) * 65536, int(0.97 * (guess or 0)))
     LAST_STATS.update(N=N, P=P, H=H, W=W, C=C)
     saved = dict(cfg=cfg, N=N, geom=geom, colors=colors, bg=bg, point_list=point_list, ranges=ranges, final_T=final_T,
-                 n_contrib=n_contrib, contrib_mask=cmask, means3D=means3D, scales=scales, rotations=rotations, shs=shs, clamped=clamped,
+                 n_contrib=n_contrib, contrib_mask=cmask, tile_queue=tq, means3D=means3D, scales=scales, rotations=rotations, shs=shs, clamped=clamped,
                  cov3D_precomp=cov3D_precomp, radii=radii, view=view, proj=proj, campos=campos)
     if keep_binning:
         saved.update(tiles_touched=tiles, offsets=offsets, tile_pairs=pairs, keys_sorted=keys_s)
     return (out_color, radii, allmap, weight), saved
+
+
+def tile_queue_views(saved):
+    tq = saved["tile_queue"]
+    n = (tq.numel() - 512) // 3
+    return dict(heads6=tq[0:256:32], heads7=tq[256:512:32], order6=tq[512:512 + n], order7=tq[512 + n:512 + 2 * n], tile_cost=tq[512 + 2 * n:512 + 3 * n])
 
 
 def render_audit(saved, lmax, skip_px=None, want_weight=False):
@@ -224,12 +232,12 @@
     dshs = torch.empty(shs.shape, **f32) if shs is not None else None
     dcolors = torch.empty(P, C, **f32) if shs is None else None
     p = _lib.ptr
-    _lib.check(lib.envgs_raster_backward(cfg, saved["N"], p(saved["geom"]), p(saved["colors"]), p(saved["bg"]),
+    _lib.check(lib.envgs_raster_backward_queued(cfg, saved["N"], p(saved["geom"]), p(saved["colors"]), p(saved["bg"]),
                                          p(saved["point_list"]), p(saved["ranges"]), p(saved["final_T"]), p(saved["n_contrib"]),
                                          p(saved.get("contrib_mask")), p(dL_dcolor), p(dL_dallmap), p(saved["means3D"]), p(saved["scales"]), p(saved["rotations"]),
                                          p(shs), p(saved["clamped"]), p(cov), p(saved["radii"]), p(saved["view"]), p(saved["proj"]),
                                          p(saved["campos"]), p(grad_rec), p(dmeans3D), p(dmeans2D), p(dscales), p(drots), p(dshs),
-                                         p(dcolors), p(dopac), p(dcov), _stream(dev)), "envgs_raster_backward")
+                                         p(dcolors), p(dopac), p(dcov), p(saved.get("tile_queue")), _stream(dev)), "envgs_raster_backward_queued")
     return dict(means3D=dmeans3D, means2D=dmeans2D, shs=dshs, colors_precomp=dcolors, opacities=dopac, scales=dscales,
                 rotations=drots, cov3D_precomp=dcov, grad_rec=grad_rec)
 
diff --git a/include/envgs_raster.h b/include/envgs_raster.h
--- a/include/envgs_raster.h
+++ b/include/envgs_raster.h
@@ -57,6 +57,15 @@
                                 float *out_color, float *allmap, float *final_T, int32_t *n_contrib,
                                 float *weight, uint8_t *contrib_mask, void *stream);
 
+ENVGS_API size_t envgs_raster_tile_queue_bytes(int32_t width, int32_t height);
+ENVGS_API int envgs_raster_bin_and_render_queued(const envgs_raster_cfg *cfg, uint32_t N,
+                                const float *geom, const int32_t *radii,
+                                const float *colors, const float *bg,
+                                uint64_t *tile_pairs, uint64_t *keys_sorted , uint32_t *point_list,
+                                void *bin_temp, size_t bin_temp_bytes, uint32_t *ranges,
+                                float *out_color, float *allmap, float *final_T, int32_t *n_contrib,
+                                float *weight, uint8_t *contrib_mask, uint32_t *tile_queue, void *stream);
+
 ENVGS_API int envgs_raster_render_audit(const envgs_raster_cfg *cfg, const float *geom, const float *colors, const float *bg,
                               const uint32_t *point_list, const uint32_t *ranges,
                               float *out_color, float *allmap, float *final_T, int32_t *n_contrib, float *weight,
@@ -75,6 +84,19 @@
                           float *dmeans3D, float *dmeans2D, float *dscales, float *drots,
                           float *dshs, float *dcolors, float *dopacities, float *dtransmat_precomp,
                           void *stream);
+ENVGS_API int envgs_raster_backward_queued(const envgs_raster_cfg *cfg, uint32_t N,
+                          const float *geom, const float *colors, const float *bg,
+                          const uint32_t *point_list, const uint32_t *ranges,
+                          const float *final_T, const int32_t *n_contrib, const uint8_t *contrib_mask ,
+                          const float *dL_dcolor, const float *dL_dallmap,
+                          const float *means3D, const float *scales, const float *rotations,
+                          const float *shs, const uint8_t *clamped, const float *transmat_precomp,
+                          const int32_t *radii,
+                          const float *viewmatrix, const float *projmatrix, const float *campos,
+                          float *grad_rec,
+                          float *dmeans3D, float *dmeans2D, float *dscales, float *drots,
+                          float *dshs, float *dcolors, float *dopacities, float *dtransmat_precomp,
+                          uint32_t *tile_queue, void *stream);
 
 ENVGS_API void envgs_prof_enable(int on);
 ENVGS_API void envgs_prof_select(uint64_t kernel_mask);
@@ -92,7 +114,8 @@
 #define ENVGS_DBG_RAYKEY 4
 #define ENVGS_DBG_SPARSE 5
 #define ENVGS_DBG_BALANCE 6
-#define ENVGS_DBG_COUNT 7
+#define ENVGS_DBG_TILE_GRID 7
+#define ENVGS_DBG_COUNT 8
 ENVGS_API void envgs_debug_set(int32_t which, int32_t value);
 ENVGS_API int32_t envgs_debug_get(int32_t which);
 
diff --git a/profiles/raster_schedule_model.py b/profiles/raster_schedule_model.py
--- /dev/null
+++ b/profiles/raster_schedule_model.py
@@ -0,0 +1,132 @@
+import argparse
+import heapq
+import importlib
+import os
+import sys
+
+HERE = os.path.dirname(os.path.abspath(__file__))
+sys.path[:] = [os.path.dirname(HERE)] + [p for p in sys.path if os.path.abspath(p or ".") != HERE]
+
+import numpy as np
+
+CLASSES = 32
+
+
+def by_class(key, tiles):
+    cls = (key.astype(np.int64) * CLASSES) // (int(key.max()) + 1)
+    return sorted(tiles, key=lambda t: (-cls[t], t))
+
+
+def fixed_dispatch(cost, slots):
+    n = len(cost)
+    per = (n + 7) // 8
+    free = [[0.0] * (slots // 8) for _ in range(8)]
+    started, end = 0.0, 0.0
+    for b in range(8 * per):
+        x, t = b & 7, (b & 7) * per + (b >> 3)
+        if t >= n:
+            continue
+        started = max(started, heapq.heappop(free[x]))
+        heapq.heappush(free[x], started + cost[t])
+        end = max(end, started + cost[t])
+    return end
+
+
+def persistent(cost, key, slots, banded, steal=True):
+    n = len(cost)
+    per = (n + 7) // 8
+    if banded:
+        queues = [by_class(key, range(x * per, min(n, (x + 1) * per))) for x in range(8)]
+    else:
+        queues = [by_class(key, range(n))] + [[] for _ in range(7)]
+    heads = [0] * 8
+    workers = [(0.0, w & 7) for w in range(slots)]
+    heapq.heapify(workers)
+    end = 0.0
+    while workers:
+        now, x = heapq.heappop(workers)
+        for k in range(8 if (steal or not banded) else 1):
+            q = (x + k) & 7 if banded else 0
+            if heads[q] < len(queues[q]):
+                t = queues[q][heads[q]]
+                heads[q] += 1
+                end = max(end, now + cost[t])
+                heapq.heappush(workers, (now + cost[t], x))
+                break
+    return end
+
+
+def report(name, cost, key, slots, out):
+    cost = cost.astype(np.float64)
+    ideal = cost.sum() / slots
+    a = fixed_dispatch(cost, slots)
+    b = persistent(cost, key, slots, True)
+    b0 = persistent(cost, key, slots, True, steal=False)
+    c = persistent(cost, key, slots, False)
+    out("    %-34s ideal %8.0f  heaviest/ideal %.2f   makespan/ideal  (a) %.3f  (b) %.3f  (b, no stealing) %.3f  (c) %.3f" % (
+        name, ideal, cost.max() / ideal, a / ideal, b / ideal, b0 / ideal, c / ideal))
+    return a, b, c
+
+
+def main():
+    ap = argparse.ArgumentParser()
+    ap.add_argument("--out", required=True)
+    ap.add_argument("--save-counts", default=None, help="directory for the per-view count arrays (.npy)")
+    ap.add_argument("--from-counts", default=None, help="directory of saved count arrays: no GPU")
+    ap.add_argument("--gaussians", type=int, default=300000)
+    ap.add_argument("--res", type=int, default=800)
+    a = ap.parse_args()
+    lines = []
+    out = lambda s="": (lines.append(s), print(s, flush=True))
+    P, H, W, C = a.gaussians, a.res, a.res, 5
+    out("R6 / R7 tile schedules simulated from the per-tile work, %d base surfels, %dx%d, the eight bench views" % (P, H, W))
+    out("R6 on 1280 slots, R7 on 1024; makespan in units of work (entries / passes); see profiles/raster_schedule_model.py")
+    out()
+    if not a.from_counts:
+        import torch
+        from envgs_amd import raster, synth
+        dev = torch.device("cuda:0")
+        g = synth.base_gaussians(P, seed=0, device=dev)
+        pkg = importlib.import_module("diff_surfel_rasterization_wet_ch05")
+        sh_degree = torch.tensor([3], device=dev)
+    tot = {"R6 by list length": [0.0] * 3, "R6 by walked entries": [0.0] * 3, "R7": [0.0] * 3}
+    for v in range(8):
+        if a.from_counts:
+            inst, walked, pas = np.load(os.path.join(a.from_counts, "raster_tiles_view%d.npy" % v)).T
+        else:
+            cam = synth.orbit_camera(v, n_views=8, H=H, W=W, fx=1111.1 * W / 800.0, device=dev)
+            st = pkg.GaussianRasterizationSettings(image_height=H, image_width=W, tanfovx=cam.tanfovx, tanfovy=cam.tanfovy, bg=torch.zeros(C, device=dev),
+                                                   scale_modifier=1.0, viewmatrix=cam.world_view_transform, projmatrix=cam.full_proj_transform,
+                                                   sh_degree=sh_degree, campos=cam.camera_center, prefiltered=False, debug=False)
+            with torch.no_grad():
+                _, sv = raster.rasterize_forward(C, g["means3D"], None, torch.zeros(P, C, device=dev), g["opacities"], g["scales"], g["rotations"], None, st)
+            rg = sv["ranges"].view(-1, 2).long().cpu().numpy()
+            cm = sv["contrib_mask"][:sv["N"]].cpu().numpy()
+            inst = rg[:, 1] - rg[:, 0]
+            gx, gy = (W + 15) // 16, (H + 15) // 16
+            last = torch.zeros(gy * 16, gx * 16, dtype=torch.int32, device=dev)
+            last[:H, :W] = sv["n_contrib"][0]
+            walked = last.view(gy, 16, gx, 16).amax(dim=(1, 3)).reshape(-1).long().cpu().numpy()
+            c_pas = np.concatenate([[0], np.cumsum(np.unpackbits(cm[:, None], axis=1).sum(1))])
+            pas = c_pas[rg[:, 0] + np.minimum(walked, inst)] - c_pas[rg[:, 0]]
+            if sv.get("tile_queue") is not None:
+                assert np.array_equal(raster.tile_queue_views(sv)["tile_cost"].cpu().numpy().astype(np.int64), pas)
+            if a.save_counts:
+                os.makedirs(a.save_counts, exist_ok=True)
+                np.save(os.path.join(a.save_counts, "raster_tiles_view%d.npy" % v), np.stack([inst, walked, pas], 1))
+        out("view %d: %d tiles, %d instances, %d walked, %d passes; per tile mean / max: instances %.0f / %d, walked %.0f / %d, passes %.0f / %d" % (
+            v, len(inst), inst.sum(), walked.sum(), pas.sum(), inst.mean(), inst.max(), walked.mean(), walked.max(), pas.mean(), pas.max()))
+        for name, cost, key, slots in (("R6 by list length", inst, inst, 1280), ("R6 by walked entries", walked, inst, 1280), ("R7", pas, pas, 1024)):
+            r = report("%s (queue key = %s)" % (name, "passes" if name == "R7" else "list length"), cost, key, slots, out)
+            tot[name] = [x + y for x, y in zip(tot[name], r)]
+    out()
+    out("summed makespan over the eight views, (b) and (c) against (a):")
+    for name, (sa, sb, sc) in tot.items():
+        out("    %-22s (a) %10.0f  (b) %10.0f = %.3f (a)  (c) %10.0f = %.3f (a)" % (name, sa, sb, sb / sa, sc, sc / sa))
+    os.makedirs(os.path.dirname(os.path.abspath(a.out)), exist_ok=True)
+    with open(a.out, "w") as f:
+        f.write("\n".join(lines) + "\n")
+
+
+if __name__ == "__main__":
+    main()
```

Result: faster. 148.6, median of 6 (+1.3%).
